# william-dawson/NTPoly

Hardware: AMD Instinct MI355X
Metric: TRS2 iters/s + SpGEMM nnz-out/s, N=262k ~200 nnz/row, 1/2/4/8 GPU (higher is better)
Workload: dtype f64

## Files before the change

### include/ntpoly_amd.h

```cpp
#ifndef NTPOLY_AMD_H
#define NTPOLY_AMD_H
#include "ntpoly_amd_process_grid.h"
#include "ntpoly_amd_psmatrix.h"
#include "ntpoly_amd_smatrix.h"
#include "ntpoly_amd_triplet_list.h"
#include "ntpoly_amd_permutation.h"
#include "ntpoly_amd_memory_pool.h"
#include "ntpoly_amd_solver_parameters.h"
#include "ntpoly_amd_density_matrix_solvers.h"
#include "ntpoly_amd_sign_solvers.h"
#include "ntpoly_amd_inverse_solvers.h"
#include "ntpoly_amd_square_root_solvers.h"
#include "ntpoly_amd_load_balancer.h"
#include "ntpoly_amd_eigen_bounds.h"
#include "ntpoly_amd_logging.h"
#include "ntpoly_amd_polynomial_solvers.h"
#include "ntpoly_amd_function_solvers.h"
#include "ntpoly_amd_linear_solvers.h"
#include "ntpoly_amd_eigen_solvers.h"
#include "ntpoly_amd_geometry.h"
#ifdef __cplusplus
extern "C" {
#endif

void ntpoly_amd_allreduce_max(double* values, const int* n);
int ntpoly_amd_band_order(const int* ih, int* newpos, long long* bandwidth);
void ntpoly_amd_band_scope_counts(long long* out);
void ntpoly_amd_band_searches(long long* out);
void ntpoly_amd_barrier();
void ntpoly_amd_block_algebra_counts(long long* out);
int ntpoly_amd_block_order(const int* ih, int* position);
int ntpoly_amd_block_order_of_pattern(const int* ih, int* position, int* ns);
void ntpoly_amd_block_scope_counts(long long* out);
void ntpoly_amd_column_fused_counts(long long* out);
int ntpoly_amd_comm_rank();
int ntpoly_amd_comm_size();
void ntpoly_amd_comm_split_matrix(const int* ih_this, int* ih_split, int* my_color, bool* split_slice);
void ntpoly_amd_complex_fusion_counts(long long* out);
int ntpoly_amd_device_count();
void ntpoly_amd_drop_block_caches();
void ntpoly_amd_drop_grouped_caches();
void ntpoly_amd_exchange_stats(long long* out);
void ntpoly_amd_fill_prepartitioned(const int* ih_this, const int* ih_triplet_list);
void ntpoly_amd_finalize_comm();
void ntpoly_amd_fusion_counts(long long* out);
void ntpoly_amd_gather_matrix_to_process(const int* ih_this, int* ih_local, const int* within_slice_id);
int ntpoly_amd_get_option(const char* name);
void ntpoly_amd_get_spgemm_accum(long long* out, double* dout);
void ntpoly_amd_get_unique_id(char* out128);
void ntpoly_amd_ghash_class_counts(long long out[4]);
void ntpoly_amd_grid_comm_info(const int* ih_grid, int* out);
void ntpoly_amd_halo_segment(const int* dim, const int* nranks, const int* s, const int* kmin, const int* kmax, int* a, int* b);
void ntpoly_amd_increment_identity(const int* ih_identity, int* ih_matB, const double* alpha);
void ntpoly_amd_init_comm(const char* id128, const int* rank, const int* nranks);
void ntpoly_amd_isr_chain_counts(long long out[3]);
int ntpoly_amd_isr_chain_step(const int* ih_X, const int* ih_X2, const int* order, const double* a, const double* b, const double* c, int* ih_Out1, int* ih_Out2);
void ntpoly_amd_last_block_stats(long long* out, double* fill);
void ntpoly_amd_last_grouped_stats(long long* out, double* ratio);
void ntpoly_amd_last_spgemm_stats(long long* out, float* ms_numeric, float* ms_total);
int ntpoly_amd_last_spgemm_thin();
void ntpoly_amd_log_element_bool(const char* key, const int* nk, const bool* v);
void ntpoly_amd_log_element_int(const char* key, const int* nk, const int* v);
void ntpoly_amd_log_element_real(const char* key, const int* nk, const double* v);
void ntpoly_amd_log_element_string(const char* key, const int* nk, const char* v, const int* nv);
void ntpoly_amd_log_enter();
void ntpoly_amd_log_exit();
void ntpoly_amd_log_header(const char* text, const int* n);
void ntpoly_amd_log_list_element(const char* key, const int* nk);
void ntpoly_amd_malloc_stats(long long* calls, double* ms);
int ntpoly_amd_matrix_is_complex(const int* ih_this);
void ntpoly_amd_matrix_local_columns(const int* ih_this, int* c0, int* c1);
void ntpoly_amd_memory(long long* in_use, long long* cached);
int ntpoly_amd_norm_axpby(const int* ih_matA, const int* ih_matB, const double* alpha, const double* beta, double* norm);
void ntpoly_amd_panel_exchange_layout(const int* dim, const int* nranks, const int* me, const long long* req, const long long* cnt, int* sa, int* sb, long long* soff, int* ra, int* rb, long long* zoff);
void ntpoly_amd_panel_product_counts(long long* out);
void ntpoly_amd_panel_range(const int* dim, const int* nranks, const int* rank, int* c0, int* c1);
void ntpoly_amd_permutation_set(int* ih_this, const int* n, const int* index_lookup);
int ntpoly_amd_pm_fused_step(const int* ih_X, const int* ih_Z, const int* ih_X2, const int* ih_X3, const double* a1, const double* a2, const double* a3, const double* thr, int* ih_Out, int* ih_Zout, double* sc);
void ntpoly_amd_pm_session_counts(long long out[4]);
void ntpoly_amd_pm_session_longest_list(long long* out);
int ntpoly_amd_recurrence_step(const int* ih_P, const int* ih_Tkm2, int* ih_Tk, int* ih_R, const double* a, const double* c);
void ntpoly_amd_recurrence_step_count(long long* out);
void ntpoly_amd_release_cache();
void ntpoly_amd_reset_spgemm_accum();
void ntpoly_amd_session_begin(const int* complex_ok);
void ntpoly_amd_session_end();
void ntpoly_amd_set_option(const char* name, const int* value);
void ntpoly_amd_slab_algebra_counts(long long* out);
void ntpoly_amd_slab_view_counts(long long out[4]);
void ntpoly_amd_split_process_grid(const int* ih_old_grid, int* ih_new_grid, int* my_color, bool* split_slice);
void ntpoly_amd_square_root_order(const int* ih_Input, int* ih_Output, const int* ih_solver_parameters, const int* inverse, const int* order);
void ntpoly_amd_synchronize();
void ntpoly_amd_thin_slab_counts(long long* out);
void ntpoly_amd_tile2_counts(long long* out);
void ntpoly_amd_trace_get(double* value, double* energy, double* sigma, long long* nnz);
int ntpoly_amd_trace_iterations();
void ntpoly_amd_trace_times(double* setup_ms, double* loop_ms);
void ntpoly_amd_triplets_get(const int* ih_list, int* col, int* row, double* val);
void ntpoly_amd_triplets_set_c(int* ih_list, const long long* n, const int* col, const int* row, const double* val_ri);
void ntpoly_amd_triplets_set_r(int* ih_list, const long long* n, const int* col, const int* row, const double* val);
void ntpoly_amd_trs2_step(int* ih_X, int* ih_X2, const int* ih_WH, const double* trace, const double* threshold, double* energy_out, double* sigma_out, double* trace_io);

#ifdef __cplusplus
}
#endif
#endif
```

### ntpoly_amd/csrc/common.hpp

```cpp
#pragma once
#include <hip/hip_runtime.h>

#include <cstdint>
#include <cstdio>
#include <cstdlib>
#include <map>
#include <string>
#include <utility>
#include <memory>
#include <vector>

namespace ntp {

[[noreturn]] void fatal(const char* file, int line, const std::string& msg);
#define NTP_FATAL(msg) ::ntp::fatal(__FILE__, __LINE__, (msg))
#define HIP_CHECK(expr)                                                              \
  do {                                                                               \
    hipError_t e_ = (expr);                                                          \
    if (e_ != hipSuccess)                                                            \
      ::ntp::fatal(__FILE__, __LINE__, std::string(#expr) + ": " + hipGetErrorString(e_)); \
  } while (0)

struct Context {
  int device = 0;
  hipStream_t stream = nullptr;
  hipStream_t comm_stream = nullptr;
  int num_cus = 256;
  bool initialised = false;
};
Context& ctx();
void ensure_init();
inline hipStream_t stream() { return ctx().stream; }
void sync_stream();
long long& host_sync_count();

struct ScalarFetch {
  const void* src[16];
  int words[16];
  void* dst[16];
  int n = 0;
  void add(const void* dev, int words8, void* host_dst) {
    src[n] = dev; words[n] = words8; dst[n] = host_dst; ++n;
  }
  void run();
};

void* dev_alloc(size_t bytes);
void dev_free(void* p);
unsigned long long dev_alloc_serial(const void* p);
void dev_release_cache();
size_t dev_bytes_in_use();
size_t dev_bytes_cached();
void dev_malloc_stats(long long* calls, double* ms);

template <typename T>
struct DevBuf {
  T* p = nullptr;
  size_t n = 0;
  DevBuf() = default;
  explicit DevBuf(size_t count) { alloc(count); }
  DevBuf(const DevBuf&) = delete;
  DevBuf& operator=(const DevBuf&) = delete;
  DevBuf(DevBuf&& o) noexcept : p(o.p), n(o.n) { o.p = nullptr; o.n = 0; }
  DevBuf& operator=(DevBuf&& o) noexcept {
    if (this != &o) {
      release();
      p = o.p; n = o.n; o.p = nullptr; o.n = 0;
    }
    return *this;
  }
  ~DevBuf() { release(); }
  void alloc(size_t count) {
    release();
    n = count;
    p = static_cast<T*>(dev_alloc((count ? count : 1) * sizeof(T)));
  }
  void release() {
    if (p) dev_free(p);
    p = nullptr; n = 0;
  }
  void upload(const T* host, size_t count) {
    if (count) HIP_CHECK(hipMemcpyAsync(p, host, count * sizeof(T), hipMemcpyHostToDevice, stream()));
  }
  void download(T* host, size_t count) const {
    const size_t bytes = count * sizeof(T);
    if (bytes > 0 && bytes <= 1024 && bytes % 8 == 0) {
      ScalarFetch f;
      f.add(p, (int)(bytes / 8), host);
      f.run();
      return;
    }
    if (count) HIP_CHECK(hipMemcpyAsync(host, p, bytes, hipMemcpyDeviceToHost, stream()));
    sync_stream();
  }
  void zero() { if (n) HIP_CHECK(hipMemsetAsync(p, 0, n * sizeof(T), stream())); }
};

constexpr size_t kIndexSlack = 1024;

struct SlabPlan {
  DevBuf<int32_t> blk_lo, blk_w, blk_kmin, blk_kn;
  DevBuf<int64_t> blk_toff;
  int64_t total = 0;
  int max_w = 0, max_kn = 0;
  int align = 0;
};
struct SlabForm {
  DevBuf<int32_t> first, last, count;
  DevBuf<int64_t> off;
  DevBuf<int64_t> tile_off;
  DevBuf<double> val, tiles;
  int64_t slots = 0;
  bool no_tile2 = false;
  std::unique_ptr<SlabPlan> next_plan;
  std::shared_ptr<struct DevMat> origin;
  DevBuf<int32_t> zlast;
  mutable int64_t span_sum = -1;
  int row_pad = 1;
  DevBuf<int32_t> lab, plast;
  bool labelled() const { return lab.p != nullptr; }
};

struct DevMat {
  int32_t rows = 0, cols = 0;
  bool cplx = false;
  int64_t nnz = 0;
  DevBuf<int64_t> outer;
  DevBuf<int32_t> inner;
  DevBuf<double> val;
  DevBuf<int32_t> cnt;
  int64_t slots = 0;
  bool loose() const { return cnt.p != nullptr; }
  mutable int zero_free = 0;
  std::unique_ptr<SlabForm> slab;
  bool expanded() const { return slab != nullptr; }
  std::shared_ptr<struct BlockForm> blk;
  bool blocked() const { return blk != nullptr; }
  mutable int block_hint = 0;
  mutable int slab_hint = 0;

  DevMat() = default;
  DevMat(int32_t r, int32_t c, bool z) { reset_empty(r, c, z); }
  DevMat(DevMat&&) noexcept = default;
  DevMat& operator=(DevMat&&) noexcept = default;
  void reset_empty(int32_t r, int32_t c, bool z);
  void alloc(int32_t r, int32_t c, bool z, int64_t nz);
  DevMat clone() const;
  size_t wval() const { return cplx ? 2 : 1; }
};

DevMat packed_copy(const DevMat& M);

struct HostTriplets {
  std::vector<int32_t> col, row;
  std::vector<double> val;
  bool cplx = false;
  size_t size() const { return col.size(); }
};

}
```

### ntpoly_amd/csrc/kernels.hip

```cpp
#include "kernels.hpp"
#include "device_util.hpp"
#include "spgemm_grouped.hpp"
#include "slab_types.hpp"
#include "spgemm_tile.hpp"
#include "spgemm_block.hpp"

#include <hip/hip_runtime.h>

#include <algorithm>
#include <cstdlib>
#include <climits>
#include <cmath>
#include <cstring>
#include <type_traits>
#include <numeric>
#include <utility>

#include <rocprim/device/device_radix_sort.hpp>

namespace ntp {

namespace {

__global__ __launch_bounds__(1024) void k_scan_excl_i64(const int64_t* __restrict__ in,
// ... 2590 lines not shown

static int64_t exclusive_scan_i64_from_i32(const int32_t* d_in, int64_t* d_out, int64_t n) {
  scan_async<int32_t>(d_in, d_out, n);
  int64_t total = 0;
  ScalarFetch f;
  f.add(d_out + n, 1, &total);
  f.run();
  return total;
}
int64_t exclusive_scan_i64(const int64_t* d_in, int64_t* d_out, int64_t n) {
  scan_async<int64_t>(d_in, d_out, n);
  int64_t total = 0;
  HIP_CHECK(hipMemcpyAsync(&total, d_out + n, sizeof(int64_t), hipMemcpyDeviceToHost, stream()));
  sync_stream();
  return total;
}

namespace {
struct TimedCall {
  hipEvent_t ev[4];
};
std::vector<hipEvent_t>& event_pool() {
  static auto* p = new std::vector<hipEvent_t>();
  return *p;
}
std::vector<TimedCall>& pending_timings() {
  static auto* p = new std::vector<TimedCall>();
  return *p;
}
hipEvent_t get_event() {
  auto& pool = event_pool();
  if (!pool.empty()) {
    hipEvent_t e = pool.back();
    pool.pop_back();
    return e;
  }
  hipEvent_t e;
  HIP_CHECK(hipEventCreate(&e));
  return e;
}
struct EventTimer {
  hipEvent_t a = nullptr, b = nullptr;
  bool on;
  explicit EventTimer(bool enable) : on(enable) {
    if (on) {
      a = get_event();
      b = get_event();
    }
  }
  void start() { if (on) HIP_CHECK(hipEventRecord(a, stream())); }
  void stop() { if (on) HIP_CHECK(hipEventRecord(b, stream())); }
};
}

namespace {
unsigned long long& value_epoch() {
  static unsigned long long e = 0;
  return e;
}
}
unsigned long long matrix_value_epoch() { return value_epoch(); }
void bump_matrix_value_epoch() { value_epoch() += 1; }
namespace {
struct DotOperand {
  const void* val = nullptr;
  unsigned long long serial = 0, epoch = 0;
  int64_t nnz = -1;
  int32_t cols = 0;
  DevBuf<int32_t> dmin, dmax;
  DevBuf<int64_t> doff;
  DevBuf<double> dexp;
  int64_t max_tile = 0;
  int align = 1;
};
template <typename T>
__global__ __launch_bounds__(256) void k_count_zero_values(Csc A, unsigned long long* __restrict__ out, int32_t* __restrict__ zlast) {
  const int j = (blockIdx.x * blockDim.x + threadIdx.x) / WAVE;
  if (j >= A.cols) return;
  const int lane = lane_id();
  const T* __restrict__ v = static_cast<const T*>(A.val);
  int zl = -1;
  for (int64_t p = A.outer[j] + lane, e = col_end(A, j); p < e; p += WAVE)
    if (Sc<T>::is_zero(v[p])) zl = max(zl, A.inner[p]);
  zl = wave_max_i32(zl);
  if (lane == 0) {
    if (zlast) zlast[j] = zl;
    if (zl >= 0) atomicAdd(out, 1ull);
  }
}
__global__ void k_span_block_max(const int32_t* __restrict__ span, int n, int J, unsigned long long* __restrict__ out) {
  const int b = blockIdx.x * blockDim.x + threadIdx.x;
  if (b * J >= n) return;
  unsigned long long t = 0;
  for (int j = b * J; j < min(n, (b + 1) * J); ++j) t += (unsigned long long)span[j];
  atomicMax(out, t);
}
DotOperand*& dot_operand_slot() {
  static DotOperand* c = new DotOperand();
  return c;
}
void drop_dot_operand() { *dot_operand_slot() = DotOperand(); }
const DotOperand& dot_operand(const DevMat& D) {
  DotOperand* c = dot_operand_slot();
  const unsigned long long ser = dev_alloc_serial(D.val.p);
  const int want_al = options().spgemm_fma == 1 ? tile_expand_align() : 1;
  if (c->val == D.val.p && c->serial == ser && ser != 0 && c->epoch == value_epoch() && c->nnz == D.nnz && c->cols == D.cols &&
      c->align == want_al)
    return *c;
  const int n = D.cols;
  c->dmin.alloc((size_t)n); c->dmax.alloc((size_t)n); c->doff.alloc((size_t)n + 1);
  DevBuf<int32_t> dlen((size_t)n), dspan((size_t)n);
  hipLaunchKernelGGL(k_col_extent, dim3(cdiv(n, 256)), dim3(256), 0, stream(), view(D), c->dmin.p, c->dmax.p, dlen.p);
  const int al = options().spgemm_fma == 1 ? tile_expand_align() : 1;
  if (al > 1) hipLaunchKernelGGL(k_span_aligned, dim3(cdiv(n, 256)), dim3(256), 0, stream(), c->dmin.p, c->dmax.p, dspan.p, n, al);
  else hipLaunchKernelGGL(k_span_of, dim3(cdiv(n, 256)), dim3(256), 0, stream(), c->dmin.p, c->dmax.p, dspan.p, n);
  scan_async<int32_t>(dspan.p, c->doff.p, (int64_t)n);
  DevBuf<unsigned long long> tmax(1);
  tmax.zero();
  hipLaunchKernelGGL(k_span_block_max, dim3(cdiv(cdiv(n, SLAB_J), 256)), dim3(256), 0, stream(), dspan.p, n, SLAB_J, tmax.p);
  int64_t total = 0;
  unsigned long long hmax = 0;
  {
    ScalarFetch f;
    f.add(c->doff.p + n, 1, &total);
    f.add(tmax.p, 1, &hmax);
    f.run();
  }
  c->max_tile = (int64_t)hmax;
  c->dexp.alloc((size_t)total + 1);
  if (al > 1)
    hipLaunchKernelGGL(k_aligned_offsets<double>, dim3(cdiv((int64_t)n * WAVE, 256)), dim3(256), 0, stream(), c->dmin.p, c->dmax.p,
                       c->doff.p, c->dexp.p, n, al);
  c->align = al;
  hipLaunchKernelGGL(k_slab_expand_a<double>, dim3(cdiv((int64_t)n * WAVE, 256)), dim3(256), 0, stream(), view(D), c->dmin.p,
                     c->doff.p, c->dexp.p);
  c->val = D.val.p;
  c->serial = ser;
  c->epoch = value_epoch();
  c->nnz = D.nnz;
  c->cols = n;
  return *c;
}
}

long long* fusion_counts() {
  static long long c[3] = {0, 0, 0};
  return c;
}
long long* complex_fusion_counts() {
  static long long c[3] = {0, 0, 0};
  return c;
}
long long* tile2_counts() {
  static long long c[2] = {0, 0};
  return c;
}

void flush_spgemm_timers() {
  auto& pend = pending_timings();
  if (pend.empty()) return;
  SpgemmAccum& acc = spgemm_accum();
  for (size_t i = 0; i < pend.size(); ++i) {
    float t_all = 0.f, t_num = 0.f;
    HIP_CHECK(hipEventSynchronize(pend[i].ev[1]));
    HIP_CHECK(hipEventElapsedTime(&t_all, pend[i].ev[0], pend[i].ev[1]));
    HIP_CHECK(hipEventElapsedTime(&t_num, pend[i].ev[2], pend[i].ev[3]));
    acc.ms_total += t_all;
    acc.ms_numeric += t_num;
    if (i + 1 == pend.size()) {
      last_spgemm_stats().ms_total = t_all;
      last_spgemm_stats().ms_numeric = t_num;
    }
    for (int k = 0; k < 4; ++k) event_pool().push_back(pend[i].ev[k]);
  }
  pend.clear();
}

namespace {
__global__ __launch_bounds__(256) void k_pack_slab(int ncols, const int32_t* __restrict__ first, const int32_t* __restrict__ last,
                                                   const int64_t* __restrict__ off, const double* __restrict__ val,
                                                   const int64_t* __restrict__ outer, int32_t* __restrict__ inner,
                                                   double* __restrict__ out) {
  const int j = (blockIdx.x * blockDim.x + threadIdx.x) / WAVE;
  if (j >= ncols) return;
  const int lane = lane_id();
  const int f = first[j], l = last[j];
  int64_t pos = outer[j];
  const double* __restrict__ src = val + off[j];
  for (int r0 = f; r0 <= l; r0 += WAVE) {
    const int r = r0 + lane;
    const double v = r <= l ? src[r - f] : 0.0;
    const unsigned long long m = __ballot(v != 0.0);
    if (v != 0.0) {
      const int64_t q = pos + __popcll(m & lanemask_lt());
      inner[q] = r;
      out[q] = v;
    }
    pos += __popcll(m);
  }
}
__global__ __launch_bounds__(256) void k_pack_slab_c(int ncols, const int32_t* __restrict__ first, const int32_t* __restrict__ last,
                                                     const int64_t* __restrict__ off, const double2* __restrict__ val,
                                                     const int64_t* __restrict__ outer, int32_t* __restrict__ inner,
                                                     double2* __restrict__ out) {
  const int j = (blockIdx.x * blockDim.x + threadIdx.x) / WAVE;
  if (j >= ncols) return;
  const int lane = lane_id();
  const int f = first[j], l = last[j];
  int64_t pos = outer[j];
  const double2* __restrict__ src = val + off[j];
  for (int r0 = f; r0 <= l; r0 += WAVE) {
    const int r = r0 + lane;
    const double2 v = r <= l ? src[r - f] : make_double2(0.0, 0.0);
    const bool nz = v.x != 0.0 || v.y != 0.0;
    const unsigned long long m = __ballot(nz);
    if (nz) {
      const int64_t q = pos + __popcll(m & lanemask_lt());
      inner[q] = r;
      out[q] = v;
    }
    pos += __popcll(m);
  }
}
template <int MAXCH, int NW>
void launch_pair3(int bin_lo, int bin_hi, int wrt, const DevMat& A, const DevMat& B, const int32_t* lo, const int32_t* span,
                  const uint8_t* binarr, const int64_t* tmpoff, int32_t* out_inner, double* out_val, int32_t* count,
                  double alpha, double thr, int dense_rule) {
  const int ngroups = cdiv(B.cols, 2);
  const int nblocks = cdiv(ngroups, NW);
  const size_t lds = (size_t)NW * 2 * (size_t)wrt * sizeof(double);
  hipLaunchKernelGGL((k_spgemm_pair3<MAXCH, NW>), dim3(xcd_grid(nblocks)), dim3(NW * WAVE), lds, stream(), view(A), view(B),
                     lo, span, binarr, bin_lo, bin_hi, tmpoff, out_inner, out_val, count, alpha, thr, dense_rule, nblocks, wrt);
}

template <typename T, int W, int NW>
void launch_window(int bin, const DevMat& A, const DevMat& B, const int32_t* lo, const int32_t* span,
                   const uint8_t* binarr, const int64_t* tmpoff, int32_t* out_inner, T* out_val,
                   int32_t* count, double alpha, double thr, int dense_rule) {
  const int nblocks = cdiv(B.cols, NW);
  hipLaunchKernelGGL((k_spgemm_window<T, W, NW>), dim3(xcd_grid(nblocks)), dim3(NW * WAVE), 0, stream(),
                     view(A), view(B), lo, span, binarr, bin, tmpoff, out_inner, out_val, count, alpha, thr,
                     dense_rule, nblocks);
}
}

namespace {
struct StripCtx { bool active = false, failed = false; };
constexpr int kMaxStrips = 16;
int* strips_memory(bool cplx) {
  static int m[2][2] = {{-1, 0}, {-1, 0}};
  return m[cplx ? 1 : 0];
}
StripCtx& strip_ctx() {
  static StripCtx c;
  return c;
}
template <typename T>
__global__ __launch_bounds__(256) void k_strip_count(Csc A, int shift, int S, int s, int32_t* __restrict__ cnt) {
  const int j = (blockIdx.x * blockDim.x + threadIdx.x) / WAVE;
  if (j >= A.cols) return;
  const int lane = lane_id();
  int c = 0;
  for (int64_t p = A.outer[j] + lane, e = A.outer[j + 1]; p < e; p += WAVE) c += ((A.inner[p] >> shift) % S) == s ? 1 : 0;
  c = (int)wave_sum_i64(c);
  if (lane == 0) cnt[j] = c;
}
template <typename T>
__global__ __launch_bounds__(256) void k_strip_fill(Csc A, int shift, int S, int s, const int64_t* __restrict__ outer,
                                                    int32_t* __restrict__ inner, T* __restrict__ val) {
  const int j = (blockIdx.x * blockDim.x + threadIdx.x) / WAVE;
  if (j >= A.cols) return;
  const int lane = lane_id();
  const T* __restrict__ Av = static_cast<const T*>(A.val);
  int64_t pos = outer[j];
  for (int64_t p0 = A.outer[j], e = A.outer[j + 1]; p0 < e; p0 += WAVE) {
    const int64_t p = p0 + lane;
    const bool in = p < e && ((A.inner[p] >> shift) % S) == s;
    const unsigned long long m = __ballot(in);
    if (in) {
      const int64_t q = pos + __popcll(m & lanemask_lt());
      inner[q] = A.inner[p];
      val[q] = Av[p];
    }
    pos += __popcll(m);
  }
}
struct StripCols { const int64_t* outer[16]; const int32_t* inner[16]; const void* val[16]; };
__global__ void k_strip_total(StripCols P, int S, int n, int32_t* __restrict__ total) {
  const int j = blockIdx.x * blockDim.x + threadIdx.x;
  if (j >= n) return;
  int t = 0;
  for (int s = 0; s < S; ++s) t += (int)(P.outer[s][j + 1] - P.outer[s][j]);
  total[j] = t;
}
template <typename T>
__global__ __launch_bounds__(256) void k_strip_merge(StripCols P, int S, int shift, int n, const int64_t* __restrict__ outer,
                                                     int32_t* __restrict__ inner, T* __restrict__ val) {
  const int j = (blockIdx.x * blockDim.x + threadIdx.x) / WAVE;
  if (j >= n) return;
  const int lane = lane_id();
  int rmin = INT_MAX, rmax = -1;
  for (int s = 0; s < S; ++s) {
    const int64_t a = P.outer[s][j], e = P.outer[s][j + 1];
    if (e > a) {
      rmin = min(rmin, P.inner[s][a]);
      rmax = max(rmax, P.inner[s][e - 1]);
// ... 947 lines not shown
  C.rows = m;
  C.cols = n;
  C.cplx = A.cplx;
  C.outer.alloc((size_t)n + 1);
  scan_async<int32_t>(count.p, C.outer.p, (int64_t)n);
  int64_t nnz = 0;
  unsigned long long slab_products = 0;
  {
    ScalarFetch f;
    f.add(C.outer.p + n, 1, &nnz);
    if (use_slab) f.add(blk_prod_scan.p + snb, 1, &slab_products);
    f.run();
  }
  if (use_slab) st.products = (int64_t)slab_products;
  C.nnz = nnz;
  C.inner.alloc((size_t)nnz + kIndexSlack);
  C.val.alloc(((size_t)nnz + kIndexSlack) * C.wval());
  const int nblocks = cdiv(n, 4);
  if (use_tile)
    hipLaunchKernelGGL(k_pack_slab, dim3(cdiv((int64_t)n * WAVE, 256)), dim3(256), 0, stream(), n, fz_first.p, fz_last.p,
                       tile_ooff.p, tmp_val.p, C.outer.p, C.inner.p, C.val.p);
  else if (use_ctile)
    hipLaunchKernelGGL(k_pack_slab_c, dim3(cdiv((int64_t)n * WAVE, 256)), dim3(256), 0, stream(), n, fz_first.p, fz_last.p,
                       tile_ooff.p, reinterpret_cast<const double2*>(tmp_val.p), C.outer.p, C.inner.p, reinterpret_cast<double2*>(C.val.p));
  else dispatch_type(A.cplx, [&](auto tag) {
    using T = decltype(tag);
    hipLaunchKernelGGL((k_compact<T>), dim3(xcd_grid(nblocks)), dim3(256), 0, stream(), n, tmpoff.p,
                       overflow ? tmpoff2.p : nullptr, overflow ? bin.p : nullptr, C.outer.p, tmp_inner.p,
                       reinterpret_cast<const T*>(tmp_val.p), tmp2_inner.p, reinterpret_cast<const T*>(tmp2_val.p),
                       C.inner.p, reinterpret_cast<T*>(C.val.p), nblocks);
  });
  t_all.stop();
  st.nnz_c = nnz;
  if (timing) {
    if (pending_timings().size() >= 4096) flush_spgemm_timers();
    pending_timings().push_back(TimedCall{{t_all.a, t_all.b, t_num.a, t_num.b}});
  }
  last_spgemm_stats() = st;
  SpgemmAccum& acc = spgemm_accum();
  acc.calls += 1;
  acc.products += st.products;
  acc.nnz_c += nnz;
  const double per = A.cplx ? 20.0 : 12.0;
  acc.alg_bytes += per * (double)(A.nnz + B.nnz + nnz) + 4.0 * ((double)A.cols + B.cols + n + 3);
}


namespace {
}

namespace {
__global__ void k_pack_reduce4(const double* __restrict__ tot, const int* __restrict__ flag, double* __restrict__ out) {
  out[0] = tot[3];
  out[1] = 0.0;
  out[2] = tot[4];
  out[3] = flag[0] == 0 ? 1.0 : 0.0;
}
__global__ void k_slab_runs_addr(const int32_t* __restrict__ first, const int32_t* __restrict__ last,
                                 const unsigned long long* __restrict__ addr, unsigned long long fallback,
                                 SlabRun* __restrict__ runs, int n, int elem_bytes) {
  const int k = blockIdx.x * blockDim.x + threadIdx.x;
  if (k >= n + 4) return;
  const bool any = k < n && last[k] >= first[k];
  SlabRun r;
  const unsigned long long a = any ? addr[k] : fallback;
  r.addr_lo = (uint32_t)a;
  r.addr_hi = (uint32_t)(a >> 32) & 0xffffu;
  r.nbytes = any ? (uint32_t)(last[k] - first[k] + 1) * (uint32_t)elem_bytes : 0u;
  r.flags = kBufferFlags;
  r.first = any ? first[k] : (1 << 30);
  r.first8 = any ? first[k] * elem_bytes : 0;
  r.span62 = any ? (last[k] - first[k] + 1) + 62 : 0;
  r.pad = 0;
  runs[k] = r;
}

__global__ __launch_bounds__(256) void k_slab_order_steps(const int32_t* __restrict__ lab, const int32_t* __restrict__ blk_kmin,
                                                          const int32_t* __restrict__ blk_kn, const int64_t* __restrict__ tile_off,
                                                          const double* __restrict__ tiles_in, const SlabRun* __restrict__ runs,
                                                          int ncols, double* __restrict__ tiles_out, SlabRun* __restrict__ blkruns,
                                                          int32_t* __restrict__ steps, int nblocks) {
  extern __shared__ unsigned long long sk[];
  const int b = xcd_block(nblocks);
  if (b < 0) return;
  const int kn = blk_kn[b], kmin = blk_kmin[b];
  if (kn == 0) return;
  int m = 1;
  while (m < kn) m <<= 1;
  for (int i = threadIdx.x; i < m; i += blockDim.x)
    sk[i] = i < kn ? (((unsigned long long)(unsigned)lab[kmin + i] << 32) | (unsigned)i) : ~0ull;
  __syncthreads();
  for (int k = 2; k <= m; k <<= 1) {
    for (int j = k >> 1; j > 0; j >>= 1) {
      for (int i = threadIdx.x; i < m; i += blockDim.x) {
        const int l = i ^ j;
        if (l > i) {
          const bool up = (i & k) == 0;
          const unsigned long long x = sk[i], y = sk[l];
          if ((x > y) == up) { sk[i] = y; sk[l] = x; }
        }
      }
      __syncthreads();
    }
  }
  const int64_t toff = tile_off[b];
  const int64_t rbase = toff / SLAB_J + 4 * (int64_t)b;
  for (int t = threadIdx.x; t < kn + 4; t += blockDim.x) {
    if (t < kn) {
      const int i = (int)(unsigned)(sk[t] & 0xffffffffull);
      const int k = kmin + i;
      if (steps) steps[rbase + t] = k;
      SlabRun r = runs[k];
      r.pad = i * (int)(SLAB_J * sizeof(double));
      blkruns[rbase + t] = r;
    } else {
      if (steps) steps[rbase + t] = ncols;
      blkruns[rbase + t] = runs[ncols];
    }
  }
  if (!tiles_out) return;
  const double2* __restrict__ src = reinterpret_cast<const double2*>(tiles_in + toff);
  double2* __restrict__ dst = reinterpret_cast<double2*>(tiles_out + toff);
  for (int i = threadIdx.x; i < kn * (SLAB_J / 2); i += blockDim.x) {
    const int t = i / (SLAB_J / 2), q = i % (SLAB_J / 2);
    dst[(size_t)t * (SLAB_J / 2) + q] = src[(size_t)(unsigned)(sk[t] & 0xffffffffull) * (SLAB_J / 2) + q];
  }
}
}

namespace {
template <int J = SLAB_J>
void launch_slab_plan(SlabPlan& P, int n, const int32_t* first, const int32_t* last, const int32_t* afirst, const int32_t* alast,
                      int align, unsigned long long* stats, DevBuf<int64_t>* tile_offsets = nullptr) {
  const int snb = cdiv(n, J);
  P.blk_lo.alloc(snb); P.blk_w.alloc(snb); P.blk_kmin.alloc(snb); P.blk_kn.alloc(snb);
  P.blk_toff.alloc((size_t)snb + 1);
  P.align = align;
  DevBuf<int64_t> bsz(snb), tsz(snb);
  if (tile_offsets) tile_offsets->alloc((size_t)snb + 1);
  hipLaunchKernelGGL((k_slab_plan<J>), dim3(cdiv((int64_t)snb * WAVE, 256)), dim3(256), 0, stream(), n, first, last, afirst,
                     alast, P.blk_lo.p, P.blk_w.p, P.blk_kmin.p, P.blk_kn.p, bsz.p, tsz.p, snb, align);
  if (options().plan_fused != 0) {
    const int part = cdiv(cdiv(snb, kOffParts), 256) * 256;
    hipLaunchKernelGGL(k_slab_offsets, dim3(cdiv(snb, part)), dim3(256), 0, stream(), P.blk_w.p, P.blk_kn.p, tsz.p, bsz.p, snb, part,
                       P.blk_toff.p, tile_offsets ? tile_offsets->p : (int64_t*)nullptr, stats);
    return;
  }
  hipLaunchKernelGGL(k_slab_reduce, dim3(64), dim3(256), 0, stream(), P.blk_w.p, P.blk_kn.p, snb, (const int32_t*)nullptr, 0, stats);
  scan_async<int64_t>(tsz.p, P.blk_toff.p, (int64_t)snb);
  if (tile_offsets) scan_async<int64_t>(bsz.p, tile_offsets->p, (int64_t)snb);
}
}

bool slab_step(DevMat& X, SlabFusion& fu, double threshold, bool dense_rule, const SlabHalo* halo) {
  fu.done = false;
  if (!X.expanded() || X.cplx || (!halo && X.rows != X.cols) || !fu.D || fu.D->cplx || fu.D->loose() || fu.D->expanded() ||
      fu.D->rows != X.rows || fu.D->cols != X.cols || (fu.mode != 1 && fu.mode != 2))
    return false;
  const bool tile = options().spgemm_fma == 1;
  if ((options().spgemm_variant >= 0 && !(tile && options().spgemm_variant / 100 == 6)) || (options().spgemm_fma && !tile) || options().spgemm_force_bin > 0 || !options().fused_update)
    return false;
  const SlabForm& in = *X.slab;
  int trows = 1;
  if (tile) {
    trows = tile_rows();
    while (trows > 1 && (in.row_pad % (16 * trows) != 0 || (halo && halo->row_pad % (16 * trows) != 0))) trows >>= 1;
  }
  const int n = X.cols, snb = cdiv(n, SLAB_J);
  const DotOperand& dop = dot_operand(*fu.D);
  if (!tile && dop.max_tile > SLAB_DTILE) return false;
  const bool timing = options().time_kernels != 0;
  EventTimer t_all(timing), t_num(timing);
  t_all.start();
  SpgemmStats st;
  st.nnz_a = st.nnz_b = X.nnz;
  DevBuf<int32_t> count((size_t)n), ofirst((size_t)n), olast((size_t)n);
  DevBuf<int64_t> tmpoff((size_t)n + 1);
  DevBuf<int64_t> zwords((size_t)4 * snb + 4 + 48);
  zwords.zero();
  if (!tile) count.zero();
  int64_t* fz_flag = zwords.p;
  int64_t* fz_pnnz = zwords.p + 2;
  double* fz_part = reinterpret_cast<double*>(zwords.p + 3 + 2 * (size_t)snb);
  unsigned long long* stats = reinterpret_cast<unsigned long long*>(zwords.p + 4 * (size_t)snb + 4);
  unsigned long long* next_stats = stats + 24;
  const int ka = halo ? halo->ka : 0, nka = halo ? halo->kb - halo->ka : n;
  const int plan_align = tile ? 16 * tile_rows() : 0;
  SlabPlan own_plan;
  SlabPlan* plan = &own_plan;
  if (!halo && in.next_plan && in.next_plan->align == plan_align && (int64_t)in.next_plan->blk_lo.n == snb) {
    plan = in.next_plan.get();
  } else if (halo && halo->plan && halo->plan->align == plan_align && (int64_t)halo->plan->blk_lo.n == snb) {
    plan = halo->plan;
  } else {
    const int32_t* afirst = halo ? halo->first - ka : in.first.p;
    const int32_t* alast = halo ? halo->last - ka : in.last.p;
    launch_slab_plan(own_plan, n, in.first.p, in.last.p, afirst, alast, plan_align, stats);
    unsigned long long hs[3] = {0, 0, 0};
    ScalarFetch f;
    f.add(own_plan.blk_toff.p + snb, 1, &own_plan.total);
    f.add(stats + 16, 3, hs);
    f.run();
    own_plan.max_w = (int)hs[0];
    own_plan.max_kn = (int)hs[1];
  }
  DevBuf<int32_t>&blk_lo = plan->blk_lo, &blk_w = plan->blk_w, &blk_kmin = plan->blk_kmin, &blk_kn = plan->blk_kn;
  DevBuf<int64_t>& blk_toff = plan->blk_toff;
  const int64_t tmp_total = plan->total;
  const unsigned long long hst[2] = {(unsigned long long)plan->max_w, (unsigned long long)plan->max_kn};
  const int64_t max_w = (int64_t)hst[0];
  auto give_up = [&]() {
    if (timing) {
      event_pool().push_back(t_all.a); event_pool().push_back(t_all.b);
      event_pool().push_back(t_num.a); event_pool().push_back(t_num.b);
    }
    return false;
  };
  if (max_w <= 0 || (!tile && max_w > 8 * SLAB_SL * WAVE)) return give_up();
  if (tile && !spgemm_tile_fits((int)hst[1], (int)max_w)) return give_up();
  if (in.labelled() && (int64_t)hst[1] > 2048) return give_up();
  if (!tile)
    hipLaunchKernelGGL((k_slab_tmpoff<SLAB_J>), dim3(cdiv(n + 1, 256)), dim3(256), 0, stream(), n, blk_w.p, blk_toff.p, tmpoff.p);
  DevBuf<char> runs(((size_t)nka + 4) * sizeof(SlabRun));
  if (halo)
    hipLaunchKernelGGL(k_slab_runs_addr, dim3(cdiv(nka + 4, 256)), dim3(256), 0, stream(), halo->first, halo->last, halo->addr,
                       (unsigned long long)reinterpret_cast<uintptr_t>(in.val.p), reinterpret_cast<SlabRun*>(runs.p), nka, 8);
  else
    hipLaunchKernelGGL(k_slab_runs, dim3(cdiv(n + 4, 256)), dim3(256), 0, stream(), in.first.p, in.last.p, in.off.p,
                       reinterpret_cast<const char*>(in.val.p), 8, reinterpret_cast<SlabRun*>(runs.p), n);
  const size_t oslots = (size_t)tmp_total + (size_t)tmp_total / 5 + kIndexSlack;
  const bool runs_only = tile && !halo && options().tile_runs_only != 0;
  DevBuf<double> oval(oslots), otiles(runs_only ? 0 : oslots);
  SlabFuseArgs fz;
  fz.am = fu.am; fz.bm = fu.bm; fz.thr_m = fu.threshold;
  fz.xexp = in.val.p; fz.xoff = in.off.p; fz.xmin = in.first.p; fz.xmax = in.last.p;
  fz.dexp = dop.dexp.p; fz.doff = dop.doff.p; fz.dmin = dop.dmin.p; fz.dmax = dop.dmax.p;
  fz.ofirst = ofirst.p; fz.olast = olast.p; fz.tiles = runs_only ? nullptr : otiles.p;
  fz.part = fz_part; fz.pnnz = reinterpret_cast<long long*>(fz_pnnz); fz.flag = reinterpret_cast<int*>(fz_flag);
  fz.col_offset = fu.col_offset;
  int64_t* blk_prod = zwords.p + 3 + snb;
  const bool labelled = in.labelled() && !halo && !tile;
  if (in.labelled() && halo) return give_up();
  DevBuf<double> tiles_ord;
  DevBuf<char> blkruns;
  DevBuf<int32_t> steps, oplast;
  const bool rowoff = labelled && options().label_rowoff != 0;
  if (labelled) {
    const size_t nrec = in.tiles.n / SLAB_J + 4 * (size_t)snb + 8;
    blkruns.alloc(nrec * sizeof(SlabRun));
    oplast.alloc((size_t)n);
    if (!rowoff) {
      tiles_ord.alloc(in.tiles.n);
      steps.alloc(nrec);
    }
    int m = 1;
    while (m < (int)hst[1]) m <<= 1;
    hipLaunchKernelGGL(k_slab_order_steps, dim3(xcd_grid(snb)), dim3(256), (size_t)m * 8, stream(), in.lab.p, blk_kmin.p, blk_kn.p,
                       in.tile_off.p, in.tiles.p, reinterpret_cast<const SlabRun*>(runs.p), n, tiles_ord.p,
                       reinterpret_cast<SlabRun*>(blkruns.p), steps.p, snb);
    fz.lab = in.lab.p;
    fz.blkruns = reinterpret_cast<const SlabRun*>(blkruns.p);
    fz.steps = steps.p;
    fz.xplast = in.plast.p;
    fz.oplast = oplast.p;
  }
  const bool scope_lab = tile && halo && !in.labelled() && scope_labels() != nullptr && in.plast.p != nullptr && fu.mode != 0;
  const bool tile_labelled = tile && ((in.labelled() && !halo) || scope_lab);
  if (tile_labelled) {
    oplast.alloc((size_t)n);
    fz.lab = scope_lab ? scope_labels() : in.lab.p;
    fz.xplast = in.plast.p;
    fz.oplast = oplast.p;
  }
  fz.prod = reinterpret_cast<long long*>(blk_prod);
  if (!halo || halo->count) fz.in_count = halo ? halo->count - ka : in.count.p;
  DevBuf<char> fz_args;
  if (!tile) {
    fz_args.alloc(sizeof(SlabFuseArgs));
    fz_args.upload(reinterpret_cast<const char*>(&fz), sizeof(SlabFuseArgs));
  }
  const int dr = dense_rule ? 1 : 0;
  t_num.start();
  auto launch = [&](auto nw_tag, auto mode_tag, auto epi_tag) {
    constexpr int FNW = decltype(nw_tag)::value;
    hipLaunchKernelGGL((k_spgemm_slab<SLAB_J, SLAB_SL, FNW, decltype(mode_tag)::value, decltype(epi_tag)::value>),
                       dim3(xcd_grid(snb)), dim3(FNW * WAVE), 0, stream(), reinterpret_cast<const SlabRun*>(runs.p) - ka,
                       (labelled && !rowoff) ? tiles_ord.p : in.tiles.p, in.tile_off.p, blk_kmin.p, blk_kn.p, blk_lo.p, blk_w.p, blk_toff.p, (int32_t*)nullptr,
                       oval.p, count.p, 1.0, threshold, dr, n, snb, reinterpret_cast<const SlabFuseArgs*>(fz_args.p));
  };
  auto by_mode = [&](auto nw_tag, auto mode_tag) {
    if (fu.mode == 1) launch(nw_tag, mode_tag, std::integral_constant<int, 1>{});
    else launch(nw_tag, mode_tag, std::integral_constant<int, 2>{});
  };
  DevBuf<int64_t> tile_ooff, tile_otoff;
  bool used_tile2 = false;
  if (tile) {
    tile_ooff.alloc((size_t)n + 1);
    tile_otoff.alloc((size_t)snb + 1);
    TileLaunch tl;
    tl.runs = reinterpret_cast<const SlabRun*>(runs.p) - ka;
    tl.bblk = in.tiles.p; tl.blk_boff = in.tile_off.p;
    if (in.tiles.p == nullptr || in.tile_off.p == nullptr) {
      tl.bblk = nullptr; tl.blk_boff = nullptr;
      tl.brun_first = in.first.p; tl.brun_last = in.last.p; tl.brun_off = in.off.p; tl.brun_val = in.val.p; tl.bbytes = in.val.n * sizeof(double); tl.brun_pad = in.row_pad;
    }
    tl.blk_kmin = blk_kmin.p; tl.blk_kn = blk_kn.p; tl.blk_lo = blk_lo.p;
    tl.blk_w = blk_w.p; tl.blk_toff = blk_toff.p; tl.out_val = oval.p; tl.count = count.p;
    tl.ofirst = ofirst.p; tl.olast = olast.p; tl.ooff = tile_ooff.p; tl.otoff = tile_otoff.p;
    tl.alpha = 1.0; tl.threshold = threshold; tl.dense_rule = dr; tl.ncols = n; tl.nblocks = snb;
    tl.max_kn = (int)hst[1]; tl.max_w = (int)max_w; tl.epi = fu.mode; tl.fz = &fz; tl.rows = trows; tl.labelled = tile_labelled;
    tl.nrows = X.rows;
    if (!halo) {
      tl.abase = in.val.p; tl.abytes = in.val.n * sizeof(double);
      tl.dbase = dop.dexp.p; tl.dbytes = dop.dexp.n * sizeof(double);
    }
    if (!halo && options().tile2 != 0 && !in.no_tile2) used_tile2 = launch_spgemm_tile2(tl, reinterpret_cast<int*>(fz_flag) + 2);
    if (!used_tile2) launch_spgemm_tile(tl);
  } else if (rowoff) {
    if (max_w > 6 * SLAB_SL * WAVE) by_mode(std::integral_constant<int, 8>{}, std::integral_constant<int, 9>{});
    else if (max_w > SLAB_NW * SLAB_SL * WAVE) by_mode(std::integral_constant<int, 6>{}, std::integral_constant<int, 9>{});
    else by_mode(std::integral_constant<int, SLAB_NW>{}, std::integral_constant<int, 9>{});
  } else if (max_w > 6 * SLAB_SL * WAVE) by_mode(std::integral_constant<int, 8>{}, std::integral_constant<int, 0>{});
  else if (max_w > SLAB_NW * SLAB_SL * WAVE) by_mode(std::integral_constant<int, 6>{}, std::integral_constant<int, 0>{});
  else by_mode(std::integral_constant<int, SLAB_NW>{}, std::integral_constant<int, 8>{});
  t_num.stop();
  DevBuf<double> lvl((size_t)5 * FT_BLOCKS), tot(5);
  hipLaunchKernelGGL(k_fused_totals, dim3(FT_BLOCKS), dim3(256), 0, stream(), count.p, n,
                     reinterpret_cast<const long long*>(fz_pnnz), reinterpret_cast<const long long*>(blk_prod), fz_part, snb,
                     (const double*)nullptr, lvl.p, 0);
  hipLaunchKernelGGL(k_fused_totals, dim3(1), dim3(256), 0, stream(), (const int32_t*)nullptr, 0, (const long long*)nullptr,
                     (const long long*)nullptr, (const double*)nullptr, 0, lvl.p, tot.p, 1);
  unsigned long long raw[5] = {0, 0, 0, 0, 0};
  int64_t flagv[2] = {0, 0};
  DevBuf<double> red4;
  if (halo && halo->reduce) {
    red4.alloc(4);
    hipLaunchKernelGGL(k_pack_reduce4, dim3(1), dim3(1), 0, stream(), tot.p, reinterpret_cast<const int*>(fz_flag), red4.p);
    halo->reduce->allreduce(red4.p);
  }
  std::unique_ptr<SlabPlan> next;
  unsigned long long next_hs[3] = {0, 0, 0};
  if (tile && !halo && options().plan_ahead != 0) {
    next.reset(new SlabPlan());
    launch_slab_plan(*next, n, ofirst.p, olast.p, ofirst.p, olast.p, plan_align, next_stats);
  }
  DevMat R;
  R.rows = X.rows;
  R.cols = n;
  R.cplx = false;
  R.zero_free = 1;
  R.slab.reset(new SlabForm());
  R.slab->first = std::move(ofirst);
  R.slab->last = std::move(olast);
  R.slab->count = std::move(count);
  R.slab->row_pad = tile ? 16 * trows : 1;
  R.slab->no_tile2 = in.no_tile2;
  R.slab->off = tile ? std::move(tile_ooff) : std::move(tmpoff);
  if (tile) R.slab->tile_off = std::move(tile_otoff);
  R.slab->val = std::move(oval);
  if (runs_only) { R.slab->tile_off.release(); } else R.slab->tiles = std::move(otiles);
  R.slab->slots = tmp_total;
  {
    ScalarFetch f;
    f.add(tot.p, 5, raw);
    f.add(fz_flag, 2, flagv);
    if (red4.p) f.add(red4.p, 4, halo->reduce->reduced);
    if (next) {
      f.add(next->blk_toff.p + snb, 1, &next->total);
      f.add(next_stats + 16, 3, next_hs);
    }
    if (halo && halo->before_fetch) halo->before_fetch(R, reinterpret_cast<const long long*>(tot.p), f);
    f.run();
    if (red4.p) halo->reduce->done = true;
  }
  t_all.stop();
  if (next) {
    next->max_w = (int)next_hs[0];
    next->max_kn = (int)next_hs[1];
  }
  if (std::getenv("NTPOLY_AMD_DEBUG_SPGEMM"))
    std::fprintf(stderr, "[slab_step] mode %d slots %lld w %llu kn %llu in-slots %lld nnz-in %lld plan %s\n", fu.mode, (long long)tmp_total,
                 hst[0], hst[1], (long long)in.slots, (long long)X.nnz, plan == &own_plan ? "made here" : "left by the step before");
  if (timing) {
    if (pending_timings().size() >= 4096) flush_spgemm_timers();
    pending_timings().push_back(TimedCall{{t_all.a, t_all.b, t_num.a, t_num.b}});
  }
  if (used_tile2 && (int32_t)flagv[1] != 0) {
    X.slab->no_tile2 = true;
    tile2_counts()[1] += 1;
    return slab_step(X, fu, threshold, dense_rule, halo);
  }
  if (used_tile2) tile2_counts()[0] += 1;
  if ((int32_t)flagv[0] != 0) {
    fu.refused += 1;
    fusion_counts()[2] += 1;
    return false;
  }
  const int64_t nnz = (int64_t)raw[0], pnz = (int64_t)raw[1];
  double hd[2];
  std::memcpy(hd, &raw[3], 2 * sizeof(double));
  const int64_t nnz_in = X.nnz;
  R.nnz = nnz;
  R.slab->next_plan = std::move(next);
  if (!tile) R.slab->tile_off = std::move(plan->blk_toff);
  if (labelled || tile_labelled) {
    R.slab->lab = std::move(X.slab->lab);
    R.slab->plast = std::move(oplast);
  }
  if (halo) fu.result = std::move(R);
  else X = std::move(R);
  fu.done = true;
  fu.dot = hd[0];
  fu.trace = hd[1];
  fu.product_nnz = pnz;
  fusion_counts()[fu.mode == 1 ? 0 : 1] += 1;
  st.slab = 1;
  st.fused = fu.mode;
  st.nnz_c = pnz;
  st.tmp_entries = tmp_total;
  const bool counted = !halo || halo->count;
  st.products = counted ? (int64_t)raw[2] : -1;
  last_spgemm_stats() = st;
  SpgemmAccum& acc = spgemm_accum();
  acc.calls += 1;
  if (counted) acc.products += (int64_t)raw[2];
  acc.nnz_c += pnz;
  acc.alg_bytes += 12.0 * (double)(2 * nnz_in + pnz) + 4.0 * (3.0 * n + 3);
  return true;
}

bool slab_from_csc(DevMat& Xs, DevBuf<int32_t>& lab) {
  if (Xs.cplx || Xs.loose() || Xs.expanded() || Xs.rows != Xs.cols || Xs.nnz == 0) return false;
  const int n = Xs.cols, snb = cdiv(n, SLAB_J);
  std::unique_ptr<SlabForm> f(new SlabForm());
  f->first.alloc((size_t)n); f->last.alloc((size_t)n); f->count.alloc((size_t)n); f->off.alloc((size_t)n + 1);
  f->tile_off.alloc((size_t)snb + 1); f->plast.alloc((size_t)n);
  DevBuf<int32_t> span((size_t)n), blk_lo(snb), blk_w(snb), blk_kmin(snb), blk_kn(snb);
  DevBuf<int64_t> bsz(snb), tsz(snb), dummy(snb);
  DevBuf<unsigned long long> stats(24);
  stats.zero();
  hipLaunchKernelGGL(k_col_extent, dim3(cdiv(n, 256)), dim3(256), 0, stream(), view(Xs), f->first.p, f->last.p, f->count.p);
  const int al = options().spgemm_fma == 1 ? tile_expand_align() : 1;
  if (al > 1) hipLaunchKernelGGL(k_span_aligned, dim3(cdiv(n, 256)), dim3(256), 0, stream(), f->first.p, f->last.p, span.p, n, al);
  else hipLaunchKernelGGL(k_span_of, dim3(cdiv(n, 256)), dim3(256), 0, stream(), f->first.p, f->last.p, span.p, n);
  scan_async<int32_t>(span.p, f->off.p, (int64_t)n);
  hipLaunchKernelGGL((k_slab_plan<SLAB_J>), dim3(cdiv((int64_t)snb * WAVE, 256)), dim3(256), 0, stream(), n, f->first.p, f->last.p,
                     f->first.p, f->last.p, blk_lo.p, blk_w.p, blk_kmin.p, blk_kn.p, bsz.p, tsz.p, snb);
  hipLaunchKernelGGL(k_slab_reduce, dim3(64), dim3(256), 0, stream(), blk_w.p, blk_kn.p, snb, (const int32_t*)nullptr, 0, stats.p);
  scan_async<int64_t>(bsz.p, f->tile_off.p, (int64_t)snb);
  int64_t tot_val = 0, tot_tiles = 0;
  unsigned long long hst[2] = {0, 0};
  {
    ScalarFetch ft;
    ft.add(f->off.p + n, 1, &tot_val);
    ft.add(f->tile_off.p + snb, 1, &tot_tiles);
    ft.add(stats.p + 16, 2, hst);
    ft.run();
  }
  const int64_t max_w = (int64_t)hst[0], max_kn = (int64_t)hst[1];
  const int pitch = ((int)max_kn + 1) | 1;
  if (max_w <= 0 || max_w > 8 * SLAB_SL * WAVE || (size_t)pitch * SLAB_J * 8 > 128 * 1024) return false;
  if ((double)tot_val > 2.0 * (double)Xs.nnz + (al > 1 ? 2.0 * al * (double)n : 0.0)) return false;
  f->val.alloc((size_t)tot_val + kIndexSlack);
  if (al > 1)
    hipLaunchKernelGGL(k_aligned_offsets<double>, dim3(cdiv((int64_t)n * WAVE, 256)), dim3(256), 0, stream(), f->first.p, f->last.p,
                       f->off.p, f->val.p, n, al);
  f->row_pad = al;
  f->tiles.alloc((size_t)tot_tiles + 16 * SLAB_J + kIndexSlack);
  hipLaunchKernelGGL(k_slab_expand_a<double>, dim3(cdiv((int64_t)n * WAVE, 256)), dim3(256), 0, stream(), view(Xs), f->first.p,
                     f->off.p, f->val.p);
  if ((size_t)pitch * SLAB_J * 8 > 64 * 1024) {
    static bool raised = false;
    if (!raised) {
      HIP_CHECK(hipFuncSetAttribute(reinterpret_cast<const void*>(&k_slab_expand_b<double, SLAB_J>),
                                    hipFuncAttributeMaxDynamicSharedMemorySize, 144 * 1024));
      raised = true;
    }
  }
  hipLaunchKernelGGL((k_slab_expand_b<double, SLAB_J>), dim3(xcd_grid(snb)), dim3(256), (size_t)pitch * SLAB_J * 8, stream(), view(Xs),
                     blk_kmin.p, blk_kn.p, f->tile_off.p, f->tiles.p, snb, pitch, 0, (const int64_t*)nullptr, (double*)nullptr,
                     (const int32_t*)nullptr, dummy.p);
  hipLaunchKernelGGL(k_col_plast, dim3(cdiv((int64_t)n * WAVE, 256)), dim3(256), 0, stream(), view(Xs), lab.p, f->plast.p);
  f->slots = std::max(tot_val, tot_tiles);
  f->lab = std::move(lab);
  DevMat R;
  R.rows = Xs.rows;
  R.cols = n;
  R.cplx = false;
  R.nnz = Xs.nnz;
  R.zero_free = Xs.zero_free;
  R.slab = std::move(f);
  Xs = std::move(R);
  return true;
}

void increment(const DevMat& A, DevMat& B, double alpha, double threshold) {
  axpby(A, B, alpha, 1.0, threshold, nullptr, nullptr, nullptr, 0);
}

namespace {
struct MergeOperand {
  Csc v;
  int32_t rows, cols;
  bool cplx;
  int64_t slots;
  bool loose;
};
void axpby_impl(const MergeOperand& A, DevMat& B, double alpha, double beta, double threshold, const DevMat* D,
                double* dot_out, double* trace_out, int32_t trace_col_offset, int64_t* a_nnz_out,
                const int64_t* d_extra = nullptr, int64_t* extra_out = nullptr, int row_block = 0,
                bool keep_loose = false) {
  if (A.rows != B.rows || A.cols != B.cols) NTP_FATAL("increment: shape mismatch");
  if (A.cplx != B.cplx) NTP_FATAL("increment: mixed scalar types must be up-cast by the caller");
  if (D && (D->rows != A.rows || D->cols != A.cols || D->cplx != A.cplx)) NTP_FATAL("increment: dot operand mismatch");
  if (dot_out) dot_out[0] = dot_out[1] = 0.0;
  if (a_nnz_out) *a_nnz_out = A.loose ? 0 : A.slots;
  const int n = A.cols;
  if (n == 0) return;
  if (!A.loose && A.slots == 0 && B.nnz == 0) return;
  DevBuf<int32_t> lo(n), span(n), count(n);
  DevBuf<uint8_t> bin(n);
  DevBuf<unsigned long long> stats(16);
  const Csc Bv = lview(B);
  hipLaunchKernelGGL(k_inc_plan, dim3(cdiv(n, 256)), dim3(256), 0, stream(), A.v, Bv, lo.p, span.p, bin.p,
                     stats.p, count.p, row_block > 0 ? 2 : options().increment_force_seq);
  hipLaunchKernelGGL(k_bin_hist, dim3(std::min(cdiv(n, 256), 512)), dim3(256), 0, stream(), bin.p, (const int64_t*)nullptr,
                     (const int32_t*)nullptr, n, stats.p);
  unsigned long long hs[16];
  {
    ScalarFetch f;
    f.add(stats.p, 16, hs);
    f.run();
  }
  const int64_t cap = A.slots + B.nnz;
  const size_t wv = A.cplx ? 2 : 1;
  DevBuf<int32_t> tmp_inner((size_t)cap + kIndexSlack);
  DevBuf<double> tmp_val(((size_t)cap + kIndexSlack) * wv);
  DevBuf<int64_t> srcoff((size_t)n + 1);
  if (keep_loose || B.loose()) {
    DevBuf<int32_t> both((size_t)n);
    hipLaunchKernelGGL(k_sum_counts, dim3(cdiv(n, 256)), dim3(256), 0, stream(), A.v, Bv, both.p);
    scan_async<int32_t>(both.p, srcoff.p, (int64_t)n);
  } else {
    hipLaunchKernelGGL(k_sum_outer, dim3(cdiv(n + 1, 256)), dim3(256), 0, stream(), A.v.outer, B.outer.p, srcoff.p, n);
  }
// ... 1406 lines not shown
  if (M.cplx || M.loose() || (M.rows != M.cols && !g_panels_ok) || M.nnz == 0 || (options().spgemm_fma != 0 && options().spgemm_fma != 1)) return false;
  const int n = M.cols;
  std::unique_ptr<SlabForm> f(new SlabForm());
  f->first.alloc((size_t)n); f->last.alloc((size_t)n); f->count.alloc((size_t)n); f->off.alloc((size_t)n + 1);
  DevBuf<int32_t> span((size_t)n);
  DevBuf<unsigned long long> zc(1);
  zc.zero();
  const int al = options().spgemm_fma == 1 ? tile_expand_align() : 1;
  hipLaunchKernelGGL(k_col_extent, dim3(cdiv(n, 256)), dim3(256), 0, stream(), view(M), f->first.p, f->last.p, f->count.p);
  hipLaunchKernelGGL(k_span_aligned, dim3(cdiv(n, 256)), dim3(256), 0, stream(), f->first.p, f->last.p, span.p, n, al);
  scan_async<int32_t>(span.p, f->off.p, (int64_t)n);
  const bool views = options().stored_zero_views != 0;
  if (M.zero_free != 1) {
    if (views) f->zlast.alloc((size_t)n);
    hipLaunchKernelGGL(k_count_zero_values<double>, dim3(cdiv((int64_t)n * WAVE, 256)), dim3(256), 0, stream(), view(M), zc.p, f->zlast.p);
  }
  int64_t tot = 0;
  unsigned long long hz = 0;
  {
    ScalarFetch ft;
    ft.add(f->off.p + n, 1, &tot);
    ft.add(zc.p, 1, &hz);
    ft.run();
  }
  if (hz == 0) f->zlast.release();
  const bool dbg = std::getenv("NTPOLY_AMD_DEBUG_SPGEMM") != nullptr;
  if (hz == 0) M.zero_free = 1;
  if ((double)tot > 2.0 * (double)M.nnz + 2.0 * al * (double)n) {
    if (dbg) std::fprintf(stderr, "[slab_enter] refused: slots %lld for %lld entries\n", (long long)tot, (long long)M.nnz);
    M.slab_hint = -1;
    return false;
  }
  f->val.alloc((size_t)tot + kIndexSlack);
  hipLaunchKernelGGL(k_aligned_offsets<double>, dim3(cdiv((int64_t)n * WAVE, 256)), dim3(256), 0, stream(), f->first.p, f->last.p,
                     f->off.p, f->val.p, n, al);
  hipLaunchKernelGGL(k_slab_expand_a<double>, dim3(cdiv((int64_t)n * WAVE, 256)), dim3(256), 0, stream(), view(M), f->first.p,
                     f->off.p, f->val.p);
  f->row_pad = al;
  f->slots = tot;
  DevMat R;
  R.rows = M.rows; R.cols = n; R.cplx = false; R.nnz = M.nnz; R.zero_free = hz == 0 ? 1 : 0;
  if (hz != 0) {
    f->origin.reset(new DevMat(std::move(M)));
    if (views) slab_view_counts()[0] += 1;
  }
  R.slab = std::move(f);
  M = std::move(R);
  return true;
}

static bool sa_axpby_impl(const DevMat* A, const DevMat& Bin, DevMat& Out, double alpha, double beta, double thr) {
  const DevMat& X = A ? *A : Bin;
  const bool cplx = X.cplx;
  const bool have_b = A != nullptr;
  const SlabForm& fa = *X.slab;
  const SlabForm* fb = have_b ? Bin.slab.get() : nullptr;
  const int n = X.cols;
  const int al = have_b ? std::max(fa.row_pad, fb->row_pad) : fa.row_pad;
  if (have_b && (fa.row_pad != fb->row_pad && (al % fa.row_pad != 0 || al % fb->row_pad != 0))) return false;
  const int64_t bound = fa.slots + (have_b ? fb->slots : 0) + 2LL * al * n;
  std::unique_ptr<SlabForm> fo(new SlabForm());
  fo->first.alloc((size_t)n); fo->last.alloc((size_t)n); fo->count.alloc((size_t)n); fo->off.alloc((size_t)n + 1);
  DevBuf<int32_t> span((size_t)n);
  DevBuf<int64_t> base((size_t)n + 1);
  DevBuf<unsigned long long> stat(2);
  stat.zero();
  hipLaunchKernelGGL(k_sa_span, dim3(cdiv(n, 256)), dim3(256), 0, stream(), fa.first.p, fa.last.p, have_b ? fb->first.p : nullptr,
                     have_b ? fb->last.p : nullptr, n, al, span.p);
  scan_async<int32_t>(span.p, base.p, (int64_t)n);
  fo->val.alloc(((size_t)bound + kIndexSlack) * (cplx ? 2 : 1));
  if (cplx) {
    const double2* va = reinterpret_cast<const double2*>(fa.val.p);
    const double2* vb = have_b ? reinterpret_cast<const double2*>(fb->val.p) : nullptr;
    double2* vo = reinterpret_cast<double2*>(fo->val.p);
    if (have_b)
      hipLaunchKernelGGL((k_sa_axpby<double2, true>), dim3(cdiv((int64_t)n * WAVE, 256)), dim3(256), 0, stream(), n, fa.first.p, fa.last.p, fa.off.p,
                         va, fb->first.p, fb->last.p, fb->off.p, vb, base.p, al, alpha, beta, thr, vo, fo->first.p, fo->last.p, fo->count.p,
                         fo->off.p, stat.p, bound, fa.zlast.p, fb->zlast.p);
    else
      hipLaunchKernelGGL((k_sa_axpby<double2, false>), dim3(cdiv((int64_t)n * WAVE, 256)), dim3(256), 0, stream(), n, fa.first.p, fa.last.p, fa.off.p,
                         va, (const int32_t*)nullptr, (const int32_t*)nullptr, (const int64_t*)nullptr, (const double2*)nullptr, base.p, al, 1.0, 0.0,
                         0.0, vo, fo->first.p, fo->last.p, fo->count.p, fo->off.p, stat.p, bound, (const int32_t*)nullptr, (const int32_t*)nullptr);
  } else if (have_b)
    hipLaunchKernelGGL((k_sa_axpby<double, true>), dim3(cdiv((int64_t)n * WAVE, 256)), dim3(256), 0, stream(), n, fa.first.p, fa.last.p, fa.off.p,
                       fa.val.p, fb->first.p, fb->last.p, fb->off.p, fb->val.p, base.p, al, alpha, beta, thr, fo->val.p, fo->first.p,
                       fo->last.p, fo->count.p, fo->off.p, stat.p, bound, fa.zlast.p, fb->zlast.p);
  else
    hipLaunchKernelGGL((k_sa_axpby<double, false>), dim3(cdiv((int64_t)n * WAVE, 256)), dim3(256), 0, stream(), n, fa.first.p, fa.last.p, fa.off.p,
                       fa.val.p, (const int32_t*)nullptr, (const int32_t*)nullptr, (const int64_t*)nullptr, (const double*)nullptr,
                       base.p, al, 1.0, 0.0, 0.0, fo->val.p, fo->first.p, fo->last.p, fo->count.p, fo->off.p, stat.p, bound, (const int32_t*)nullptr,
                       (const int32_t*)nullptr);
  DevBuf<long long> tot;
  sa_sum_counts(fo->count.p, n, tot);
  int64_t nnz = 0, slots = 0;
  unsigned long long hs = 0;
  {
    ScalarFetch ft;
    ft.add(tot.p, 1, &nnz);
    ft.add(base.p + n, 1, &slots);
    ft.add(stat.p, 1, &hs);
    ft.run();
  }
  if (hs & 4ull) slab_view_counts()[3] += 1;
  if (hs != 0) return false;
  if (have_b && (fa.origin || fb->origin)) slab_view_counts()[2] += 1;
  fo->row_pad = al;
  fo->slots = slots;
  DevMat R;
  R.rows = X.rows; R.cols = n; R.cplx = cplx; R.nnz = nnz; R.zero_free = 1;
  R.slab = std::move(fo);
  Out = std::move(R);
  return true;
}

bool slab_axpby(const DevMat& A, DevMat& B, double alpha, double beta, double threshold) {
  if (!sa_operand(A) || !sa_operand(B) || A.cols != B.cols || &A == &B) return false;
  if (alpha == 0.0 || beta == 0.0) return false;
  if (!sa_mergeable(A) || !sa_mergeable(B)) return false;
  DevMat R;
  if (!sa_axpby_impl(&A, B, R, alpha, beta, threshold)) return false;
  value_epoch() += 1;
  B = std::move(R);
  return true;
}

bool slab_axpby_to(const DevMat& A, const DevMat& B, DevMat& Out, double alpha, double beta, double threshold) {
  if (!sa_operand(A) || !sa_operand(B) || A.cols != B.cols || &A == &B) return false;
  if (alpha == 0.0 || beta == 0.0 || !sa_mergeable(A) || !sa_mergeable(B)) return false;
  DevMat R;
  if (!sa_axpby_impl(&A, B, R, alpha, beta, threshold)) return false;
  Out = std::move(R);
  return true;
}

bool slab_clone(const DevMat& A, DevMat& Out) {
  if (sa_operand(A) && sa_view(A)) { sa_clone_view(A, Out); return true; }
  if (!sa_operand(A) || A.zero_free != 1) return false;
  return sa_axpby_impl(nullptr, A, Out, 1.0, 0.0, 0.0);
}

bool slab_scale(DevMat& A, double c) {
  if (!sa_operand(A) || c == 0.0 || (A.slab->origin && !sa_view(A))) return false;
  SlabForm& f = *A.slab;
  if (f.origin) {
    scale(*f.origin, c);
    slab_view_counts()[2] += 1;
  }
  value_epoch() += 1;
  hipLaunchKernelGGL(k_sa_scale<double>, dim3(cdiv((int64_t)A.cols * WAVE, 256)), dim3(256), 0, stream(), A.cols, f.first.p, f.last.p, f.off.p,
                     f.val.p, c);
  f.tiles.release();
  f.tile_off.release();
  f.next_plan.reset();
  return true;
}

bool slab_dot(const DevMat& A, const DevMat& B, double out[2]) {
  if (!sa_operand(A) || !sa_operand(B) || A.cols != B.cols) return false;
  const int n = A.cols;
  const SlabForm &fa = *A.slab, &fb = *B.slab;
  DevBuf<double> part((size_t)2 * n), res(2);
  hipLaunchKernelGGL(k_sa_dot, dim3(cdiv((int64_t)n * WAVE, 256)), dim3(256), 0, stream(), n, fa.first.p, fa.last.p, fa.off.p, fa.val.p,
                     fb.first.p, fb.last.p, fb.off.p, fb.val.p, part.p);
  reduce_sum2_async(part.p, n, res.p);
  unsigned long long h[2] = {0, 0};
  ScalarFetch ft;
  ft.add(res.p, 2, h);
  ft.run();
  std::memcpy(out, h, sizeof(h));
  return true;
}

bool slab_norm(const DevMat& A, double* out) {
  if (!sa_operand(A)) return false;
  const SlabForm& f = *A.slab;
  DevBuf<double> cs((size_t)A.cols);
  hipLaunchKernelGGL(k_sa_colstat<double>, dim3(cdiv((int64_t)A.cols * WAVE, 256)), dim3(256), 0, stream(), A.cols, f.first.p, f.last.p, f.off.p,
                     f.val.p, 0, 0, cs.p, (double*)nullptr);
  *out = max_of(cs, (size_t)A.cols);
  return true;
}

bool slab_gershgorin(const DevMat& A, int32_t col_offset, double* mn, double* mx) {
  if (!sa_operand(A)) return false;
  const SlabForm& f = *A.slab;
  DevBuf<double> lo((size_t)A.cols), hi((size_t)A.cols), res(2);
  hipLaunchKernelGGL(k_sa_colstat<double>, dim3(cdiv((int64_t)A.cols * WAVE, 256)), dim3(256), 0, stream(), A.cols, f.first.p, f.last.p, f.off.p,
                     f.val.p, col_offset, 1, lo.p, hi.p);
  launch_reduce_minmax(lo.p, hi.p, (int64_t)A.cols, res.p);
  double h[2];
  res.download(h, 2);
  *mn = h[0];
  *mx = h[1];
  return true;
}

namespace {
__global__ __launch_bounds__(256) void k_sa_tiles(int n, const int32_t* __restrict__ first, const int32_t* __restrict__ last,
                                                  const int64_t* __restrict__ off, const double* __restrict__ val,
                                                  const int32_t* __restrict__ blk_kmin, const int32_t* __restrict__ blk_kn,
                                                  const int64_t* __restrict__ boff, double* __restrict__ tiles, int nblocks) {
  const int b = xcd_block(nblocks);
  if (b < 0) return;
  const int kmin = blk_kmin[b], kn = blk_kn[b], kn2 = (kn + 1) & ~1;
  const int c = threadIdx.x & 15, j = b * SLAB_J + c;
  const bool colv = j < n;
  const int f = colv ? first[j] : INT_MAX, l = colv ? last[j] : -1;
  const double* __restrict__ p = (colv && l >= f) ? val + (off[j] - f) : val;
  double* __restrict__ dst = tiles + boff[b];
  for (int idx = threadIdx.x; idx < kn2 * SLAB_J; idx += 256) {
    const int r = kmin + (idx >> 4);
    dst[idx] = (r >= f && r <= l) ? p[r] : 0.0;
  }
}
struct EmptyDot {
  DevBuf<int32_t> dmin, dmax;
  DevBuf<int64_t> doff;
  DevBuf<double> dexp;
  int n = 0;
};
const EmptyDot& empty_dot(int n) {
  static EmptyDot* e = new EmptyDot();
  if (e->n < n) {
    e->dmin.alloc((size_t)n); e->dmax.alloc((size_t)n); e->doff.alloc((size_t)n + 1); e->dexp.alloc(8);
    std::vector<int32_t> hmin((size_t)n, INT_MAX), hmax((size_t)n, -1);
    e->dmin.upload(hmin.data(), (size_t)n);
    e->dmax.upload(hmax.data(), (size_t)n);
    sync_stream();
    e->doff.zero();
    e->dexp.zero();
    e->n = n;
  }
  return *e;
}

bool slab_multiply_loop(const DevMat& A, const DevMat& B, DevMat& C, double alpha, double threshold, bool dense_rule) {
  const SlabForm &fa = *A.slab, &fb = *B.slab;
  const int n = B.cols, snb = cdiv(n, SLAB_J);
  const bool timing = options().time_kernels != 0;
  EventTimer t_all(timing), t_num(timing);
  t_all.start();
  auto give_up = [&]() {
    if (timing) {
      event_pool().push_back(t_all.a); event_pool().push_back(t_all.b);
      event_pool().push_back(t_num.a); event_pool().push_back(t_num.b);
    }
    return false;
  };
  SlabPlan P;
  DevBuf<int64_t> zwords((size_t)4 * snb + 4 + 24);
  zwords.zero();
  int64_t* fz_flag = zwords.p;
  int64_t* fz_pnnz = zwords.p + 2;
  double* fz_part = reinterpret_cast<double*>(zwords.p + 3 + 2 * (size_t)snb);
  unsigned long long* stats = reinterpret_cast<unsigned long long*>(zwords.p + 4 * (size_t)snb + 4);
  const bool have_tiles = fb.tiles.p != nullptr && (int64_t)fb.tile_off.n == (int64_t)snb + 1;
  DevBuf<int64_t> boff;
  launch_slab_plan(P, n, fb.first.p, fb.last.p, fa.first.p, fa.last.p, 0, stats, have_tiles ? nullptr : &boff);
  unsigned long long hs[3] = {0, 0, 0};
  int64_t btotal = 0;
  {
    ScalarFetch f;
    f.add(P.blk_toff.p + snb, 1, &P.total);
    f.add(stats + 16, 3, hs);
    if (!have_tiles) f.add(boff.p + snb, 1, &btotal);
    f.run();
  }
  P.max_w = (int)hs[0];
  P.max_kn = (int)hs[1];
  const int64_t max_w = P.max_w;
  if (max_w <= 0 || max_w > 8 * SLAB_SL * WAVE || (((int64_t)P.max_kn + 1) | 1) * SLAB_J * 8 > 128 * 1024) return give_up();
  if (!have_tiles) {
    SlabForm& mb = const_cast<SlabForm&>(fb);
    mb.tiles.alloc((size_t)btotal + 16 * SLAB_J + kIndexSlack);
    hipLaunchKernelGGL(k_sa_tiles, dim3(xcd_grid(snb)), dim3(256), 0, stream(), n, fb.first.p, fb.last.p, fb.off.p, fb.val.p,
                       P.blk_kmin.p, P.blk_kn.p, boff.p, mb.tiles.p, snb);
    mb.tile_off = std::move(boff);
  }
  DevBuf<int64_t> tmpoff((size_t)n + 1);
  hipLaunchKernelGGL((k_slab_tmpoff<SLAB_J>), dim3(cdiv(n + 1, 256)), dim3(256), 0, stream(), n, P.blk_w.p, P.blk_toff.p, tmpoff.p);
  DevBuf<char> runs(((size_t)A.cols + 4) * sizeof(SlabRun));
  hipLaunchKernelGGL(k_slab_runs, dim3(cdiv(A.cols + 4, 256)), dim3(256), 0, stream(), fa.first.p, fa.last.p, fa.off.p,
                     reinterpret_cast<const char*>(fa.val.p), 8, reinterpret_cast<SlabRun*>(runs.p), A.cols);
  const size_t oslots = (size_t)P.total + kIndexSlack;
  std::unique_ptr<SlabForm> fo(new SlabForm());
  fo->first.alloc((size_t)n); fo->last.alloc((size_t)n); fo->count.alloc((size_t)n);
  fo->count.zero();
  fo->val.alloc(oslots);
  fo->tiles.alloc(oslots);
  const EmptyDot& ed = empty_dot(n);
  SlabFuseArgs fz;
  fz.dexp = ed.dexp.p; fz.doff = ed.doff.p; fz.dmin = ed.dmin.p; fz.dmax = ed.dmax.p;
  fz.ofirst = fo->first.p; fz.olast = fo->last.p; fz.tiles = fo->tiles.p;
  fz.part = fz_part; fz.pnnz = reinterpret_cast<long long*>(fz_pnnz); fz.flag = reinterpret_cast<int*>(fz_flag);
  fz.col_offset = 0;
  DevBuf<char> fz_args(sizeof(SlabFuseArgs));
  fz_args.upload(reinterpret_cast<const char*>(&fz), sizeof(SlabFuseArgs));
  const int dr = dense_rule ? 1 : 0;
  t_num.start();
  auto launch = [&](auto nw_tag, auto mode_tag) {
    constexpr int FNW = decltype(nw_tag)::value;
    hipLaunchKernelGGL((k_spgemm_slab<SLAB_J, SLAB_SL, FNW, decltype(mode_tag)::value, 1>), dim3(xcd_grid(snb)), dim3(FNW * WAVE), 0,
                       stream(), reinterpret_cast<const SlabRun*>(runs.p), fb.tiles.p, fb.tile_off.p, P.blk_kmin.p, P.blk_kn.p,
                       P.blk_lo.p, P.blk_w.p, P.blk_toff.p, (int32_t*)nullptr, fo->val.p, fo->count.p, alpha, threshold, dr, n, snb,
                       reinterpret_cast<const SlabFuseArgs*>(fz_args.p));
  };
// ... 521 lines not shown
```

### ntpoly_amd/csrc/kernels.hpp

```cpp
#pragma once
#include <functional>
#include "common.hpp"

namespace ntp {

struct SpgemmStats {
  int64_t nnz_a = 0, nnz_b = 0, nnz_c = 0;
  int64_t products = 0;
  int64_t tmp_entries = 0;
  int slab = 0;
  int fused = 0;
  int64_t bin_cols[6] = {0, 0, 0, 0, 0, 0};
  int64_t overflow_cols = 0;
  int grouped = 0;
  int strips = 0;
  int64_t gh_failed_cols = 0, gh_groups = 0, gh_tile_rows = 0;
  int gh_level = 0, gh_minhash = 0;
  double gh_union_ratio = 0;
  int block = 0;
  double block_fill = 0;
  int64_t block_tile_products = 0, block_cand = 0;
  int thin = 0;
  float ms_total = 0.f;
  float ms_numeric = 0.f;
};

struct EngineOptions {
  int spgemm_force_bin = -1;
  int increment_force_seq = 0;
  int time_kernels = 0;
  int spgemm_fma = 1;
  int block_path = 1;
  int slab_algebra = 1;
  int plan_ahead = 1;
  int operand_cache = 1;
  int tile_rows = 2;
  int tile_waves = 0;
  int thin_left = 1;
 int complex_sessions = 1;
  int column_fused = 1;
  int complex_tile = 1;
  int block_complex = 1;
  int tile2 = 0;
  int tile_runs_only = 1;
  int load_balance = 1;
  int virtual_grid = 0;
  int fused_update = 1;
  int block_scope = 1;
  int block_scope_complex = 1;
  int block_match = 0;
  int block_unfused = 0;
  int panel_sessions = 1;
  int thin_slab_complex = 1;
  int complex_poly_sessions = 2;
  int stored_zero_views = 1;
  int complex_panels = 1;
  int complex_density = 1;
  int ghash_mfma = 1;
  int ghash_mfma_complex = 1;
  int pm_session = 1;
  int isr_chain = 1;
  int tile_off32 = 1;
  int tile_bbuf = 2;
  int plan_fused = 1;
  int exchange_ahead = 1;
  int band_scope = 1;
  int label_order = 1;
  int label_rowoff = 1;
  int loose_iterates = 1;
  int halo_overlap = 1;
  int spgemm_variant = -1;
};
EngineOptions& options();
SpgemmStats& last_spgemm_stats();
struct SpgemmAccum { int64_t calls = 0, products = 0, nnz_c = 0; double alg_bytes = 0, ms_numeric = 0, ms_total = 0; };
SpgemmAccum& spgemm_accum();
void flush_spgemm_timers();

struct LooseProduct {
  bool valid = false;
  int32_t rows = 0, cols = 0;
  int64_t slots = 0;
  DevBuf<int64_t> start;
  DevBuf<int32_t> count;
  DevBuf<int32_t> inner;
  DevBuf<double> val;
  DevBuf<int64_t> prod_scan;
  int64_t prod_index = -1;
};

struct ColRange { int32_t a, b; };
struct SlabFusion {
  int mode = 0;
  double am = 0, bm = 0, threshold = 0;
  const DevMat* D = nullptr;
  int32_t col_offset = 0;
  int32_t panel_c0 = -1;
  bool done = false;
  DevMat result;
  double dot = 0, trace = 0;
  int64_t product_nnz = 0;
  int64_t refused = 0;
};
void spgemm(const DevMat& A, const DevMat& B, DevMat& C, double alpha, double threshold,
            bool dense_rule, LooseProduct* loose = nullptr, const ColRange* arange = nullptr, SlabFusion* fuse = nullptr);
bool trs2_block_step(DevMat& X, int mode, double threshold, bool dense_rule, const DevMat& D, double out[4]);
struct BlockKeepScope {
  BlockKeepScope();
  ~BlockKeepScope();
  BlockKeepScope(const BlockKeepScope&) = delete;
  BlockKeepScope& operator=(const BlockKeepScope&) = delete;
};
struct SlabReduce {
  void (*allreduce)(double* dev4) = nullptr;
  double reduced[4] = {0, 0, 0, 0};
  bool done = false;
};
struct SlabHalo {
  int32_t ka = 0, kb = 0;
  const int32_t* first = nullptr;
  const int32_t* last = nullptr;
  const unsigned long long* addr = nullptr;
  const int32_t* count = nullptr;
  int row_pad = 1;
  SlabReduce* reduce = nullptr;
  std::function<void(const DevMat& result, const long long* d_nnz, ScalarFetch& fetch)> before_fetch;
  SlabPlan* plan = nullptr;
  int thin = 0;
  int64_t nnz_a = 0;
  std::function<void(ScalarFetch& fetch)> on_fetch;
};
bool slab_plan_fits_tile(int max_kn, int max_w);
struct SlabPlan;
bool slab_multiply_takes_panel(const DevMat& A, const DevMat& B, int left_row_pad, int32_t ka, int32_t kb, const SlabPlan* plan);
void slab_plan_panel_async(const DevMat& X, const int64_t* d_ext_all, int pitch, int32_t dim, int P, SlabPlan& plan,
                           DevBuf<int32_t>& gfirst, DevBuf<int32_t>& glast, unsigned long long* stats24);
bool slab_step(DevMat& X, SlabFusion& fuse, double threshold, bool dense_rule, const SlabHalo* halo = nullptr);
void slab_request_async(const DevMat& X, int64_t* d_out4, const long long* d_nnz = nullptr);
void slab_extents_async(const DevMat& X, int64_t* d_ext, int64_t* d_pre);
void slab_pack_runs_async(const DevMat& X, const int64_t* d_pre, int32_t ja, int32_t jb, double* dst);
void slab_halo_layout_async(const int64_t* d_ext_all, const int64_t* d_pre_all, int pitch, int32_t dim, int P, int me,
                            int32_t ka, int32_t kb, const int32_t* d_ra, const int64_t* d_zoff, const double* d_recv,
                            const DevMat& X, int32_t* d_first, int32_t* d_last, unsigned long long* d_addr,
                            const int64_t* d_cnt_all = nullptr, int32_t* d_count = nullptr,
                            const int32_t* h_ra = nullptr, const int64_t* h_zoff = nullptr);
void slab_export_async(const DevMat& X, int64_t* d_out4, const long long* d_nnz, int64_t* d_ext, int64_t* d_pre, int64_t* d_cnt64);
void slab_counts_async(const DevMat& X, int64_t* d_cnt64);
bool slab_enter(DevMat& M);
bool slab_multiply(const DevMat& A, const DevMat& B, DevMat& C, double alpha, double threshold, bool dense_rule, const SlabHalo* left = nullptr);
inline bool block_arithmetic_ok() { return options().spgemm_fma == 1 || (options().spgemm_fma == 0 && options().block_unfused != 0); }
bool slab_panels_ok();
void slab_allow_panels(bool on);
bool sa_operand_c(const DevMat& M);
bool sa_readable_c(const DevMat& M);
bool slab_enter_c(DevMat& M, bool* not_run_like = nullptr, bool allow_view = true);
long long* slab_view_counts();
long long* ghash_class_counts();
void drop_grouped_caches();
bool slab_multiply_c(const DevMat& A, const DevMat& B, DevMat& C, double alpha, double threshold, bool dense_rule, const SlabHalo* left = nullptr);
bool slab_multiply_c_takes_panel(const DevMat& A, const DevMat& B, int left_row_pad, int32_t ka, int32_t kb, const SlabPlan* plan);
bool slab_add_diagonal_c(DevMat& B, double alpha, int32_t col_offset);
bool slab_norm_axpby_c(const DevMat& A, const DevMat& B, double alpha, double beta, double* out);
bool slab_recurrence_step_c(const DevMat& P, const DevMat& Tkm2, DevMat& Tk, DevMat& R, double a, double c);
bool slab_dot_trace_c(const DevMat& A, const DevMat* B, int32_t col_offset, double dot[2], double* trace);
bool slab_axpby(const DevMat& A, DevMat& B, double alpha, double beta, double threshold);
bool slab_axpby_to(const DevMat& A, const DevMat& B, DevMat& Out, double alpha, double beta, double threshold);
bool slab_clone(const DevMat& A, DevMat& Out);
bool slab_scale(DevMat& A, double c);
bool slab_dot(const DevMat& A, const DevMat& B, double out[2]);
bool slab_norm(const DevMat& A, double* out);
bool slab_axpby_c(const DevMat& A, DevMat& B, double alpha, double beta, double threshold);
bool slab_axpby_to_c(const DevMat& A, const DevMat& B, DevMat& Out, double alpha, double beta, double threshold);
bool slab_clone_c(const DevMat& A, DevMat& Out);
bool slab_scale_c(DevMat& A, double c);
bool slab_norm_c(const DevMat& A, double* out);
bool slab_gershgorin(const DevMat& A, int32_t col_offset, double* mn, double* mx);
bool slab_add_diagonal(DevMat& B, double alpha, int32_t col_offset);
bool slab_trs4_traces(const DevMat& X, const DevMat& X2, int32_t col_offset, double* trace_fx, double* trace_gx);
bool slab_trs4_operand(const DevMat& X, const DevMat& X2, double sigma, int32_t col_offset, DevMat& Out);
bool slab_norm_axpby(const DevMat& A, const DevMat& B, double alpha, double beta, double* out);
bool slab_isr_chain5(const DevMat& X, const DevMat& X2, double a, double b, double c, int32_t col_offset, DevMat& Temp2, DevMat& Temp);
bool slab_isr_chain3(const DevMat& X, const DevMat& X2, int32_t col_offset, DevMat& Out);
struct ZeroList {
  DevBuf<int64_t> off;
  DevBuf<int32_t> row;
  int64_t count = 0;
  void clear() { off.release(); row.release(); count = 0; }
};
bool slab_pm_sigma(const DevMat& X, const ZeroList& Z, const DevMat& X2, double thr, int32_t col_offset, double out2[2]);
bool slab_pm_update(const DevMat& X, const ZeroList& Z, const DevMat& X2, const DevMat& X3, double a1, double a2, double a3, double thr,
                    DevMat& Out, ZeroList& Zout);
void insert_stored_zeros(DevMat& M, const ZeroList& Z);
void zero_list_from_pattern(const DevMat& M, ZeroList& Z);
DevMat zero_list_matrix(const ZeroList& Z, int32_t rows, int32_t cols);
bool slab_trace(const DevMat& A, int32_t col_offset, double* out);
int64_t slab_span_sum(const DevMat& M);
long long slab_product_count(const DevMat& A, const DevMat& B);
bool slab_from_csc(DevMat& Xs, DevBuf<int32_t>& lab);
bool relabel_enter(DevMat& X, const DevMat& D);
const DevMat* relabelled_operand(const DevMat& D);
void relabel_giveup(const DevMat& D);
void drop_thin_transposes();
void drop_operand_caches();
void set_scope_labels(const int32_t* lab);
const int32_t* scope_labels();
void drop_pending_exchange();
bool find_band_order(const DevMat& A, DevBuf<int32_t>& newpos, int64_t* bandwidth);
int64_t column_span_sum(const DevMat& A);
unsigned long long pattern_fingerprint_of(const DevMat& A);
long long* fusion_counts();
long long* complex_fusion_counts();
long long* tile2_counts();
long long& band_searches();

void increment(const DevMat& A, DevMat& B, double alpha, double threshold);
void increment_blocked(const DevMat& A, DevMat& B, double alpha, double threshold, int32_t row_block);
void axpby(const DevMat& A, DevMat& B, double alpha, double beta, double threshold, const DevMat* D, double* dot_out,
           double* trace_out = nullptr, int32_t trace_col_offset = 0);
void axpby(const LooseProduct& A, DevMat& B, double alpha, double beta, double threshold, const DevMat* D, double* dot_out,
           double* trace_out, int32_t trace_col_offset, int64_t* a_nnz_out, bool keep_loose = false);
DevMat packed_copy(const DevMat& M);
void pack(DevMat& M);
bool square_keep_loose(DevMat& X, double threshold, bool dense_rule, const DevMat& D, double out[2], double* trace_out,
                       int32_t col_offset);
void pairwise(const DevMat& A, const DevMat& B, DevMat& C, bool conj_a);
void dot(const DevMat& A, const DevMat& B, double out[2]);
void dot_trace(const DevMat& A, const DevMat& B, double out[2], double* trace_out, int32_t col_offset);
void grand_sum(const DevMat& A, double out[2]);
double trace(const DevMat& A, int32_t col_offset);
void column_abs_sums(const DevMat& A, DevBuf<double>& out);
double max_of(const DevBuf<double>& v, size_t n);
void gershgorin(const DevMat& A, int32_t col_offset, double* mn, double* mx);
void scale(DevMat& A, double c);
void conjugate(DevMat& A);
void scale_columns(DevMat& A, const double* d_factor);
DevMat to_complex(const DevMat& A);
DevMat to_real(const DevMat& A);
DevMat identity(int32_t n, int32_t col_offset, int32_t cols, bool cplx);
int64_t identity_check(const DevMat& A, int32_t col_offset);
DevMat transpose(const DevMat& A);
DevMat remap_general(const DevMat& A, const int32_t* d_row_map, const int32_t* d_col_map, int32_t new_rows,
                     int32_t col_lo, int32_t col_hi, bool drop_exact_zeros);
DevMat transpose_slice(const DevMat& A, int32_t col_lo, int32_t col_hi);
DevMat column_slice(const DevMat& A, int32_t c0, int32_t c1);
DevMat mask_columns(const DevMat& A, int32_t col_offset, int32_t block, int32_t slices, int32_t slice);
DevMat concat_columns(const std::vector<const DevMat*>& parts);

DevMat from_triplets(const HostTriplets& t, int32_t rows, int32_t cols, int32_t col_offset);
void to_triplets(const DevMat& A, int32_t col_offset, HostTriplets& out);

void copy_shift_i64(const int64_t* d_src, int64_t* d_dst, int64_t count, int64_t shift);

void rebase_i64(const int64_t* d_src, int64_t* d_dst, int64_t count, int64_t add);
void fill_i64(int64_t* d_dst, int64_t count, int64_t v);
void row_range(const DevMat& A, int32_t* lo, int32_t* hi);
void halo_request_async(const DevMat& B, int64_t nnz_a, int64_t* d_out4);
void halo_interior_async(const DevMat& B, int32_t c0, int32_t c1, int64_t* d_out5);
void halo_counts_async(const int64_t* d_req, const int64_t* d_outer_all, int pitch, int32_t dim, int P, int me, int64_t* d_cnt,
                       int64_t* d_bound);
void halo_bounds_async(const DevMat& A, int32_t c0, const int32_t* d_sa, const int32_t* d_sb, int P, int64_t* d_bound,
                       int64_t* d_cnt_row);

bool spgemm_thin_left(const DevMat& A, const DevMat& B, DevMat& C, double alpha, double threshold, int dense_rule_bits, int64_t* products,
                      hipEvent_t ev_begin, hipEvent_t ev_end);
struct ThinSlabArgs {
  const int32_t *blk_lo = nullptr, *blk_w = nullptr;
  const int64_t* blk_toff = nullptr;
  const int32_t *bfirst = nullptr, *blast = nullptr;
  const int64_t* boff = nullptr;
  const double* bval = nullptr;
  const int32_t *afirst = nullptr, *alast = nullptr;
  const int64_t* aoff = nullptr;
  const double* aval = nullptr;
  const int64_t* at_outer = nullptr;
  const int32_t* at_inner = nullptr;
  const double* at_val = nullptr;
  double* out_val = nullptr;
  int32_t *count = nullptr, *ofirst = nullptr, *olast = nullptr;
  int64_t* ooff = nullptr;
  double alpha = 1.0, threshold = 0.0;
  int dense_rule = 0, ncols = 0, nrows = 0;
  int* flag = nullptr;
  const unsigned long long* aaddr = nullptr;
  int nblocks = 0;
};
void launch_thin_slab(const ThinSlabArgs& a, bool left, bool cplx = false);
struct ThinRows {
  DevBuf<int64_t> outer;
  DevBuf<int32_t> inner;
  DevBuf<double> val;
};
void thin_rows_from_runs(bool cplx, const int32_t* first, const int32_t* last, const unsigned long long* addr, const int64_t* off,
                         const double* base, int32_t ka, int32_t kb, int32_t nrows, int64_t cap, ThinRows& out);
inline int slab_thin_rule(int64_t nnz_a, int64_t nnz_b, int64_t dim) {
  return (nnz_a <= 8 * dim && nnz_b >= nnz_a) ? 1 : (nnz_b <= 8 * dim) ? 2 : 0;
}
long long* thin_slab_counts();
unsigned long long matrix_value_epoch();
void bump_matrix_value_epoch();
bool add_identity_inplace(DevMat& B, double alpha, int32_t c0);
bool norm_axpy_columns(const DevMat& A, const DevMat& B, double alpha, double* norm);
DevMat filter(const DevMat& A, double threshold);
void to_dense(const DevMat& A, double* d_dense, int64_t ld);
DevMat from_dense(const double* d_dense, int64_t ld, int32_t rows, int32_t c0, int32_t cols, bool cplx, double threshold);
void dense_zero_columns(double* d_dense, int64_t ld, int32_t rows, int32_t c_first, int32_t c_end, bool cplx);
void dense_eigh(double* d_A, int32_t n, bool cplx, double* d_W);
void dense_cholesky(const double* d_A, double* d_L, int32_t n, double threshold, int32_t rank);
int64_t exclusive_scan_i64(const int64_t* d_in, int64_t* d_out, int64_t n);
void scan_i32_async(const int32_t* d_in, int64_t* d_out, int64_t n);
void scan_i64_async(const int64_t* d_in, int64_t* d_out, int64_t n);

}
```

### ntpoly_amd/csrc/slab_extra.hip

```cpp
#include <hip/hip_runtime.h>

#include <climits>
#include <cstdio>
#include <cstdlib>
#include <cstring>
#include <memory>

#include "device_util.hpp"
#include "kernels.hpp"

namespace ntp {
namespace {
__global__ __launch_bounds__(256) void k_sa_products(int n, const int32_t* __restrict__ first, const int32_t* __restrict__ last,
                                                     const int64_t* __restrict__ off, const double* __restrict__ val,
                                                     const int32_t* __restrict__ acount, int acols, unsigned long long* __restrict__ out) {
  __shared__ long long red[4];
  const int j = (blockIdx.x * blockDim.x + threadIdx.x) / WAVE;
  long long p = 0;
  if (j < n) {
    const int f = first[j], l = last[j];
    if (l >= f) {
      const double* __restrict__ v = val + (off[j] - f);
      for (int k = f + lane_id(); k <= l; k += WAVE)
        if (v[k] != 0.0 && k < acols) p += acount[k];
    }
  }
  p = wave_sum_i64(p);
  if (lane_id() == 0) red[threadIdx.x / WAVE] = p;
  __syncthreads();
  if (threadIdx.x == 0) {
    const long long t = red[0] + red[1] + red[2] + red[3];
    if (t) atomicAdd(out, (unsigned long long)t);
  }
}
}

namespace {
__global__ __launch_bounds__(256) void k_sa_add_diagonal(int n, const int32_t* __restrict__ first, const int32_t* __restrict__ last,
                                                         const int64_t* __restrict__ off, double* __restrict__ val,
                                                         int32_t* __restrict__ count, int col_offset, double alpha, int apply,
                                                         unsigned long long* __restrict__ st) {
  const int j = blockIdx.x * blockDim.x + threadIdx.x;
  int flag = 0, delta = 0;
  if (j < n) {
    const int d = j + col_offset, f = first[j], l = last[j];
    if (l < f || d < f || d > l) {
      flag = 1;
    } else {
      double* p = val + (off[j] + (d - f));
      const double old = *p;
      const bool hb = old != 0.0;
      const double s = hb ? __dadd_rn(alpha, old) : alpha;
      const bool keep = fabs(s) > 0.0;
      if (!keep && (d == f || d == l)) flag = 2;
      delta = (keep ? 1 : 0) - (hb ? 1 : 0);
      if (apply) {
        *p = keep ? s : 0.0;
        count[j] += delta;
      }
    }
  }
  if (!apply) {
    const unsigned long long any = __ballot(flag != 0);
    if (any) {
      int fl = flag;
      for (int o = 32; o > 0; o >>= 1) fl |= __shfl_xor(fl, o, WAVE);
      if (lane_id() == 0) atomicOr(st, (unsigned long long)fl);
    }
    const long long dsum = wave_sum_i64(delta);
    if (lane_id() == 0 && dsum) atomicAdd(st + 1, (unsigned long long)dsum);
  }
}
}

bool slab_add_diagonal(DevMat& B, double alpha, int32_t col_offset) {
  if (!B.expanded() || B.cplx || (B.rows != B.cols && !slab_panels_ok()) || B.slab->labelled() || B.slab->origin || B.zero_free != 1 || alpha == 0.0) return false;
  SlabForm& f = *B.slab;
  const int n = B.cols;
  DevBuf<unsigned long long> st(2);
  st.zero();
  hipLaunchKernelGGL(k_sa_add_diagonal, dim3(cdiv(n, 256)), dim3(256), 0, stream(), n, f.first.p, f.last.p, f.off.p, f.val.p, f.count.p,
                     col_offset, alpha, 0, st.p);
  unsigned long long h[2] = {0, 0};
  {
    ScalarFetch ft;
    ft.add(st.p, 2, h);
    ft.run();
  }
  if (h[0] != 0) return false;
  hipLaunchKernelGGL(k_sa_add_diagonal, dim3(cdiv(n, 256)), dim3(256), 0, stream(), n, f.first.p, f.last.p, f.off.p, f.val.p, f.count.p,
                     col_offset, alpha, 1, st.p);
  B.nnz += (long long)h[1];
  f.tiles.release();
  f.tile_off.release();
  return true;
}

namespace {
struct Trs4Elem {
  double fx, gx;
};
__device__ inline Trs4Elem trs4_elem(double x, double x2, double d) {
  Trs4Elem e;
  e.fx = __dadd_rn(__dmul_rn(4.0, x), __dmul_rn(-3.0, x2));
  e.gx = __dadd_rn(x2, __dadd_rn(__dmul_rn(-2.0, x), d));
  return e;
}
template <int MODE>
__global__ __launch_bounds__(256) void k_sa_trs4(int n, const int32_t* __restrict__ fa, const int32_t* __restrict__ la,
                                                 const int64_t* __restrict__ offa, const double* __restrict__ va,
                                                 const int32_t* __restrict__ fb, const int32_t* __restrict__ lb,
                                                 const int64_t* __restrict__ offb, const double* __restrict__ vb, int col_offset,
                                                 double sigma, int al, const int64_t* __restrict__ base, double* __restrict__ part,
                                                 double* __restrict__ out, int32_t* __restrict__ ofirst, int32_t* __restrict__ olast,
                                                 int32_t* __restrict__ ocount, int64_t* __restrict__ ooff, int64_t bound,
                                                 unsigned long long* __restrict__ stat) {
  const int j = (blockIdx.x * blockDim.x + threadIdx.x) / WAVE;
  if (j >= n) return;
  const int lane = lane_id();
  const int fA = fa[j], lA = la[j], fB = fb[j], lB = lb[j], dg = j + col_offset;
  const bool anyA = lA >= fA, anyB = lB >= fB;
  int f = dg, l = dg;
  if (anyA) { f = min(f, fA); l = max(l, lA); }
  if (anyB) { f = min(f, fB); l = max(l, lB); }
  const int a0 = f / al * al, a1 = (l / al + 1) * al;
  const double* __restrict__ pa = anyA ? va + (offa[j] - fA) : va;
  const double* __restrict__ pb = anyB ? vb + (offb[j] - fB) : vb;
  if (MODE == 0) {
    double s0 = 0.0, s1 = 0.0;
    for (int r = a0 + lane; r < a1; r += WAVE) {
      const double x = (anyA && r >= fA && r <= lA) ? pa[r] : 0.0;
      const double x2 = (anyB && r >= fB && r <= lB) ? pb[r] : 0.0;
      const Trs4Elem e = trs4_elem(x, x2, r == dg ? 1.0 : 0.0);
      s0 = __dadd_rn(s0, __dmul_rn(x2, e.fx));
      s1 = __dadd_rn(s1, __dmul_rn(x2, e.gx));
    }
    s0 = wave_sum_f64(s0);
    s1 = wave_sum_f64(s1);
    if (lane == 0) { part[2 * (size_t)j] = s0; part[2 * (size_t)j + 1] = s1; }
  } else {
    const int64_t slot = base[j];
    if (slot + (int64_t)(a1 - a0) > bound) {
      if (lane == 0) { ofirst[j] = INT_MAX; olast[j] = -1; ocount[j] = 0; ooff[j] = slot; atomicOr(stat, 2ull); }
      return;
    }
    double* __restrict__ dst = out + (slot - a0);
    int cnt = 0, kf = INT_MAX, kl = -1;
    for (int r = a0 + lane; r < a1; r += WAVE) {
      const double x = (anyA && r >= fA && r <= lA) ? pa[r] : 0.0;
      const double x2 = (anyB && r >= fB && r <= lB) ? pb[r] : 0.0;
      const Trs4Elem e = trs4_elem(x, x2, r == dg ? 1.0 : 0.0);
      const double p = __dadd_rn(e.fx, __dmul_rn(sigma, e.gx));
      const bool keep = p != 0.0;
      dst[r] = keep ? p : 0.0;
      cnt += keep ? 1 : 0;
      kf = min(kf, keep ? r : INT_MAX);
      kl = max(kl, keep ? r : -1);
    }
    cnt = (int)wave_sum_i64(cnt);
    kf = wave_min_i32(kf);
    kl = wave_max_i32(kl);
    if (lane == 0) {
      ofirst[j] = kf; olast[j] = kl; ocount[j] = cnt;
      ooff[j] = slot + (cnt ? kf - a0 : 0);
    }
  }
}
__global__ void k_sa_trs4_span(const int32_t* __restrict__ fa, const int32_t* __restrict__ la, const int32_t* __restrict__ fb,
                               const int32_t* __restrict__ lb, int n, int col_offset, int al, int32_t* __restrict__ span) {
  const int j = blockIdx.x * blockDim.x + threadIdx.x;
  if (j >= n) return;
  int f = j + col_offset, l = j + col_offset;
  if (la[j] >= fa[j]) { f = min(f, fa[j]); l = max(l, la[j]); }
  if (lb[j] >= fb[j]) { f = min(f, fb[j]); l = max(l, lb[j]); }
  span[j] = (l / al + 1) * al - f / al * al;
}
__global__ __launch_bounds__(256) void k_sa_count_sum(const int32_t* __restrict__ v, int n, unsigned long long* __restrict__ out) {
  __shared__ long long red[4];
  long long s = 0;
  for (int i = blockIdx.x * 256 + threadIdx.x; i < n; i += gridDim.x * 256) s += v[i];
  s = wave_sum_i64(s);
  if (lane_id() == 0) red[threadIdx.x / WAVE] = s;
  __syncthreads();
  if (threadIdx.x == 0) {
    const long long t = red[0] + red[1] + red[2] + red[3];
    if (t) atomicAdd(out, (unsigned long long)t);
  }
}
__global__ __launch_bounds__(256) void k_sa_sum_pairs(const double* __restrict__ in, int n, int chunk, double* __restrict__ out) {
  __shared__ double ra[256], rb[256];
  const int lo = blockIdx.x * chunk, hi = min(n, lo + chunk);
  double a = 0.0, b = 0.0;
  for (int i = lo + threadIdx.x; i < hi; i += 256) {
    a = __dadd_rn(a, in[2 * (size_t)i]);
    b = __dadd_rn(b, in[2 * (size_t)i + 1]);
  }
  ra[threadIdx.x] = a;
  rb[threadIdx.x] = b;
  __syncthreads();
  for (int o = 128; o > 0; o >>= 1) {
    if ((int)threadIdx.x < o) {
      ra[threadIdx.x] = __dadd_rn(ra[threadIdx.x], ra[threadIdx.x + o]);
      rb[threadIdx.x] = __dadd_rn(rb[threadIdx.x], rb[threadIdx.x + o]);
    }
    __syncthreads();
  }
  if (threadIdx.x == 0) { out[2 * blockIdx.x] = ra[0]; out[2 * blockIdx.x + 1] = rb[0]; }
}
void sum_pairs_async(const double* part, int n, double* out2) {
  const int chunk = 2048, g = cdiv(n, chunk);
  if (g <= 1) {
    hipLaunchKernelGGL(k_sa_sum_pairs, dim3(1), dim3(256), 0, stream(), part, n, std::max(n, 1), out2);
    return;
  }
  DevBuf<double> lvl((size_t)2 * g);
  hipLaunchKernelGGL(k_sa_sum_pairs, dim3(g), dim3(256), 0, stream(), part, n, chunk, lvl.p);
  hipLaunchKernelGGL(k_sa_sum_pairs, dim3(1), dim3(256), 0, stream(), lvl.p, g, g, out2);
}
bool trs4_operands(const DevMat& X, const DevMat& X2) {
  auto ok = [](const DevMat& M) {
    return M.expanded() && !M.cplx && (M.rows == M.cols || slab_panels_ok()) && !M.slab->labelled() && !M.slab->origin && M.zero_free == 1;
  };
  return ok(X) && ok(X2) && X.cols == X2.cols && X.slab->row_pad == X2.slab->row_pad;
}
}

bool slab_trs4_traces(const DevMat& X, const DevMat& X2, int32_t col_offset, double* trace_fx, double* trace_gx) {
  if (!trs4_operands(X, X2)) return false;
  const SlabForm &fa = *X.slab, &fb = *X2.slab;
  const int n = X.cols;
  DevBuf<double> part((size_t)2 * n), res(2);
  hipLaunchKernelGGL((k_sa_trs4<0>), dim3(cdiv((int64_t)n * WAVE, 256)), dim3(256), 0, stream(), n, fa.first.p, fa.last.p, fa.off.p, fa.val.p,
                     fb.first.p, fb.last.p, fb.off.p, fb.val.p, col_offset, 0.0, std::max(1, fa.row_pad), (const int64_t*)nullptr, part.p,
                     (double*)nullptr, (int32_t*)nullptr, (int32_t*)nullptr, (int32_t*)nullptr, (int64_t*)nullptr, (int64_t)0,
                     (unsigned long long*)nullptr);
  sum_pairs_async(part.p, n, res.p);
  unsigned long long h[2] = {0, 0};
  ScalarFetch ft;
  ft.add(res.p, 2, h);
  ft.run();
  double d[2];
  std::memcpy(d, h, sizeof(h));
  *trace_fx = d[0];
  *trace_gx = d[1];
  return true;
}

// ... 1005 lines not shown
```

### ntpoly_amd/csrc/spgemm_tile.hip

```cpp
#include "spgemm_tile.hpp"
#include <string>

#include <hip/hip_runtime.h>

#include <cstdio>
#include <cstdlib>
#include <vector>

#include "device_util.hpp"
#include "kernels.hpp"

namespace ntp {
namespace {

typedef double v4d __attribute__((ext_vector_type(4)));
typedef double v2d __attribute__((ext_vector_type(2)));
template <int R> struct RowVec;
template <> struct RowVec<1> { typedef double type; };
template <> struct RowVec<2> { typedef v2d type; };
template <> struct RowVec<4> { typedef v4d type; };
template <int R> __device__ inline double rv_get(const typename RowVec<R>::type& x, int m) { return x[m]; }
template <> __device__ inline double rv_get<1>(const double& x, int) { return x; }
template <int R> __device__ inline void rv_set(typename RowVec<R>::type& x, int m, double v) { x[m] = v; }
template <> __device__ inline void rv_set<1>(double& x, int, double v) { x = v; }
template <int R> __device__ inline typename RowVec<R>::type rv_load(unsigned long long addr) {
  return *reinterpret_cast<const typename RowVec<R>::type __attribute__((address_space(1)))*>(addr);
}
template <int R> __device__ inline typename RowVec<R>::type rv_load(const double* p) { return rv_load<R>(reinterpret_cast<unsigned long long>(p)); }
template <int R> __device__ inline void rv_store(double* p, const typename RowVec<R>::type& v) {
  *reinterpret_cast<typename RowVec<R>::type __attribute__((address_space(1)))*>(reinterpret_cast<unsigned long long>(p)) = v;
}

typedef unsigned v4u __attribute__((ext_vector_type(4)));
typedef unsigned v2u __attribute__((ext_vector_type(2)));
constexpr unsigned TILE_OOB = 0xffffff00u;
template <int R> __device__ inline typename RowVec<R>::type rv_buffer_load(__amdgpu_buffer_rsrc_t rsrc, unsigned off);
template <> __device__ inline double rv_buffer_load<1>(__amdgpu_buffer_rsrc_t rsrc, unsigned off) {
  return __builtin_bit_cast(double, __builtin_amdgcn_raw_buffer_load_b64(rsrc, off, 0, 0));
}
template <> __device__ inline v2d rv_buffer_load<2>(__amdgpu_buffer_rsrc_t rsrc, unsigned off) {
  return __builtin_bit_cast(v2d, __builtin_amdgcn_raw_buffer_load_b128(rsrc, off, 0, 0));
}
template <> __device__ inline v4d rv_buffer_load<4>(__amdgpu_buffer_rsrc_t rsrc, unsigned off) {
  const v2d lo = __builtin_bit_cast(v2d, __builtin_amdgcn_raw_buffer_load_b128(rsrc, off, 0, 0));
  const v2d hi = __builtin_bit_cast(v2d, __builtin_amdgcn_raw_buffer_load_b128(rsrc, off + 16u, 0, 0));
  return v4d{lo[0], lo[1], hi[0], hi[1]};
}

struct alignas(16) TileRec {
  unsigned long long rz;
  int32_t first;
  uint32_t span;
};
#ifndef NTP_TILE_PF
#define NTP_TILE_PF 6
#endif
constexpr int TILE_PF = NTP_TILE_PF;
constexpr int TILE_RPAD = 4;
__host__ __device__ constexpr int tile_bp(bool) { return 17; }
__host__ __device__ constexpr int tile_bpad(bool) { return 2; }
struct alignas(16) TileDefer {
  int32_t r, jj, prow, pad;
  double o, d;
};
constexpr int TILE_DEFER = 48;


struct TileArgs {
  const SlabRun* runs;
  const double* bblk;
  const int64_t* blk_boff;
  const int32_t *blk_kmin, *blk_kn, *blk_lo, *blk_w;
  const int64_t* blk_toff;
  double* out_val;
  int32_t* count;
  int32_t *ofirst, *olast;
  int64_t* ooff;
  int64_t* otoff;
  double alpha, threshold;
  int dense_rule, ncols, nblocks;
  int nrows;
  int k4max, tmax;
  SlabFuseArgs fzv;
  const int32_t *brun_first, *brun_last;
  const int64_t* brun_off;
  const double* brun_val;
  int bpair;
  uint32_t bbytes;
  const double* zero;
  const void* abase;
  uint32_t abytes;
  const void* dbase;
  uint32_t dbytes;
  int ablate;
#ifdef NTP_TILE_STAMPS
  long long* stamps;
  long long* blkdur;
#endif
};

__host__ __device__ inline size_t tile_lds_bytes(int k4max, int tmax, int lab_rows = 0) {
  return (size_t)lab_rows * 4 + (size_t)(k4max + tile_bpad(lab_rows > 0)) * tile_bp(lab_rows > 0) * 8 + (size_t)(k4max + TILE_RPAD) * sizeof(TileRec) + (size_t)tmax * 4 + (size_t)(k4max / 4 + 1) * 8 + 16 + TILE_DEFER * sizeof(TileDefer) + 16 * 5 * 4 +
         2 * 8 * 8 + (size_t)tmax * 16 + 8 + (size_t)(k4max + 8) * 4 + 64;
}

#ifdef NTP_TILE_STAMPS
#define STAMP(i) do { if (lane == 0 && b % 97 == 0 && b / 97 < 64 && (i) < 64) a.stamps[((b / 97) * 8 + wave) * 64 + (i)] = __builtin_amdgcn_s_memtime(); } while (0)
#else
#define STAMP(i) do { } while (0)
#endif

template <int EPI, int TILE_NW, int R, bool LAB, bool OFF32>
#ifdef NTP_TILE_WPE3
__global__ __launch_bounds__(TILE_NW* WAVE) __attribute__((amdgpu_waves_per_eu((((EPI == 0 || !LAB) && R <= 2) && TILE_NW != 4) ? 4 : 3, 8))) void k_spgemm_tile(const TileArgs a) {
#else
__global__ __launch_bounds__(TILE_NW* WAVE) __attribute__((amdgpu_waves_per_eu(R <= 2 ? 4 : 3, 8))) void k_spgemm_tile(const TileArgs a) {
#endif
  extern __shared__ __attribute__((aligned(16))) char smem[];
  constexpr bool LABK = LAB && EPI != 0;
  constexpr int BP = tile_bp(LABK), BPAD = tile_bpad(LABK);
  const int b = xcd_block(a.nblocks);
  if (b < 0) return;
  const int tid = threadIdx.x, wave = uni_i32(tid / WAVE), lane = lane_id();
  const int lo = a.blk_lo[b], w = a.blk_w[b], kmin = a.blk_kmin[b], kn = a.blk_kn[b];
  const int64_t tbase = a.blk_toff[b];
  const bool brun = a.brun_val != nullptr;
  int bf0 = INT_MAX, bl0 = -1, bf1 = INT_MAX, bl1 = -1;
  const double *bp0 = nullptr, *bp1 = nullptr;
  unsigned bo0 = 0u, bo1 = 0u;
  auto thread_extents = [&]() {
    const int c0 = b * SLAB_J + 2 * (tid & 7);
    if (c0 < a.ncols) {
      bf0 = a.brun_first[c0]; bl0 = a.brun_last[c0];
      const int64_t o = a.brun_off[c0];
      bp0 = a.brun_val + (o - bf0);
      bo0 = ((unsigned)o - (unsigned)bf0) * 8u;
    }
    if (c0 + 1 < a.ncols) {
      bf1 = a.brun_first[c0 + 1]; bl1 = a.brun_last[c0 + 1];
      const int64_t o = a.brun_off[c0 + 1];
      bp1 = a.brun_val + (o - bf1);
      bo1 = ((unsigned)o - (unsigned)bf1) * 8u;
    }
  };
  constexpr bool PAIR_OK = (TILE_NW == 4 || TILE_NW == 8) && BPAD == 2;
  constexpr int CPW = PAIR_OK ? SLAB_J / TILE_NW : 1;
  [[maybe_unused]] int cbf[CPW], cbl[CPW];
  [[maybe_unused]] unsigned cbo[CPW];
  const bool bpair = PAIR_OK && brun && a.bbytes != 0u && a.bpair != 0;
  if (bpair) {
#pragma unroll
    for (int m = 0; m < CPW; ++m) {
      const int c = b * SLAB_J + CPW * wave + m;
      cbf[m] = INT_MAX; cbl[m] = -1; cbo[m] = 0u;
      if (c < a.ncols) {
        cbf[m] = a.brun_first[c]; cbl[m] = a.brun_last[c];
        cbo[m] = ((unsigned)a.brun_off[c] - (unsigned)cbf[m]) * 8u;
      }
    }
  } else if (brun) thread_extents();
  [[maybe_unused]] int e_raw = 0, e_xpl = -1;
  [[maybe_unused]] int64_t e_raw8 = 0;
  if constexpr (EPI != 0) {
    const int jc0 = min(b * SLAB_J + (tid & 15), a.ncols - 1);
    const int sel = (tid >> 4) & 3;
    if constexpr (EPI == 2) {
      const int32_t* p4 = sel == 0 ? a.fzv.dmin : sel == 1 ? a.fzv.dmax : sel == 2 ? a.fzv.xmin : a.fzv.xmax;
      const int64_t* p8 = (sel & 1) ? a.fzv.xoff : a.fzv.doff;
      e_raw = p4[jc0];
      e_raw8 = p8[jc0];
      if constexpr (LAB) e_xpl = a.fzv.xplast[jc0];
    } else {
      const int32_t* p4 = (sel & 1) ? a.fzv.dmax : a.fzv.dmin;
      e_raw = p4[jc0];
      e_raw8 = a.fzv.doff[jc0];
    }
  }
  if (b == 0 && tid == 0) {
    a.ooff[a.ncols] = a.blk_toff[a.nblocks];
    if (EPI != 0 && a.otoff) a.otoff[a.nblocks] = a.blk_toff[a.nblocks];
  }
  if (kn == 0) {
    const int j = b * SLAB_J + tid;
    if (tid < SLAB_J && j < a.ncols) {
      a.ofirst[j] = INT_MAX;
      a.olast[j] = -1;
      a.count[j] = 0;
      a.ooff[j] = tbase + (int64_t)tid * w;
      if constexpr (EPI != 0) {
        if (a.fzv.oplast) a.fzv.oplast[j] = -1;
        if (EPI == 2 && a.fzv.xmax[j] >= a.fzv.xmin[j]) atomicOr(a.fzv.flag, 1);
      }
    }
    if (EPI != 0 && tid == 0) a.otoff[b] = tbase;
    return;
  }
  STAMP(0);
#ifdef NTP_TILE_STAMPS
  if (tid == 0 && a.blkdur) a.blkdur[4 * b] = __builtin_amdgcn_s_memtime();
#endif
  double* Bs = reinterpret_cast<double*>(smem) + (BPAD / 2) * BP;
  TileRec* recs = reinterpret_cast<TileRec*>(reinterpret_cast<double*>(smem) + (size_t)(a.k4max + BPAD) * BP);
  int* grmin = reinterpret_cast<int*>(recs + a.k4max + TILE_RPAD);
  int* grmax = grmin + (a.k4max / 4 + 1);
  unsigned* colmask = reinterpret_cast<unsigned*>(grmax + (a.k4max / 4 + 1));
  TileDefer* dlist = reinterpret_cast<TileDefer*>(colmask + ((a.tmax + 2 * (a.k4max / 4 + 1) + 3) & ~3) - 2 * (a.k4max / 4 + 1));
  int* col_cnt = reinterpret_cast<int*>(dlist + TILE_DEFER);
  int* col_first = col_cnt + 16;
  int* col_last = col_first + 16;
  int* col_pmax = col_last + 16;
  int* col_plast = col_pmax + 16;
  double* red = reinterpret_cast<double*>(col_plast + 16);
  double* tred = red + 2 * 8;
  int* misc = reinterpret_cast<int*>(tred + 2 * a.tmax);
  [[maybe_unused]] int* cntl = misc + 6 + 1;
  [[maybe_unused]] int* labs = misc + 6 + (a.k4max + 8);

  const int KG = (kn + 3) >> 2, K4 = KG * 4;
  constexpr int TROWS = 16 * R;
  typedef typename RowVec<R>::type VR;
  const int T = (w + TROWS - 1) / TROWS;
  if (kn > 0 && w > 0 && tbase >= 0) STAMP(56);
  constexpr int NT = TILE_NW * WAVE, BCH = 3072 / NT;
  const double2* __restrict__ bsrc = reinterpret_cast<const double2*>(a.bblk + (a.blk_boff ? a.blk_boff[b] : 0));
  double2 btmp[BCH];
  auto brun_load = [&](int i) {
    const int r = kmin + (i >> 3);
    double2 v;
#ifdef NTP_ABL_NOBLOAD
    v.x = (i < kn * 8 && r >= bf0 && r <= bl0) ? 1.0 : 0.0;
    v.y = (i < kn * 8 && r >= bf1 && r <= bl1) ? 1.0 : 0.0;
    return v;
#endif
    v.x = (i < kn * 8 && r >= bf0 && r <= bl0) ? bp0[r] : 0.0;
    v.y = (i < kn * 8 && r >= bf1 && r <= bl1) ? bp1[r] : 0.0;
    return v;
  };
  [[maybe_unused]] int bcnt[BCH];
  [[maybe_unused]] const int32_t* __restrict__ prod_count = nullptr;
  [[maybe_unused]] bool want_prod = false;
  if constexpr (EPI != 0) {
    want_prod = a.fzv.prod != nullptr;
    prod_count = a.fzv.in_count;
  }
#ifndef NTP_TILE_NO_RECFIRST
  constexpr int RCH = (384 + 4 + NT - 1) / NT;
// ... 146 lines not shown
          for (int u = 0; u < CCH; ++u)
            if (tid + u * NT <= K4) cntl[tid + u * NT] = tid + u * NT < K4 ? ctmp[u] : 0;
          if (tid == 0) cntl[-1] = 0;
        }
      }
#pragma unroll
      for (int m = 0; m < CPW; ++m) {
        double* const bcol = Bs + (pair_r - kmin) * BP + CPW * wave + m;
#pragma unroll
        for (int u = 0; u < 3; ++u) {
          if (pair_r - kmin + 128 * u < K4) {
            bcol[128 * u * BP] = btmp[m * 3 + u].x;
            bcol[(128 * u + 1) * BP] = btmp[m * 3 + u].y;
          }
          if constexpr (EPI != 0)
            nzm |= ((btmp[m * 3 + u].x != 0.0) ? 1u : 0u) << (2 * (m * 3 + u)) | ((btmp[m * 3 + u].y != 0.0) ? 2u : 0u) << (2 * (m * 3 + u));
        }
      }
    }
  }
  else {
#pragma unroll
    for (int u = 0; u < BCH; ++u) {
      const int i = tid + u * NT;
      if (i < K4 * 8) { Bs[(i >> 3) * BP + 2 * (i & 7)] = btmp[u].x; Bs[(i >> 3) * BP + 2 * (i & 7) + 1] = btmp[u].y; }
      if constexpr (EPI != 0) prod_p += (long long)(((btmp[u].x != 0.0) ? 1 : 0) + ((btmp[u].y != 0.0) ? 1 : 0)) * bcnt[u];
    }
  }
  for (int i = tid + BCH * NT; i < K4 * 8; i += NT) {
    const double2 v = brun ? brun_load(i) : (i < kn * 8 ? bsrc[i] : make_double2(0.0, 0.0));
    Bs[(i >> 3) * BP + 2 * (i & 7)] = v.x;
    Bs[(i >> 3) * BP + 2 * (i & 7) + 1] = v.y;
    if constexpr (EPI != 0) {
      if (want_prod && i < kn * 8)
        prod_p += (long long)(((v.x != 0.0) ? 1 : 0) + ((v.y != 0.0) ? 1 : 0)) * (prod_count ? prod_count[kmin + (i >> 3)] : 1);
    }
  }
  STAMP(61);
  if constexpr (LAB) {
#pragma unroll
    for (int u = 0; u < LABCH; ++u)
      if (tid + u * NT < T * TROWS) labs[tid + u * NT] = labtmp[u];
  }
  for (int t = tid; t < T; t += NT) {
    colmask[t] = 0u;
    if constexpr (EPI != 0) { tred[2 * t] = 0.0; tred[2 * t + 1] = 0.0; }
  }
  if (tid < 16) {
    col_cnt[tid] = 0;
    col_first[tid] = INT_MAX;
    col_last[tid] = -1;
    col_pmax[tid] = -1;
    col_plast[tid] = -1;
  }
  if (tid < 6) misc[tid] = 0;
  __syncthreads();
  STAMP(62);
  STAMP(63);
  if constexpr (EPI != 0) {
    if (want_prod) {
      if constexpr (PAIR_OK) {
        if (bpath == 2) {
#pragma unroll
          for (int u = 0; u < 3; ++u) {
            const int rho = pair_r - kmin + 128 * u;
            const int c0 = cntl[min(rho, K4)], c1 = cntl[min(rho + 1, K4)];
#pragma unroll
            for (int m = 0; m < CPW; ++m)
              prod_p += (long long)(((nzm >> (2 * (m * 3 + u))) & 1u) ? c0 : 0) + (long long)(((nzm >> (2 * (m * 3 + u) + 1)) & 1u) ? c1 : 0);
          }
        }
      }
      prod_p = wave_sum_i64(prod_p);
      if (lane == 0 && prod_p) atomicAdd(reinterpret_cast<unsigned long long*>(misc + 2), (unsigned long long)prod_p);
    }
  }
  if constexpr (LAB) {
    const int32_t* __restrict__ lab_g = a.fzv.lab;
    for (int i = tid + LABCH * NT; i < T * TROWS; i += NT) labs[i] = lab_g[min(lo + i, a.nrows - 1)];
    __syncthreads();
  }
  STAMP(1);

  const int jj = lane & 15, q = lane >> 4;
  const int j = b * SLAB_J + jj;
  const bool colv = j < a.ncols;
  const int jc = min(j, a.ncols - 1);
  const double* const zp = a.zero;
  const unsigned long long zaddr = reinterpret_cast<unsigned long long>(zp);
  double* const orun = a.out_val + (tbase + (int64_t)jj * w - lo);
  [[maybe_unused]] double* otile = nullptr;
  [[maybe_unused]] int xf = INT_MAX, xlrow = -1, xpl = -1, df = INT_MAX, dl = -1;
  [[maybe_unused]] const double *xrz = zp, *drz = zp;
  [[maybe_unused]] double am = 0, bm = 0, thr_m = 0;
  [[maybe_unused]] int diag = -1;
  if constexpr (EPI != 0) {
    if (a.fzv.tiles) otile = a.fzv.tiles + (tbase - (int64_t)lo * SLAB_J + jj);
    const int pj = 4 * jj;
    auto pull64 = [&](int from, int64_t v) {
      const int lo32 = __builtin_amdgcn_ds_bpermute(from, (int)(unsigned)(unsigned long long)v);
      const int hi32 = __builtin_amdgcn_ds_bpermute(from, (int)(unsigned)((unsigned long long)v >> 32));
      return (int64_t)(((unsigned long long)(unsigned)hi32 << 32) | (unsigned long long)(unsigned)lo32);
    };
    const int e_d0 = __builtin_amdgcn_ds_bpermute(pj, e_raw), e_d1 = __builtin_amdgcn_ds_bpermute(pj + 64, e_raw);
    const int64_t e_doff = EPI == 2 ? pull64(pj, e_raw8) : e_raw8;
    const int d0 = e_d0, d1 = e_d1;
    if (colv && d1 >= d0) {
      df = d0;
      dl = d1;
      drz = a.fzv.dexp + (e_doff - d0);
    }
    diag = j + a.fzv.col_offset;
    if constexpr (EPI == 2) {
      am = a.fzv.am; bm = a.fzv.bm; thr_m = a.fzv.thr_m;
      const int e_x0 = __builtin_amdgcn_ds_bpermute(pj + 128, e_raw), e_x1 = __builtin_amdgcn_ds_bpermute(pj + 192, e_raw);
      const int64_t e_xoff = pull64(pj + 64, e_raw8);
      const int x0 = e_x0, x1 = e_x1;
      if (colv && x1 >= x0) {
        xf = x0;
        xlrow = x1;
        xrz = a.fzv.xexp + (e_xoff - x0);
        xpl = LAB ? e_xpl : x1;
        if (x0 < lo || x1 >= lo + w) atomicOr(a.fzv.flag, 1);
      }
    }
  }
  [[maybe_unused]] unsigned xo0 = 0, xsp = 0, do0 = 0, dsp = 0;
  [[maybe_unused]] int xf1 = INT_MAX, df1 = INT_MAX;
  [[maybe_unused]] __amdgpu_buffer_rsrc_t xrsrc, drsrc;
  if constexpr (OFF32 && EPI != 0) {
    drsrc = __builtin_amdgcn_make_buffer_rsrc(const_cast<void*>(a.dbase), 0, a.dbytes, 0x00020000);
    if (dl >= df) {
      df1 = df - (R - 1);
      dsp = (unsigned)(dl - df + (R - 1));
      do0 = (unsigned)(reinterpret_cast<unsigned long long>(drz) - reinterpret_cast<unsigned long long>(a.dbase));
    }
    if constexpr (EPI == 2) {
      xrsrc = __builtin_amdgcn_make_buffer_rsrc(const_cast<void*>(a.abase), 0, a.abytes, 0x00020000);
      if (xlrow >= xf) {
        xf1 = xf - (R - 1);
        xsp = (unsigned)(xlrow - xf + (R - 1));
        xo0 = (unsigned)(reinterpret_cast<unsigned long long>(xrz) - reinterpret_cast<unsigned long long>(a.abase));
      }
    }
  }
  const double alpha = a.alpha, thr = a.threshold;
  const bool dense_rule = (a.dense_rule & 1) != 0;
  double dsum = 0.0, tsum = 0.0;
  int pn = 0;
  const int rend = lo + w;
  const int mid = (T - 1) >> 1;

  [[maybe_unused]] int sidx = 4;
#ifdef NTP_TILE_STATIC
  for (int ti = 0;; ++ti) {
    const int ts = ti * TILE_NW + ((ti & 1) ? TILE_NW - 1 - wave : wave);
    if (ti * TILE_NW >= T) break;
    if (ts >= T) continue;
#else
  for (;;) {
    int ts = 0;
    if (lane == 0) ts = atomicAdd(&misc[4], 1);
    ts = __builtin_amdgcn_readfirstlane(ts);
    if (ts >= T) break;
    if constexpr (EPI != 0) { dsum = 0.0; tsum = 0.0; }
#endif
    STAMP(sidx); ++sidx;
    const int t = (ts & 1) ? mid + ((ts + 1) >> 1) : mid - (ts >> 1);
    const int r0 = lo + TROWS * t;
    int g0 = INT_MAX, g1 = -1;
    for (int c = 0; c < KG; c += WAVE) {
      const int gq = min(c + lane, KG);
      const unsigned long long m = __ballot(grmin[gq] <= r0 + TROWS - 1 && grmax[gq] >= r0);
      if (m) {
        if (g0 == INT_MAX) g0 = c + (int)__builtin_ctzll(m);
        g1 = c + 63 - (int)__builtin_clzll(m);
      }
    }
    [[maybe_unused]] VR xv[4], dv[4];
    auto epilogue_loads = [&]() {
#pragma unroll
      for (int v = 0; v < 4; ++v) {
        const int rb = r0 + R * (4 * v + q);
        if constexpr (OFF32) {
          if constexpr (EPI == 2) xv[v] = rv_buffer_load<R>(xrsrc, (unsigned)(rb - xf1) <= xsp ? xo0 + (unsigned)rb * 8u : TILE_OOB);
          if constexpr (EPI != 0) dv[v] = rv_buffer_load<R>(drsrc, (unsigned)(rb - df1) <= dsp ? do0 + (unsigned)rb * 8u : TILE_OOB);
        } else {
          if constexpr (EPI == 2) xv[v] = rv_load<R>(((rb + R - 1 >= xf) & (rb <= xlrow)) ? xrz + rb : zp);
          if constexpr (EPI != 0) {
            dv[v] = rv_load<R>(((rb + R - 1 >= df) & (rb <= dl)) ? drz + rb : zp);
          }
        }
      }
    };
    v4d acc[R];
#pragma unroll
    for (int m = 0; m < R; ++m) acc[m] = v4d{0.0, 0.0, 0.0, 0.0};
    if (g1 >= g0) {
      const int rl = r0 + R * jj;
      [[maybe_unused]] const unsigned long long r8 = (unsigned long long)((long long)rl * 8);
      const uint4* __restrict__ rq = reinterpret_cast<const uint4*>(recs) + q;
      const double* __restrict__ bq = Bs + q * BP + jj;
#ifdef NTP_TILE_ABL_NOLOAD
      const unsigned long long abl_base = reinterpret_cast<unsigned long long>(a.out_val) & ~0x3fffull;
#endif
#ifdef NTP_ABLATIONS
      const unsigned long long abl_base = reinterpret_cast<unsigned long long>(a.out_val) & ~0x3fffull;
#endif
      [[maybe_unused]] const unsigned r8lo = (unsigned)rl * 8u;
      [[maybe_unused]] __amdgpu_buffer_rsrc_t arsrc;
      if constexpr (OFF32) arsrc = __builtin_amdgcn_make_buffer_rsrc(const_cast<void*>(a.abase), 0, a.abytes, 0x00020000);
      auto run_load = [&](const uint4 raw) -> VR {
        const bool ok = (unsigned)(rl - (int)raw.z) <= raw.w;
        if constexpr (OFF32) {
          return rv_buffer_load<R>(arsrc, ok ? raw.x + r8lo : TILE_OOB);
        } else {
          const unsigned long long rz = (unsigned long long)raw.x | ((unsigned long long)raw.y << 32);
#ifdef NTP_ABLATIONS
          if (a.ablate == 1) return rv_load<R>(ok ? abl_base + ((rz + r8 - abl_base) & 0x3fe0ull) : zaddr);
#endif
          return rv_load<R>(ok ? rz + r8 : zaddr);
        }
      };
      auto gi = [&](int x) { return OFF32 ? x : min(x, KG); };
      auto bi = [&](int x) { return OFF32 ? x : min(x, KG - 1); };
      VR ring[TILE_PF];
      double bb[3];
#pragma unroll
      for (int u = 0; u < TILE_PF; ++u) ring[u] = run_load(rq[4 * gi(g0 + u)]);
      bb[0] = bq[4 * BP * g0];
      bb[1] = bq[4 * BP * bi(g0 + 1)];
      bb[2] = 0.0;
      uint4 raw = rq[4 * gi(g0 + TILE_PF)];
      int g = g0;
      STAMP(sidx);
      for (; g + TILE_PF - 1 <= g1; g += TILE_PF) {
#pragma unroll
        for (int u = 0; u < TILE_PF; ++u) {
          const uint4 raw_n = rq[4 * gi(g + u + TILE_PF + 1)];
          __builtin_amdgcn_sched_barrier(0);
#pragma unroll
          for (int m = 0; m < R; ++m) acc[m] = __builtin_amdgcn_mfma_f64_16x16x4f64(rv_get<R>(ring[u], m), bb[u % 3], acc[m], 0, 0, 0);
          __builtin_amdgcn_sched_barrier(0);
          ring[u] = run_load(raw);
          bb[(u + 2) % 3] = bq[4 * BP * bi(g + u + 2)];
          raw = raw_n;
          __builtin_amdgcn_sched_barrier(0);
        }
      }
      epilogue_loads();
#pragma unroll
      for (int u = 0; u < TILE_PF - 1; ++u) {
        if (g + u <= g1) {
          const double bt = bq[4 * BP * (g + u)];
#pragma unroll
          for (int m = 0; m < R; ++m) acc[m] = __builtin_amdgcn_mfma_f64_16x16x4f64(rv_get<R>(ring[u], m), bt, acc[m], 0, 0, 0);
        }
      }
    }
    else epilogue_loads();
    ++sidx; STAMP(sidx); ++sidx;
#ifdef NTP_ABLATIONS
    if (a.ablate == 2) {
      if (acc[0][0] == 1.2345e300) colmask[t] = 1u;
      continue;
    }
#endif
    {
      bool live = false;
#pragma unroll
      for (int v = 0; v < 4; ++v) {
#pragma unroll
        for (int m = 0; m < R; ++m) {
          const double vv = acc[m][v];
          live |= dense_rule ? (fabs(vv) > thr) : (fabs(__dmul_rn(alpha, vv)) > thr);
          if constexpr (EPI == 2) live |= rv_get<R>(xv[v], m) != 0.0;
        }
      }
      if (__ballot(live) == 0ull) {
        if (lane == 0) colmask[t] = 0u;
        STAMP(sidx); ++sidx;
        continue;
      }
    }
#ifndef NTP_TILE_NO_FULL_TILES
    if constexpr (EPI == 2 && !LAB) {
      bool full = true;
      VR both[4];
#pragma unroll
      for (int v = 0; v < 4; ++v) {
#pragma unroll
        for (int m = 0; m < R; ++m) {
          const double vv = acc[m][v];
          const double sv = __dmul_rn(alpha, vv);
          const double bv = rv_get<R>(xv[v], m);
          const double bo = __dadd_rn(__dmul_rn(am, sv), __dmul_rn(bm, bv));
          full &= (dense_rule ? (fabs(vv) > thr) : (fabs(sv) > thr)) & (bv != 0.0) & (fabs(bo) > thr_m);
          rv_set<R>(both[v], m, bo);
        }
      }
      if (__ballot(!full) == 0ull) {
        pn += 64 * 4 * R;
        const bool has_diag = r0 <= b * SLAB_J + SLAB_J - 1 + a.fzv.col_offset && r0 + TROWS - 1 >= b * SLAB_J + a.fzv.col_offset;
#pragma unroll
        for (int v = 0; v < 4; ++v) {
#pragma unroll
          for (int m = 0; m < R; ++m) {
            const double o = rv_get<R>(both[v], m);
            dsum = __dadd_rn(dsum, __dmul_rn(o, rv_get<R>(dv[v], m)));
            if (has_diag) tsum = __dadd_rn(tsum, (r0 + R * (4 * v + q) + m == diag) ? o : 0.0);
          }
        }
        if (q == 0) {
          atomicAdd(&col_cnt[jj], TROWS);
          atomicMin(&col_first[jj], r0);
          atomicMax(&col_last[jj], r0 + TROWS - 1);
          atomicMax(&col_pmax[jj], r0 + TROWS - 1);
        }
#pragma unroll
        for (int v = 0; v < 4; ++v) rv_store<R>(orun + (r0 + R * (4 * v + q)), both[v]);
        if (otile) {
#pragma unroll
          for (int v = 0; v < 4; ++v) {
#pragma unroll
            for (int m = 0; m < R; ++m) otile[(int64_t)(r0 + R * (4 * v + q) + m) * SLAB_J] = rv_get<R>(both[v], m);
          }
        }
        if (lane == 0) colmask[t] = 0xffffu;
#ifndef NTP_TILE_STATIC
        {
          const double td = wave_sum_f64(dsum), tt = wave_sum_f64(tsum);
          if (lane == 0) {
            tred[2 * t] = td;
            tred[2 * t + 1] = tt;
          }
        }
#endif
        STAMP(sidx); ++sidx;
        continue;
      }
    }
#endif
    VR res[4];
    unsigned long long anykeep = 0;
    int c_l = 0, f_l = INT_MAX, l_l = -1, pm_l = -1, pl_l = -1;
#pragma unroll
    for (int v = 0; v < 4; ++v) {
#pragma unroll
      for (int m = 0; m < R; ++m) {
        const int r = r0 + R * (4 * v + q) + m;
        const double vv = acc[m][v];
        const double sv = __dmul_rn(alpha, vv);
        const bool ha = dense_rule ? (fabs(vv) > thr) : (fabs(sv) > thr);
        bool keep;
        double o;
        [[maybe_unused]] double dval = 0.0;
        [[maybe_unused]] int pr = r;
        if constexpr (EPI != 0) {
          dval = rv_get<R>(dv[v], m);
          if constexpr (LAB) pr = labs[r - lo];
        }
        if constexpr (EPI != 2) {
          keep = ha;
          o = sv;
        } else {
          const double bv = rv_get<R>(xv[v], m);
          const bool hb = bv != 0.0;
          const double bs = __dmul_rn(bm, bv);
          const double wa = __dmul_rn(am, sv);
          const double both = __dadd_rn(wa, bs);
          o = ha ? (hb ? both : wa) : bs;
          const bool big = fabs(o) > thr_m;
          if (ha) {
            keep = (!hb && pr > xpl) || big;
          } else {
            keep = hb && big;
            if (hb && !big) {
              const int slot = atomicAdd(&misc[0], 1);
              if (slot < TILE_DEFER) {
                *reinterpret_cast<int4*>(&dlist[slot]) = make_int4(r, jj, pr, 0);
                dlist[slot].o = o;
                dlist[slot].d = dval;
              }
            }
          }
        }
        pn += (int)__popcll(__ballot(ha));
        anykeep |= __ballot(keep);
        if constexpr (EPI != 0) {
          dsum = __dadd_rn(dsum, __dmul_rn(keep ? o : 0.0, keep ? dval : 0.0));
          tsum = __dadd_rn(tsum, (keep && r == diag) ? o : 0.0);
          pm_l = max(pm_l, ha ? pr : -1);
          pl_l = max(pl_l, keep ? pr : -1);
        }
        c_l += keep ? 1 : 0;
        f_l = min(f_l, keep ? r : INT_MAX);
        l_l = max(l_l, keep ? r : -1);
        rv_set<R>(res[v], m, keep ? o : 0.0);
      }
    }
    const unsigned cm = (unsigned)((anykeep | (anykeep >> 16) | (anykeep >> 32) | (anykeep >> 48)) & 0xffffull);
    if (c_l) {
      atomicAdd(&col_cnt[jj], c_l);
      atomicMin(&col_first[jj], f_l);
      atomicMax(&col_last[jj], l_l);
      if constexpr (EPI != 0) {
        if constexpr (LAB) atomicMax(&col_plast[jj], pl_l);
      }
    }
    if constexpr (EPI == 2) {
      if (pm_l >= 0) atomicMax(&col_pmax[jj], pm_l);
    }
    if ((cm >> jj) & 1u) {
#pragma unroll
      for (int v = 0; v < 4; ++v) rv_store<R>(orun + (r0 + R * (4 * v + q)), res[v]);
    }
    if constexpr (EPI != 0) {
      if (cm && otile) {
#pragma unroll
        for (int v = 0; v < 4; ++v) {
#pragma unroll
          for (int m = 0; m < R; ++m) otile[(int64_t)(r0 + R * (4 * v + q) + m) * SLAB_J] = rv_get<R>(res[v], m);
        }
      }
    }
    if (lane == 0) colmask[t] = cm;
#ifndef NTP_TILE_STATIC
    if constexpr (EPI != 0) {
      const double td = wave_sum_f64(dsum), tt = wave_sum_f64(tsum);
      if (lane == 0) {
        tred[2 * t] = td;
        tred[2 * t + 1] = tt;
      }
    }
#endif
    STAMP(sidx); ++sidx;
  }
  STAMP(2);
#ifdef NTP_TILE_STATIC
  if constexpr (EPI != 0) {
    dsum = wave_sum_f64(dsum);
    tsum = wave_sum_f64(tsum);
    if (lane == 0) {
      red[2 * wave] = dsum;
      red[2 * wave + 1] = tsum;
    }
  }
#endif
  if (lane == 0 && pn) atomicAdd(&misc[1], pn);
  __syncthreads();
  STAMP(3);
  if constexpr (EPI == 2) {
    const int nd = misc[0];
    if (nd != 0) {
    if (nd > TILE_DEFER) {
      if (tid == 0) atomicOr(a.fzv.flag, 1);
    } else {
      for (int i = tid; i < nd; i += TILE_NW * WAVE) {
        const int4 e = *reinterpret_cast<const int4*>(&dlist[i]);
        const bool kept = e.z > col_pmax[e.y];
        if (kept) {
          atomicAdd(&col_cnt[e.y], 1);
          atomicMin(&col_first[e.y], e.x);
          atomicMax(&col_last[e.y], e.x);
          if constexpr (LAB) atomicMax(&col_plast[e.y], e.z);
        }
        dlist[i].pad = kept ? 1 : 0;
      }
    }
    __syncthreads();
    if (nd <= TILE_DEFER && tid < nd) {
      const TileDefer e = dlist[tid];
      if (e.pad) {
        int rank = 0;
        for (int m2 = 0; m2 < nd; ++m2) {
          const TileDefer f = dlist[m2];
          rank += (f.pad && (f.r < e.r || (f.r == e.r && f.jj < e.jj))) ? 1 : 0;
        }
        Bs[rank] = __dmul_rn(e.o, e.d);
        Bs[TILE_DEFER + rank] = (e.r == b * SLAB_J + e.jj + a.fzv.col_offset) ? e.o : 0.0;
      }
    }
    __syncthreads();
    }
  }
  if (tid < SLAB_J) {
    const int jt = b * SLAB_J + tid;
    const int cf = col_first[tid], cl = col_last[tid];
    if (jt < a.ncols) {
      a.count[jt] = col_cnt[tid];
      a.ofirst[jt] = cf;
      a.olast[jt] = cl;
      a.ooff[jt] = tbase + (int64_t)tid * w + (cl >= cf ? cf - lo : 0);
      if constexpr (EPI != 0) {
        if constexpr (LAB) a.fzv.oplast[jt] = col_plast[tid];
      }
    }
  }
  int tk0 = INT_MAX, tk1 = -1;
#pragma unroll
  for (int c = 0; c < SLAB_J; ++c) {
    tk0 = min(tk0, col_first[c]);
    tk1 = max(tk1, col_last[c]);
  }
  if constexpr (EPI != 0) {
    if (tid == 0) {
      a.otoff[b] = tbase + (tk1 >= tk0 ? (int64_t)(tk0 - lo) * SLAB_J : 0);
      a.fzv.pnnz[b] = misc[1];
      if (a.fzv.prod) a.fzv.prod[b] = *reinterpret_cast<long long*>(misc + 2);
    }
    if (tid == 64) {
      double x = 0.0, y = 0.0;
#ifdef NTP_TILE_STATIC
      for (int qq = 0; qq < TILE_NW; ++qq) {
        x = __dadd_rn(x, red[2 * qq]);
        y = __dadd_rn(y, red[2 * qq + 1]);
      }
#else
      for (int t2 = 0; t2 < T; ++t2) {
        x = __dadd_rn(x, tred[2 * t2]);
        y = __dadd_rn(y, tred[2 * t2 + 1]);
      }
#endif
      if constexpr (EPI == 2) {
        const int nd = min(misc[0], TILE_DEFER);
        int nk = 0;
        for (int m2 = 0; m2 < nd; ++m2) nk += dlist[m2].pad;
        for (int m2 = 0; m2 < nk; ++m2) {
          x = __dadd_rn(x, Bs[m2]);
          y = __dadd_rn(y, Bs[TILE_DEFER + m2]);
        }
      }
      a.fzv.part[2 * b] = x;
      a.fzv.part[2 * b + 1] = y;
    }
  }
  for (int p = tid; p < T * SLAB_J; p += TILE_NW * WAVE) {
    const int t = p >> 4, c = p & 15;
    const unsigned cmk = colmask[t];
    const int cf = col_first[c], cl = col_last[c];
    const int r0 = lo + TROWS * t;
    if (cl >= cf && r0 + TROWS - 1 >= cf && r0 <= cl && !((cmk >> c) & 1u)) {
      double* dst = a.out_val + (tbase + (int64_t)c * w - lo);
      for (int r = r0; r < min(r0 + TROWS, rend); ++r) dst[r] = 0.0;
    }
    if constexpr (EPI != 0) {
      if (a.fzv.tiles && tk1 >= tk0 && r0 + TROWS - 1 >= tk0 && r0 <= tk1 && cmk == 0u) {
        double* dst = a.fzv.tiles + (tbase - (int64_t)lo * SLAB_J + c);
        for (int r = r0; r < min(r0 + TROWS, rend); ++r) dst[(int64_t)r * SLAB_J] = 0.0;
      }
    }
  }
  if constexpr (EPI == 2) {
    const int nd = min(misc[0], TILE_DEFER);
    if (nd > 0) {
      __syncthreads();
      for (int i = tid; i < nd; i += TILE_NW * WAVE) {
        const TileDefer e = dlist[i];
        if (!e.pad) continue;
        a.out_val[tbase + (int64_t)e.jj * w + (e.r - lo)] = e.o;
        if (a.fzv.tiles) a.fzv.tiles[tbase + (int64_t)(e.r - lo) * SLAB_J + e.jj] = e.o;
      }
    }
  }
  STAMP(55);
#ifdef NTP_TILE_STAMPS
  if (tid == 0 && a.blkdur) {
    a.blkdur[4 * b + 1] = __builtin_amdgcn_s_memtime();
    a.blkdur[4 * b + 2] = EPI == 2 ? misc[0] : 0;
    a.blkdur[4 * b + 3] = kn;
  }
#endif
}

}

#ifndef NTP_WITH_TILE2
bool launch_spgemm_tile2(const TileLaunch&, int*) { return false; }
#endif

int tile_rows() {
  const int r = options().tile_rows;
  return r == 4 ? 4 : r == 1 ? 1 : 2;
}

bool spgemm_tile_fits(int max_kn, int max_w) {
  const int k4 = std::max(8, (max_kn + 3) & ~3), tm = (max_w + 15) >> 4;
  return max_kn > 0 && max_w > 0 && std::max(tile_lds_bytes(k4, tm, 16 * tm + 64), tile_lds_bytes(k4, tm, 0)) <= 150 * 1024;
}

void launch_spgemm_tile(const TileLaunch& L) {
  TileArgs a;
  a.runs = static_cast<const SlabRun*>(L.runs);
  a.bblk = L.bblk; a.blk_boff = L.blk_boff; a.blk_kmin = L.blk_kmin; a.blk_kn = L.blk_kn; a.blk_lo = L.blk_lo; a.blk_w = L.blk_w;
  a.blk_toff = L.blk_toff; a.out_val = L.out_val; a.count = L.count; a.ofirst = L.ofirst; a.olast = L.olast; a.ooff = L.ooff;
  a.otoff = L.otoff; a.alpha = L.alpha; a.threshold = L.threshold; a.dense_rule = L.dense_rule; a.ncols = L.ncols;
  a.nblocks = L.nblocks;
  a.nrows = L.nrows > 0 ? L.nrows : L.ncols;
  a.k4max = std::max(8, (L.max_kn + 3) & ~3);
  const int trows = 16 * (L.rows == 4 ? 4 : L.rows == 2 ? 2 : 1);
  a.tmax = (L.max_w + trows - 1) / trows;
  if (L.fz) a.fzv = *static_cast<const SlabFuseArgs*>(L.fz);
  a.brun_first = L.brun_first; a.brun_last = L.brun_last; a.brun_off = L.brun_off; a.brun_val = L.brun_val;
  a.bbytes = (options().tile_bbuf != 0 && L.brun_val && L.bbytes > 0 && L.bbytes < 0xffffe000ull) ? (uint32_t)L.bbytes : 0u;
  a.bpair = (a.bbytes != 0u && options().tile_bbuf >= 2 && L.brun_pad >= 2 && L.brun_pad % 2 == 0) ? 1 : 0;
  static DevBuf<double>* zeros = nullptr;
  if (!zeros) {
    zeros = new DevBuf<double>(8);
    zeros->zero();
  }
  a.zero = zeros->p;
  bool off32 = options().tile_off32 != 0 && L.abase != nullptr && L.abytes > 0 && L.abytes < 0xfffff000ull;
  if (off32 && L.epi != 0) {
    const SlabFuseArgs& fzh = *static_cast<const SlabFuseArgs*>(L.fz);
    const char *a0 = static_cast<const char*>(L.abase), *x0 = reinterpret_cast<const char*>(fzh.xexp);
    off32 = L.dbase != nullptr && L.dbytes > 0 && L.dbytes < 0xfffff000ull && (L.epi != 2 || (x0 >= a0 && x0 < a0 + L.abytes));
  }
  a.abase = off32 ? L.abase : nullptr;
  a.abytes = off32 ? (uint32_t)L.abytes : 0u;
  a.dbase = off32 ? L.dbase : nullptr;
  a.dbytes = off32 ? (uint32_t)L.dbytes : 0u;
  a.ablate = options().spgemm_variant == 601 ? 1 : options().spgemm_variant == 602 ? 2 : 0;
#ifdef NTP_TILE_STAMPS
  static DevBuf<long long>* stamps = nullptr;
  if (!stamps) stamps = new DevBuf<long long>(64 * 8 * 64);
  stamps->zero();
  a.stamps = stamps->p;
  static DevBuf<long long>* blkdur = nullptr;
  if (!blkdur || blkdur->n < (size_t)4 * L.nblocks) { delete blkdur; blkdur = new DevBuf<long long>((size_t)4 * L.nblocks); }
  blkdur->zero();
  a.blkdur = blkdur->p;
#endif
  const size_t lds = tile_lds_bytes(a.k4max, a.tmax, (L.labelled && L.epi != 0) ? a.tmax * trows : 0);
#ifdef NTP_TILE_WIDE3
  const bool wide = 3 * ((lds + 511) & ~(size_t)511) > 160 * 1024;
#else
  const bool wide = 4 * ((lds + 511) & ~(size_t)511) > 160 * 1024;
#endif
  const int tw = options().tile_waves;
  const int nw = (tw == 4 || tw == 5 || tw == 6 || tw == 8) ? tw : (wide ? 8 : 4);
  auto go = [&](auto epi_tag, auto nw_tag, auto r_tag, auto lab_tag, auto off_tag) {
    constexpr int E = decltype(epi_tag)::value, NW = decltype(nw_tag)::value, RR = decltype(r_tag)::value;
    constexpr bool LB = decltype(lab_tag)::value, OF = decltype(off_tag)::value;
    static size_t raised = 0;
    if (lds > 64 * 1024 && lds > raised) {
      HIP_CHECK(hipFuncSetAttribute(reinterpret_cast<const void*>(&k_spgemm_tile<E, NW, RR, LB, OF>), hipFuncAttributeMaxDynamicSharedMemorySize,
                                    150 * 1024));
      raised = 150 * 1024;
    }
    hipLaunchKernelGGL((k_spgemm_tile<E, NW, RR, LB, OF>), dim3(xcd_grid(L.nblocks)), dim3(NW * WAVE), lds, stream(), a);
  };
  auto by_off = [&](auto epi_tag, auto nw_tag, auto r_tag, auto lab_tag) {
    constexpr int NW = decltype(nw_tag)::value, RR = decltype(r_tag)::value;
    if constexpr ((NW == 4 || NW == 8) && RR <= 2) {
      if (off32) return go(epi_tag, nw_tag, r_tag, lab_tag, std::true_type{});
    }
    go(epi_tag, nw_tag, r_tag, lab_tag, std::false_type{});
  };
  auto by_nw = [&](auto epi_tag, auto r_tag, auto lab_tag) {
    if (nw == 4) by_off(epi_tag, std::integral_constant<int, 4>{}, r_tag, lab_tag);
    else if (nw == 5) by_off(epi_tag, std::integral_constant<int, 5>{}, r_tag, lab_tag);
    else if (nw == 6) by_off(epi_tag, std::integral_constant<int, 6>{}, r_tag, lab_tag);
    else by_off(epi_tag, std::integral_constant<int, 8>{}, r_tag, lab_tag);
  };
  auto by_r = [&](auto epi_tag) {
    constexpr int E = decltype(epi_tag)::value;
    using F = std::false_type; using T = std::true_type;
    using R1 = std::integral_constant<int, 1>; using R2 = std::integral_constant<int, 2>; using R4 = std::integral_constant<int, 4>;
    if constexpr (E != 0) {
      if (L.labelled) {
        if (L.rows >= 2) by_nw(epi_tag, R2{}, T{});
        else by_nw(epi_tag, R1{}, T{});
        return;
      }
    }
    if (L.rows == 4) by_nw(epi_tag, R4{}, F{});
    else if (L.rows == 2) by_nw(epi_tag, R2{}, F{});
    else by_nw(epi_tag, R1{}, F{});
  };
  if (L.epi == 0) by_r(std::integral_constant<int, 0>{});
  else if (L.epi == 1) by_r(std::integral_constant<int, 1>{});
  else by_r(std::integral_constant<int, 2>{});
#ifdef NTP_TILE_STAMPS
  if (const char* f = std::getenv("NTP_TILE_STAMPS_FILE")) {
    std::vector<long long> h(64 * 8 * 64);
    HIP_CHECK(hipStreamSynchronize(stream()));
    HIP_CHECK(hipMemcpy(h.data(), stamps->p, h.size() * 8, hipMemcpyDeviceToHost));
    if (FILE* fp = std::fopen(f, "wb")) { std::fwrite(h.data(), 8, h.size(), fp); std::fclose(fp); }
    std::vector<long long> hb((size_t)4 * L.nblocks);
    HIP_CHECK(hipMemcpy(hb.data(), blkdur->p, hb.size() * 8, hipMemcpyDeviceToHost));
    if (FILE* fp = std::fopen((std::string(f) + ".blocks").c_str(), "wb")) { std::fwrite(hb.data(), 8, hb.size(), fp); std::fclose(fp); }
  }
#endif
}

}
```

### ntpoly_amd/csrc/spgemm_tile.hpp

```cpp
#pragma once
#include "slab_types.hpp"

namespace ntp {

struct TileLaunch {
  const void* runs = nullptr;
  const double* bblk = nullptr;
  const int64_t* blk_boff = nullptr;
  const int32_t *blk_kmin = nullptr, *blk_kn = nullptr, *blk_lo = nullptr, *blk_w = nullptr;
  const int64_t* blk_toff = nullptr;
  double* out_val = nullptr;
  int32_t* count = nullptr;
  int32_t *ofirst = nullptr, *olast = nullptr;
  int64_t* ooff = nullptr;
  int64_t* otoff = nullptr;
  double alpha = 1.0, threshold = 0.0;
  int dense_rule = 0, ncols = 0, nblocks = 0;
  int max_kn = 0, max_w = 0;
  int epi = 0;
  int rows = 1;
  const void* fz = nullptr;
  const int32_t *brun_first = nullptr, *brun_last = nullptr;
  const int64_t* brun_off = nullptr;
  const double* brun_val = nullptr;
  size_t bbytes = 0;
  int brun_pad = 1;
  const void* abase = nullptr;
  size_t abytes = 0;
  const void* dbase = nullptr;
  size_t dbytes = 0;
  int nrows = 0;
  bool labelled = false;
};
bool spgemm_tile_fits(int max_kn, int max_w);
int tile_rows();
inline int tile_expand_align() { return 16 * tile_rows(); }
void launch_spgemm_tile(const TileLaunch& a);
bool launch_spgemm_tile2(const TileLaunch& a, int* fail);
bool spgemm_tile_c_fits(int max_kn, int max_w);
void launch_spgemm_tile_c(const TileLaunch& a);

}
```

### ntpoly_amd/csrc/wrp.cpp

```cpp
#include <algorithm>
#include <cmath>
#include <cstring>

#include "engine.hpp"
#include "spgemm_block.hpp"
#include "io.hpp"

using namespace ntp;

namespace {
constexpr int SIZE_wrp = 12;

template <typename T>
T* get(const int* ih) {
  T* p;
  std::memcpy(&p, ih, sizeof(p));
  if (!p) NTP_FATAL("null handle passed to the C ABI");
  return p;
}
PSMatrix* get_unpacked(const int* ih) {
  PSMatrix* p;
  std::memcpy(&p, ih, sizeof(p));
  if (!p) NTP_FATAL("null handle passed to the C ABI");
  return p;
}
template <>
PSMatrix* get<PSMatrix>(const int* ih) {
  PSMatrix* p = get_unpacked(ih);
  if (p->loc.loose() || p->loc.expanded() || p->loc.blocked()) pack(p->loc);
  return p;
}
struct ApiSession {
  CommScope cs;
  SlabSession s;
  explicit ApiSession(const int* ih_first) : cs(get_unpacked(ih_first)->grid), s(true, true) {}
  PSMatrix* mat(const int* ih) const { return s.opened ? get_unpacked(ih) : get<PSMatrix>(ih); }
};
template <typename T>
void put(int* ih, T* p) {
  std::memset(ih, 0, sizeof(int) * SIZE_wrp);
  std::memcpy(ih, &p, sizeof(p));
}

struct Pool {
  int dummy = 0;
};
struct LocalMat {
  DevMat m;
};

const ProcessGrid* default_grid() {
  if (!global_grid_constructed()) NTP_FATAL("the global process grid has not been constructed");
  return &global_grid();
}
std::string fstring(const char* s, const int* n) { return std::string(s, (size_t)*n); }

void local_diagonal_scale(DevMat& m, const HostTriplets& t) {
  if (m.cols == 0) return;
  const size_t w = m.wval();
  std::vector<double> f((size_t)m.cols * w, 0.0);
  for (int32_t j = 0; j < m.cols; ++j) f[(size_t)j * w] = 1.0;
  for (size_t i = 0; i < t.size(); ++i) {
    const int32_t col = t.col[i] - 1;
    if (col < 0 || col >= m.cols) continue;
    const double re = t.cplx ? t.val[2 * i] : t.val[i], im = t.cplx ? t.val[2 * i + 1] : 0.0;
    double& fr = f[(size_t)col * w];
    if (m.cplx) {
      double& fi = f[(size_t)col * w + 1];
      const double nr = fr * re - fi * im, ni = fr * im + fi * re;
      fr = nr;
      fi = ni;
    } else {
      fr *= re;
    }
  }
  DevBuf<double> d(f.size());
  d.upload(f.data(), f.size());
  scale_columns(m, d.p);
  sync_stream();
}
void local_print(const DevMat& m, const char* path) {
  HostTriplets t;
  to_triplets(m, 0, t);
  FILE* f = path ? std::fopen(path, "w") : stdout;
  if (!f) NTP_FATAL(std::string("cannot open ") + path + " for writing");
  std::fprintf(f, "%%%%MatrixMarket matrix coordinate %s general\n%%\n", m.cplx ? "complex" : "real");
  std::fprintf(f, "%d %d %lld\n", m.rows, m.cols, (long long)m.nnz);
  for (size_t i = 0; i < t.size(); ++i) {
    if (m.cplx) std::fprintf(f, "%d %d %.17g %.17g\n", t.row[i], t.col[i], t.val[2 * i], t.val[2 * i + 1]);
    else std::fprintf(f, "%d %d %.17g\n", t.row[i], t.col[i], t.val[i]);
  }
  if (path) std::fclose(f);
  else std::fflush(f);
}
std::unique_ptr<SlabSession> g_test_session;
}

extern "C" {

void ntpoly_amd_get_unique_id(char* out128) { comm_get_unique_id(out128); }
void ntpoly_amd_init_comm(const char* id128, const int* rank, const int* nranks) { comm_init(id128, *rank, *nranks); }
void ntpoly_amd_finalize_comm() { comm_finalize(); }
int ntpoly_amd_comm_rank() { return base_world().rank; }
int ntpoly_amd_comm_size() { return base_world().nranks; }
void ntpoly_amd_barrier() { comm_barrier(); }
void ntpoly_amd_allreduce_max(double* values, const int* n) { comm_allreduce_max(values, *n); }
void ntpoly_amd_synchronize() {
  ensure_init();
  sync_stream();
  HIP_CHECK(hipDeviceSynchronize());
}
int ntpoly_amd_device_count() {
  int n = 0;
  if (hipGetDeviceCount(&n) != hipSuccess) return 0;
  return n;
}
void ntpoly_amd_panel_range(const int* dim, const int* nranks, const int* rank, int* c0, int* c1) {
  panel_range(*dim, *nranks, *rank, c0, c1);
}
void ntpoly_amd_halo_segment(const int* dim, const int* nranks, const int* s, const int* kmin, const int* kmax, int* a,
                             int* b) {
  halo_segment(*dim, *nranks, *s, *kmin, *kmax, a, b);
}
void ntpoly_amd_panel_exchange_layout(const int* dim, const int* nranks, const int* me, const long long* req, const long long* cnt,
                                      int* sa, int* sb, long long* soff, int* ra, int* rb, long long* zoff) {
  panel_exchange_layout(*dim, *nranks, *me, reinterpret_cast<const int64_t*>(req), reinterpret_cast<const int64_t*>(cnt), sa, sb,
                        reinterpret_cast<int64_t*>(soff), ra, rb, reinterpret_cast<int64_t*>(zoff));
}
void ntpoly_amd_set_option(const char* name, const int* value) {
  const std::string n(name);
  if (n == "spgemm_force_bin") options().spgemm_force_bin = *value;
  else if (n == "increment_force_seq") options().increment_force_seq = *value;
  else if (n == "spgemm_fma") options().spgemm_fma = *value;
  else if (n == "plan_ahead") options().plan_ahead = *value;
  else if (n == "slab_algebra") options().slab_algebra = *value;
  else if (n == "operand_cache") options().operand_cache = *value;
  else if (n == "tile_rows") options().tile_rows = *value;
  else if (n == "tile_waves") options().tile_waves = *value;
  else if (n == "time_kernels") options().time_kernels = *value;
  else if (n == "spgemm_variant") options().spgemm_variant = *value;
  else if (n == "halo_overlap") options().halo_overlap = *value;
  else if (n == "load_balance") options().load_balance = *value;
  else if (n == "virtual_grid") options().virtual_grid = *value;
  else if (n == "loose_iterates") options().loose_iterates = *value;
  else if (n == "fused_update") options().fused_update = *value;
  else if (n == "label_order") options().label_order = *value;
  else if (n == "band_scope") options().band_scope = *value;
  else if (n == "exchange_ahead") options().exchange_ahead = *value;
  else if (n == "plan_fused") options().plan_fused = *value;
  else if (n == "tile_off32") options().tile_off32 = *value;
  else if (n == "tile_bbuf") options().tile_bbuf = *value;
  else if (n == "ghash_mfma") options().ghash_mfma = *value;
  else if (n == "ghash_mfma_complex") options().ghash_mfma_complex = *value;
  else if (n == "block_unfused") options().block_unfused = *value;
  else if (n == "block_match") options().block_match = *value;
  else if (n == "block_scope") options().block_scope = *value;
  else if (n == "block_scope_complex") options().block_scope_complex = *value;
  else if (n == "panel_sessions") options().panel_sessions = *value;
  else if (n == "complex_panels") options().complex_panels = *value;
  else if (n == "complex_density") options().complex_density = *value;
  else if (n == "label_rowoff") options().label_rowoff = *value;
  else if (n == "block_path") options().block_path = *value;
  else if (n == "tile_runs_only") options().tile_runs_only = *value;
  else if (n == "tile2") options().tile2 = *value;
  else if (n == "complex_tile") options().complex_tile = *value;
  else if (n == "block_complex") options().block_complex = *value;
  else if (n == "thin_left") options().thin_left = *value;
  else if (n == "thin_slab_complex") options().thin_slab_complex = *value;
  else if (n == "complex_poly_sessions") options().complex_poly_sessions = *value;
  else if (n == "stored_zero_views") options().stored_zero_views = *value;
  else if (n == "pm_session") options().pm_session = *value;
  else if (n == "isr_chain") options().isr_chain = *value;
  else if (n == "column_fused") options().column_fused = *value;
  else if (n == "complex_sessions") options().complex_sessions = *value;
  else NTP_FATAL("unknown option " + n);
}
int ntpoly_amd_get_option(const char* name) {
  const std::string n(name);
  if (n == "spgemm_fma") return options().spgemm_fma;
  if (n == "slab_algebra") return options().slab_algebra;
  if (n == "plan_ahead") return options().plan_ahead;
  if (n == "tile_rows") return options().tile_rows;
  if (n == "tile2") return options().tile2;
  if (n == "block_path") return options().block_path;
  if (n == "label_order") return options().label_order;
  if (n == "band_scope") return options().band_scope;
  if (n == "exchange_ahead") return options().exchange_ahead;
  if (n == "plan_fused") return options().plan_fused;
  if (n == "tile_off32") return options().tile_off32;
  if (n == "tile_bbuf") return options().tile_bbuf;
  if (n == "ghash_mfma") return options().ghash_mfma;
  if (n == "ghash_mfma_complex") return options().ghash_mfma_complex;
  if (n == "block_unfused") return options().block_unfused;
  if (n == "block_match") return options().block_match;
  if (n == "block_scope") return options().block_scope;
  if (n == "block_scope_complex") return options().block_scope_complex;
  if (n == "panel_sessions") return options().panel_sessions;
  if (n == "complex_panels") return options().complex_panels;
  if (n == "complex_density") return options().complex_density;
  if (n == "fused_update") return options().fused_update;
  if (n == "loose_iterates") return options().loose_iterates;
  if (n == "complex_tile") return options().complex_tile;
  if (n == "block_complex") return options().block_complex;
  if (n == "thin_left") return options().thin_left;
  if (n == "thin_slab_complex") return options().thin_slab_complex;
  if (n == "complex_poly_sessions") return options().complex_poly_sessions;
  if (n == "stored_zero_views") return options().stored_zero_views;
  if (n == "pm_session") return options().pm_session;
  if (n == "isr_chain") return options().isr_chain;
  if (n == "column_fused") return options().column_fused;
  if (n == "complex_sessions") return options().complex_sessions;
  NTP_FATAL("unknown option " + n);
}
void ntpoly_amd_last_spgemm_stats(long long* out, float* ms_numeric, float* ms_total) {
  flush_spgemm_timers();
  const SpgemmStats& s = last_spgemm_stats();
  out[0] = s.nnz_a; out[1] = s.nnz_b; out[2] = s.nnz_c; out[3] = s.products; out[4] = s.tmp_entries;
  for (int i = 0; i < 6; ++i) out[5 + i] = s.bin_cols[i];
  out[11] = s.overflow_cols;
  out[12] = s.slab;
  *ms_numeric = s.ms_numeric;
  *ms_total = s.ms_total;
}
void ntpoly_amd_last_grouped_stats(long long* out, double* ratio) {
  const SpgemmStats& s = last_spgemm_stats();
  out[0] = s.grouped; out[1] = s.gh_failed_cols; out[2] = s.gh_groups; out[3] = s.gh_level; out[4] = s.gh_minhash;
  out[5] = s.gh_tile_rows;
  *ratio = s.gh_union_ratio;
}
void ntpoly_amd_ghash_class_counts(long long out[4]) {
  for (int q = 0; q < 4; ++q) out[q] = ghash_class_counts()[q];
}
void ntpoly_amd_drop_grouped_caches() { drop_grouped_caches(); }
int ntpoly_amd_last_spgemm_thin() { return last_spgemm_stats().thin; }
void ntpoly_amd_thin_slab_counts(long long* out) {
  for (int q = 0; q < 6; ++q) out[q] = thin_slab_counts()[q];
}
void ntpoly_amd_session_begin(const int* complex_ok) {
  if (g_test_session) NTP_FATAL("ntpoly_amd_session_begin: a session is already open");
  g_test_session.reset(new SlabSession(true, false, *complex_ok != 0));
}
void ntpoly_amd_session_end() { g_test_session.reset(); }
int ntpoly_amd_recurrence_step(const int* ih_P, const int* ih_Tkm2, int* ih_Tk, int* ih_R, const double* a, const double* c) {
  return ps_recurrence_step(*get_unpacked(ih_P), *get_unpacked(ih_Tkm2), *get_unpacked(ih_Tk), *get_unpacked(ih_R), *a, *c) ? 1 : 0;
}
void ntpoly_amd_isr_chain_counts(long long out[3]) {
  for (int q = 0; q < 3; ++q) out[q] = isr_chain_counts()[q];
}
int ntpoly_amd_isr_chain_step(const int* ih_X, const int* ih_X2, const int* order, const double* a, const double* b, const double* c,
                              int* ih_Out1, int* ih_Out2) {
  return ps_isr_chain_step(*get_unpacked(ih_X), *get_unpacked(ih_X2), *order, *a, *b, *c, *get_unpacked(ih_Out1), *get_unpacked(ih_Out2)) ? 1 : 0;
}
void ntpoly_amd_pm_session_counts(long long out[4]) {
  for (int q = 0; q < 4; ++q) out[q] = pm_session_counts()[q];
}
void ntpoly_amd_pm_session_longest_list(long long* out) { *out = pm_session_counts()[4]; }
int ntpoly_amd_pm_fused_step(const int* ih_X, const int* ih_Z, const int* ih_X2, const int* ih_X3, const double* a1, const double* a2,
                             const double* a3, const double* thr, int* ih_Out, int* ih_Zout, double* sc) {
  const PSMatrix &X = *get<PSMatrix>(ih_X), &Z = *get<PSMatrix>(ih_Z), &X2 = *get<PSMatrix>(ih_X2), &X3 = *get<PSMatrix>(ih_X3);
  PSMatrix &Out = *get<PSMatrix>(ih_Out), &Zout = *get<PSMatrix>(ih_Zout);
  CommScope cs(X.grid);
  if (world().active() || X.cplx || Z.cplx || X2.cplx || X3.cplx || X.dim != Z.dim || X.dim != X2.dim || X.dim != X3.dim) return 0;
  DevMat x = X.loc.clone(), x2 = X2.loc.clone(), x3 = X3.loc.clone();
  if (!slab_enter(x) || !slab_enter(x2) || !slab_enter(x3)) return 0;
  ZeroList zl, zn;
  zero_list_from_pattern(Z.loc, zl);
  DevMat R;
  double t[2] = {0.0, 0.0};
  if (!slab_pm_sigma(x, zl, x2, *thr, X.c0, t) || !slab_pm_update(x, zl, x2, x3, *a1, *a2, *a3, *thr, R, zn)) return 0;
  sc[0] = t[0];
  sc[1] = t[1];
  pack(R);
  for (PSMatrix* m : {&Out, &Zout}) { m->grid = X.grid; m->dim = X.dim; m->cplx = false; m->c0 = X.c0; m->c1 = X.c1; }
  Out.loc = std::move(R);
  Zout.loc = zero_list_matrix(zn, X.loc.rows, X.loc.cols);
  return 1;
}
void ntpoly_amd_recurrence_step_count(long long* out) { *out = recurrence_step_count(); }
void ntpoly_amd_last_block_stats(long long* out, double* fill) {
  const SpgemmStats& s = last_spgemm_stats();
  out[0] = s.block; out[1] = s.block_tile_products; out[2] = s.block_cand;
  *fill = s.block_fill;
}
int ntpoly_amd_block_order(const int* ih, int* position) {
  PSMatrix& m = *get<PSMatrix>(ih);
  std::vector<int32_t> pos;
  if (!block_order_for(m.loc, pos)) return 0;
  std::memcpy(position, pos.data(), sizeof(int32_t) * pos.size());
  return 1;
}
void ntpoly_amd_drop_block_caches() { drop_block_caches(); }
int ntpoly_amd_block_order_of_pattern(const int* ih, int* position, int* ns) {
  PSMatrix& m = *get<PSMatrix>(ih);
  DevMat full = ps_gather_full(m);
  std::vector<int32_t> pos;
  int32_t s = 0;
  if (!block_order_of_pattern(full, pos, &s)) return 0;
  std::memcpy(position, pos.data(), sizeof(int32_t) * pos.size());
  *ns = s;
  return 1;
}
void ntpoly_amd_exchange_stats(long long* out) {
  out[0] = exchange_stats().exchanges;
  out[1] = exchange_stats().host_syncs;
  out[2] = host_sync_count();
}
int ntpoly_amd_band_order(const int* ih, int* newpos, long long* bandwidth) {
  PSMatrix& m = *get<PSMatrix>(ih);
  DevBuf<int32_t> pos;
  int64_t bw = 0;
  if (!find_band_order(m.loc, pos, &bw)) return 0;
  HIP_CHECK(hipMemcpyAsync(newpos, pos.p, sizeof(int32_t) * (size_t)m.loc.cols, hipMemcpyDeviceToHost, stream()));
  sync_stream();
  *bandwidth = bw;
  return 1;
}
void ntpoly_amd_fusion_counts(long long* out) {
  for (int q = 0; q < 3; ++q) out[q] = fusion_counts()[q];
}
void ntpoly_amd_complex_fusion_counts(long long* out) {
  for (int q = 0; q < 3; ++q) out[q] = complex_fusion_counts()[q];
}
void ntpoly_amd_tile2_counts(long long* out) {
  for (int q = 0; q < 2; ++q) out[q] = tile2_counts()[q];
}
void ntpoly_amd_gather_matrix_to_process(const int* ih_this, int* ih_local, const int* within_slice_id) {
  const PSMatrix& m = *get<PSMatrix>(ih_this);
  DevMat full = ps_gather_full(m);
  const ProcessGrid& g = m.grid ? *m.grid : global_grid();
  const int slice_size = g.num_rows * g.num_cols;
  const int in_slice = g.global_rank - slice_size * g.my_slice;
  if (*within_slice_id >= 0 && *within_slice_id != in_slice) return;
  auto* L = new LocalMat();
  L->m = std::move(full);
  put(ih_local, L);
}
void ntpoly_amd_comm_split_matrix(const int* ih_this, int* ih_split, int* my_color, bool* split_slice) {
  const PSMatrix& m = *get<PSMatrix>(ih_this);
  if (!m.grid) NTP_FATAL("CommSplitMatrix of a matrix that was never constructed");
  auto* out = new PSMatrix();
  ps_comm_split(m, *out, my_color, split_slice);
  put(ih_split, out);
}
void ntpoly_amd_split_process_grid(const int* ih_old_grid, int* ih_new_grid, int* my_color, bool* split_slice) {
  put(ih_new_grid, split_process_grid(*get<ProcessGrid>(ih_old_grid), my_color, split_slice));
}
void ntpoly_amd_grid_comm_info(const int* ih_grid, int* out) {
  const ProcessGrid* g = get<ProcessGrid>(ih_grid);
  out[0] = g->global_rank;
  out[1] = g->total;
  out[2] = g->comm != nullptr ? 1 : 0;
}
void ntpoly_amd_band_scope_counts(long long* out) {
  for (int q = 0; q < 2; ++q) out[q] = band_scope_counts()[q];
}
void ntpoly_amd_block_scope_counts(long long* out) {
  out[0] = band_scope_counts()[2];
  out[1] = block_scope_products();
}
void ntpoly_amd_column_fused_counts(long long* out) {
  out[0] = column_fused_counts()[0];
  out[1] = column_fused_counts()[1];
}
void ntpoly_amd_increment_identity(const int* ih_identity, int* ih_matB, const double* alpha) {
  ps_increment_identity(*get<PSMatrix>(ih_identity), *get<PSMatrix>(ih_matB), *alpha);
}
int ntpoly_amd_norm_axpby(const int* ih_matA, const int* ih_matB, const double* alpha, const double* beta, double* norm) {
  return ps_norm_axpby(*get<PSMatrix>(ih_matA), *get<PSMatrix>(ih_matB), *alpha, *beta, norm) ? 1 : 0;
}
void ntpoly_amd_block_algebra_counts(long long* out) {
  out[0] = block_algebra_counts()[0];
  out[1] = block_algebra_counts()[1];
}
void ntpoly_amd_slab_algebra_counts(long long* out) {
  for (int q = 0; q < 4; ++q) out[q] = slab_algebra_counts()[q];
}
void ntpoly_amd_slab_view_counts(long long out[4]) {
  for (int q = 0; q < 4; ++q) out[q] = slab_view_counts()[q];
}
void ntpoly_amd_panel_product_counts(long long* out) {
  out[0] = panel_product_counts()[0];
  out[1] = panel_product_counts()[1];
  out[2] = panel_product_counts()[2];
}
void ntpoly_amd_band_searches(long long* out) { *out = band_searches(); }
void ntpoly_amd_reset_spgemm_accum() {
  flush_spgemm_timers();
  spgemm_accum() = SpgemmAccum();
}
void ntpoly_amd_get_spgemm_accum(long long* out, double* dout) {
  flush_spgemm_timers();
  const SpgemmAccum& a = spgemm_accum();
  out[0] = a.calls; out[1] = a.products; out[2] = a.nnz_c;
  dout[0] = a.alg_bytes; dout[1] = a.ms_numeric; dout[2] = a.ms_total;
}
int ntpoly_amd_trace_iterations() { return last_trace().iterations; }
void ntpoly_amd_trace_get(double* value, double* energy, double* sigma, long long* nnz) {
  const SolverTrace& t = last_trace();
  for (int i = 0; i < t.iterations; ++i) {
    value[i] = t.value[(size_t)i];
    energy[i] = t.energy[(size_t)i];
    sigma[i] = t.sigma[(size_t)i];
    nnz[i] = t.nnz[(size_t)i];
  }
}
void ntpoly_amd_trace_times(double* setup_ms, double* loop_ms) {
  *setup_ms = last_trace().setup_ms;
  *loop_ms = last_trace().loop_ms;
}
void ntpoly_amd_memory(long long* in_use, long long* cached) {
  *in_use = (long long)dev_bytes_in_use();
  *cached = (long long)dev_bytes_cached();
}
void ntpoly_amd_release_cache() {
  drop_operand_caches();
  dev_release_cache();
}
void ntpoly_amd_malloc_stats(long long* calls, double* ms) { dev_malloc_stats(calls, ms); }
void ntpoly_amd_triplets_set_r(int* ih_list, const long long* n, const int* col, const int* row, const double* val) {
  HostTriplets* t = get<HostTriplets>(ih_list);
  t->cplx = false;
  t->col.assign(col, col + *n);
  t->row.assign(row, row + *n);
  t->val.assign(val, val + *n);
}
void ntpoly_amd_triplets_set_c(int* ih_list, const long long* n, const int* col, const int* row, const double* val_ri) {
  HostTriplets* t = get<HostTriplets>(ih_list);
  t->cplx = true;
  t->col.assign(col, col + *n);
  t->row.assign(row, row + *n);
  t->val.assign(val_ri, val_ri + 2 * *n);
}
void ntpoly_amd_triplets_get(const int* ih_list, int* col, int* row, double* val) {
  const HostTriplets* t = get<HostTriplets>(ih_list);
  std::copy(t->col.begin(), t->col.end(), col);
  std::copy(t->row.begin(), t->row.end(), row);
  std::copy(t->val.begin(), t->val.end(), val);
}

void ConstructGlobalProcessGrid_wrp(const int* world_comm, const int* process_rows, const int* process_columns,
                                    const int* process_slices) {
  comm_bind_mpi(*world_comm);
  construct_grid(global_grid(), *process_rows, *process_columns, *process_slices, base_world());
}
void ConstructGlobalProcessGrid_onlyslice_wrp(const int* world_comm, const int* process_slices) {
  comm_bind_mpi(*world_comm);
  construct_grid_default(global_grid(), *process_slices, base_world());
}
void ConstructGlobalProcessGrid_default_wrp(const int* world_comm) {
  comm_bind_mpi(*world_comm);
  construct_grid_default(global_grid(), 1, base_world());
}
void CopyProcessGrid_wrp(const int* ih_old_grid, int* ih_new_grid) {
  put(ih_new_grid, new ProcessGrid(*get<ProcessGrid>(ih_old_grid)));
}
int GetGlobalMySlice_wrp() { return global_grid().my_slice; }
int GetGlobalMyColumn_wrp() { return global_grid().my_col; }
int GetGlobalMyRow_wrp() { return global_grid().my_row; }
bool GetGlobalIsRoot_wrp() { return global_grid().is_root(); }
int GetGlobalNumSlices_wrp() { return global_grid().num_slices; }
int GetGlobalNumColumns_wrp() { return global_grid().num_cols; }
int GetGlobalNumRows_wrp() { return global_grid().num_rows; }
void WriteGlobalProcessGridInfo_wrp() { write_grid_info(global_grid()); }
void DestructGlobalProcessGrid_wrp() {}
void ConstructProcessGrid_wrp(int* ih_grid, const int* world_comm, const int* process_rows, const int* process_columns,
                              const int* process_slices) {
  comm_bind_mpi(*world_comm);
  ProcessGrid* g = new ProcessGrid();
  construct_grid(*g, *process_rows, *process_columns, *process_slices, base_world());
  put(ih_grid, g);
}
void ConstructProcessGrid_onlyslice_wrp(int* ih_grid, const int* world_comm, const int* process_slices) {
  comm_bind_mpi(*world_comm);
  ProcessGrid* g = new ProcessGrid();
  construct_grid_default(*g, *process_slices, base_world());
  put(ih_grid, g);
}
void ConstructProcessGrid_default_wrp(int* ih_grid, const int* world_comm) {
  comm_bind_mpi(*world_comm);
  ProcessGrid* g = new ProcessGrid();
  construct_grid_default(*g, 1, base_world());
  put(ih_grid, g);
}
int GetMySlice_wrp(const int* ih_grid) { return get<ProcessGrid>(ih_grid)->my_slice; }
int GetMyColumn_wrp(const int* ih_grid) { return get<ProcessGrid>(ih_grid)->my_col; }
int GetMyRow_wrp(const int* ih_grid) { return get<ProcessGrid>(ih_grid)->my_row; }
int GetNumSlices_wrp(const int* ih_grid) { return get<ProcessGrid>(ih_grid)->num_slices; }
int GetNumColumns_wrp(const int* ih_grid) { return get<ProcessGrid>(ih_grid)->num_cols; }
int GetNumRows_wrp(const int* ih_grid) { return get<ProcessGrid>(ih_grid)->num_rows; }
void WriteProcessGridInfo_wrp(const int* ih_grid) { write_grid_info(*get<ProcessGrid>(ih_grid)); }
void DestructProcessGrid_wrp(int* ih_grid) { delete get<ProcessGrid>(ih_grid); }

void ConstructTripletList_r_wrp(int* ih_this, const int* size) {
  HostTriplets* t = new HostTriplets();
  t->cplx = false;
  t->col.assign((size_t)*size, 0);
  t->row.assign((size_t)*size, 0);
  t->val.assign((size_t)*size, 0.0);
  put(ih_this, t);
}
void ResizeTripletList_r_wrp(int* ih_this, const int* size) {
  HostTriplets* t = get<HostTriplets>(ih_this);
  t->col.resize((size_t)*size);
  t->row.resize((size_t)*size);
  t->val.resize((size_t)*size);
}
void AppendToTripletList_r_wrp(int* ih_this, const int* index_column, const int* index_row, const double* point_value) {
  HostTriplets* t = get<HostTriplets>(ih_this);
  t->col.push_back(*index_column);
  t->row.push_back(*index_row);
  t->val.push_back(*point_value);
}
void SetTripletAt_r_wrp(int* ih_this, const int* index, const int* index_column, const int* index_row,
                        const double* point_value) {
  HostTriplets* t = get<HostTriplets>(ih_this);
  const size_t i = (size_t)*index - 1;
  t->col[i] = *index_column;
  t->row[i] = *index_row;
  t->val[i] = *point_value;
}
void GetTripletAt_r_wrp(const int* ih_this, const int* index, int* index_column, int* index_row, double* point_value) {
  const HostTriplets* t = get<HostTriplets>(ih_this);
  const size_t i = (size_t)*index - 1;
  *index_column = t->col[i];
  *index_row = t->row[i];
  *point_value = t->val[i];
}
void DestructTripletList_r_wrp(int* ih_this) { delete get<HostTriplets>(ih_this); }
static void sort_triplets(const HostTriplets& in, HostTriplets& out) {
  const size_t n = in.size(), w = in.cplx ? 2 : 1;
  std::vector<size_t> order(n);
  for (size_t i = 0; i < n; ++i) order[i] = i;
  std::stable_sort(order.begin(), order.end(), [&](size_t a, size_t b) {
    if (in.col[a] != in.col[b]) return in.col[a] < in.col[b];
    return in.row[a] < in.row[b];
  });
  out.cplx = in.cplx;
  out.col.resize(n);
  out.row.resize(n);
  out.val.resize(n * w);
  for (size_t i = 0; i < n; ++i) {
// ... 684 lines not shown
```

### ntpoly_amd/host.py

```python
import contextlib
import ctypes as C

import numpy as np

from . import capi
from .capi import b, d, handle, i, lib, ll, s


def ConstructGlobalProcessGrid(process_rows=None, process_columns=None, process_slices=None, world_comm=0):
    if process_rows is None and process_slices is None:
        lib.ConstructGlobalProcessGrid_default_wrp(i(world_comm))
    elif process_rows is None:
        lib.ConstructGlobalProcessGrid_onlyslice_wrp(i(world_comm), i(process_slices))
    else:
        lib.ConstructGlobalProcessGrid_wrp(i(world_comm), i(process_rows), i(process_columns), i(process_slices))


def WriteGridInfo():
    lib.WriteGlobalProcessGridInfo_wrp()


def DestructGlobalProcessGrid():
    lib.DestructGlobalProcessGrid_wrp()

# ... 688 lines not shown
    @staticmethod
    def ReduceDimension(AMat, dim, RMat, solver_parameters):
        lib.ReduceDimension_wrp(AMat.ih, i(dim), RMat.ih, solver_parameters.ih)


class GeometryOptimization:
    @staticmethod
    def PurificationExtrapolate(PreviousDensity, Overlap, trace, NewDensity, solver_parameters):
        lib.PurificationExtrapolate_wrp(PreviousDensity.ih, Overlap.ih, d(trace), NewDensity.ih, solver_parameters.ih)

    @staticmethod
    def LowdinExtrapolate(PreviousDensity, OldOverlap, NewOverlap, NewDensity, solver_parameters):
        lib.LowdinExtrapolate_wrp(PreviousDensity.ih, OldOverlap.ih, NewOverlap.ih, NewDensity.ih, solver_parameters.ih)


class MatrixConversion:
    @staticmethod
    def SnapMatrixToSparsityPattern(mat, pattern):
        lib.SnapMatrixToSparsityPattern_wrp(mat.ih, pattern.ih)


class EigenSolvers:
    @staticmethod
    def EigenDecomposition(matrix, eigenvalues, nvals, eigenvectors, solver_parameters):
        lib.EigenDecomposition_wrp(matrix.ih, eigenvalues.ih, i(nvals), eigenvectors.ih, solver_parameters.ih)

    @staticmethod
    def EigenValues(matrix, eigenvalues, nvals, solver_parameters):
        lib.EigenDecomposition_novec_wrp(matrix.ih, eigenvalues.ih, i(nvals), solver_parameters.ih)

    @staticmethod
    def SingularValueDecomposition(matrix, leftvectors, rightvectors, singularvalues, solver_parameters):
        lib.SingularValueDecompostion_wrp(matrix.ih, leftvectors.ih, rightvectors.ih, singularvalues.ih,
                                          solver_parameters.ih)

    @staticmethod
    def EstimateGap(H, K, chemical_potential, solver_parameters):
        gap = C.c_double()
        lib.EstimateGap_wrp(H.ih, K.ih, d(chemical_potential), C.byref(gap), solver_parameters.ih)
        return gap.value


class FermiOperator:
    @staticmethod
    def ComputeDenseFOE(H, ISQ, trace, Density, inv_temp, solver_parameters):
        e, mu = C.c_double(), C.c_double()
        lib.ComputeDenseFOE_wrp(H.ih, ISQ.ih, d(trace), Density.ih, d(inv_temp), C.byref(e), C.byref(mu), solver_parameters.ih)
        return e.value, mu.value

    @staticmethod
    def WOM_GC(H, ISQ, Density, chemical_potential, inv_temp, solver_parameters):
        e = C.c_double()
        lib.WOM_GC_wrp(H.ih, ISQ.ih, Density.ih, d(chemical_potential), d(inv_temp), C.byref(e), solver_parameters.ih)
        return e.value

    @staticmethod
    def WOM_C(H, ISQ, Density, trace, inv_temp, solver_parameters):
        e = C.c_double()
        lib.WOM_C_wrp(H.ih, ISQ.ih, Density.ih, d(trace), d(inv_temp), C.byref(e), solver_parameters.ih)
        return e.value


class DenseSolvers:
    @staticmethod
    def DenseDensity(H, ISQ, trace, Density, solver_parameters):
        return DensityMatrixSolvers._run(lib.DenseDensity_wrp, H, ISQ, trace, Density, solver_parameters)

    @staticmethod
    def _f(name, In, Out, solver_parameters):
        getattr(lib, name)(In.ih, Out.ih, solver_parameters.ih)

    SquareRoot = staticmethod(lambda a, o, p: DenseSolvers._f("DenseSquareRoot_wrp", a, o, p))
    InverseSquareRoot = staticmethod(lambda a, o, p: DenseSolvers._f("DenseInverseSquareRoot_wrp", a, o, p))
    Exponential = staticmethod(lambda a, o, p: DenseSolvers._f("ComputeDenseExponential_wrp", a, o, p))
    Logarithm = staticmethod(lambda a, o, p: DenseSolvers._f("ComputeDenseLogarithm_wrp", a, o, p))
    Sine = staticmethod(lambda a, o, p: DenseSolvers._f("DenseSine_wrp", a, o, p))
    Cosine = staticmethod(lambda a, o, p: DenseSolvers._f("DenseCosine_wrp", a, o, p))
    Invert = staticmethod(lambda a, o, p: DenseSolvers._f("DenseInvert_wrp", a, o, p))
    SignFunction = staticmethod(lambda a, o, p: DenseSolvers._f("DenseSignFunction_wrp", a, o, p))


class LoadBalancer:
    @staticmethod
    def PermuteMatrix(mat_in, mat_out, permutation, memorypool=None):
        pool = memorypool if memorypool is not None else PMatrixMemoryPool(mat_in)
        lib.PermuteMatrix_wrp(mat_in.ih, mat_out.ih, permutation.ih, pool.ih)

    @staticmethod
    def UndoPermuteMatrix(mat_in, mat_out, permutation, memorypool=None):
        pool = memorypool if memorypool is not None else PMatrixMemoryPool(mat_in)
        lib.UndoPermuteMatrix_wrp(mat_in.ih, mat_out.ih, permutation.ih, pool.ih)


class EigenBounds:
    @staticmethod
    def PowerBounds(matrix, solver_parameters):
        v = C.c_double()
        lib.PowerBounds_wrp(matrix.ih, C.byref(v), solver_parameters.ih)
        return v.value

    @staticmethod
    def GershgorinBounds(matrix):
        mn, mx = C.c_double(), C.c_double()
        lib.GershgorinBounds_wrp(matrix.ih, C.byref(mn), C.byref(mx))
        return mn.value, mx.value


def ActivateLogger(start_document=False, file_name=None):
    if file_name:
        raw, n = s(file_name)
        lib.ActivateLoggerFile_wrp(b(start_document), raw, n)
    else:
        lib.ActivateLogger_wrp(b(start_document))


def DeactivateLogger():
    lib.DeactivateLogger_wrp()


def last_spgemm_stats():
    out = (C.c_longlong * 13)()
    a, t = C.c_float(), C.c_float()
    lib.ntpoly_amd_last_spgemm_stats(out, C.byref(a), C.byref(t))
    return dict(nnz_a=out[0], nnz_b=out[1], nnz_c=out[2], products=out[3], tmp_entries=out[4],
                bins=[out[5 + k] for k in range(6)], overflow=out[11], slab=out[12], ms_numeric=a.value, ms_total=t.value)


def band_order(M):
    pos = np.zeros(M.GetActualDimension(), dtype=np.int32)
    bw = C.c_longlong()
    lib.ntpoly_amd_band_order.restype = C.c_int
    ok = lib.ntpoly_amd_band_order(M.ih, pos.ctypes.data_as(C.c_void_p), C.byref(bw))
    return (pos, int(bw.value)) if ok else None


def fusion_counts():
    out = (C.c_longlong * 3)()
    lib.ntpoly_amd_fusion_counts(out)
    return dict(square=out[0], update=out[1], repeated=out[2])


def complex_fusion_counts():
    out = (C.c_longlong * 3)()
    lib.ntpoly_amd_complex_fusion_counts(out)
    return dict(square=out[0], update=out[1], repeated=out[2])


def tile2_counts():
    out = (C.c_longlong * 2)()
    lib.ntpoly_amd_tile2_counts(out)
    return dict(done=out[0], repeated=out[1])


def band_scope_counts():
    out = (C.c_longlong * 2)()
    lib.ntpoly_amd_band_scope_counts(out)
    return dict(solves=out[0], searched=out[1])


def block_scope_counts():
    out = (C.c_longlong * 2)()
    lib.ntpoly_amd_block_scope_counts(out)
    return dict(solves=out[0], products=out[1])


def band_searches():
    out = C.c_longlong()
    lib.ntpoly_amd_band_searches(C.byref(out))
    return int(out.value)


def slab_algebra_counts():
    out = (C.c_longlong * 4)()
    lib.ntpoly_amd_slab_algebra_counts(out)
    return dict(products=out[0], merges=out[1], others=out[2], refusals=out[3])


def slab_view_counts():
    out = (C.c_longlong * 4)()
    lib.ntpoly_amd_slab_view_counts(out)
    return dict(built=out[0], products=out[1], taken=out[2], declined=out[3])


def ghash_class_counts():
    out = (C.c_longlong * 4)()
    lib.ntpoly_amd_ghash_class_counts(out)
    return dict(real_mfma=out[0], real_vector=out[1], complex_mfma=out[2], complex_vector=out[3])


def drop_grouped_caches():
    lib.ntpoly_amd_drop_grouped_caches()


def panel_product_counts():
    out = (C.c_longlong * 3)()
    lib.ntpoly_amd_panel_product_counts(out)
    return dict(slab=out[0], declined=out[1], host_syncs=out[2])


def thin_slab_counts():
    out = (C.c_longlong * 6)()
    lib.ntpoly_amd_thin_slab_counts(out)
    return dict(real_left=out[0], real_right=out[1], complex_left=out[2], complex_right=out[3], panel_real=out[4], panel_complex=out[5])


@contextlib.contextmanager
def solver_session(complex_ok=True):
    lib.ntpoly_amd_session_begin(C.byref(C.c_int(1 if complex_ok else 0)))
    try:
        yield
    finally:
        lib.ntpoly_amd_session_end()


def recurrence_step(P, Tkm2, Tk, R, a, c):
    lib.ntpoly_amd_recurrence_step.restype = C.c_int
    return bool(lib.ntpoly_amd_recurrence_step(P.ih, Tkm2.ih, Tk.ih, R.ih, d(a), d(c)))


def recurrence_step_count():
    out = C.c_longlong()
    lib.ntpoly_amd_recurrence_step_count(C.byref(out))
    return int(out.value)


def pm_session_counts():
    out = (C.c_longlong * 4)()
    lib.ntpoly_amd_pm_session_counts(out)
    return dict(sigma=int(out[0]), updates=int(out[1]), zeros=int(out[2]), left=int(out[3]))


def pm_session_longest_list():
    out = C.c_longlong()
    lib.ntpoly_amd_pm_session_longest_list(C.byref(out))
    return int(out.value)


def pm_fused_step(X, Z, X2, X3, a1, a2, a3, thr, Out, Zout):
    sc = (C.c_double * 2)()
    lib.ntpoly_amd_pm_fused_step.restype = C.c_int
    ok = lib.ntpoly_amd_pm_fused_step(X.ih, Z.ih, X2.ih, X3.ih, d(a1), d(a2), d(a3), d(thr), Out.ih, Zout.ih, sc)
    return (sc[0], sc[1]) if ok else None


def isr_chain_counts():
    out = (C.c_longlong * 3)()
    lib.ntpoly_amd_isr_chain_counts(out)
    return dict(order5=int(out[0]), order3=int(out[1]), refused=int(out[2]))


def isr_chain_step(X, X2, order, a, b, c, Out1, Out2):
    lib.ntpoly_amd_isr_chain_step.restype = C.c_int
    ok = lib.ntpoly_amd_isr_chain_step(X.ih, X2.ih, C.byref(C.c_int(int(order))), d(a), d(b), d(c), Out1.ih, Out2.ih)
    return True if ok else None


def last_grouped_stats():
    out = (C.c_longlong * 6)()
    r = C.c_double()
    lib.ntpoly_amd_last_grouped_stats(out, C.byref(r))
    return dict(used=int(out[0]), failed_cols=int(out[1]), groups=int(out[2]), level=int(out[3]), minhash=int(out[4]),
                tile_rows=int(out[5]), union_ratio=r.value)


def last_block_stats():
    out = (C.c_longlong * 3)()
    r = C.c_double()
    lib.ntpoly_amd_last_block_stats(out, C.byref(r))
    return dict(used=int(out[0]), tile_products=int(out[1]), candidates=int(out[2]), fill=r.value)


def last_spgemm_thin():
    lib.ntpoly_amd_last_spgemm_thin.restype = C.c_int
    return int(lib.ntpoly_amd_last_spgemm_thin())


def block_order(M):
    pos = np.zeros(M.GetActualDimension(), dtype=np.int32)
    lib.ntpoly_amd_block_order.restype = C.c_int
    ok = lib.ntpoly_amd_block_order(M.ih, pos.ctypes.data_as(C.c_void_p))
    return pos if ok else None


def block_order_of_pattern(M):
    pos = np.zeros(M.GetActualDimension(), dtype=np.int32)
    ns = C.c_int()
    lib.ntpoly_amd_block_order_of_pattern.restype = C.c_int
    ok = lib.ntpoly_amd_block_order_of_pattern(M.ih, pos.ctypes.data_as(C.c_void_p), C.byref(ns))
    return (pos, int(ns.value)) if ok else None


def increment_identity(Identity, B, alpha):
    lib.ntpoly_amd_increment_identity(Identity.ih, B.ih, d(alpha))


def norm_axpby(A, B, alpha, beta):
    r = C.c_double()
    lib.ntpoly_amd_norm_axpby.restype = C.c_int
    ok = lib.ntpoly_amd_norm_axpby(A.ih, B.ih, d(alpha), d(beta), C.byref(r))
    return r.value if ok else None


def column_fused_counts():
    out = (C.c_longlong * 2)()
    lib.ntpoly_amd_column_fused_counts(out)
    return dict(identity_in_place=int(out[0]), norms_of_differences=int(out[1]))
# ... 58 lines not shown
```

Before: 690.3.

## Skip SpGEMM output tiles whose norm bound falls below the drop threshold

Adds per-32-element segment max-abs values for slab matrices, written by the tile SpGEMM epilogue (and by a separate segmax kernel when missing). Before computing a tile, a wave sums the products of A segment maxima and B row maxima as an upper bound on output magnitude. If that bound is under the threshold, the tile is zeroed and its computation skipped. This cuts multiply work on tiles that would be filtered anyway, at the cost of extra amax writes, bound evaluation, atomics and an added memory fence.

```diff
diff --git a/include/ntpoly_amd.h b/include/ntpoly_amd.h
--- a/include/ntpoly_amd.h
+++ b/include/ntpoly_amd.h
@@ -93,6 +93,7 @@
 void ntpoly_amd_synchronize();
 void ntpoly_amd_thin_slab_counts(long long* out);
 void ntpoly_amd_tile2_counts(long long* out);
+void ntpoly_amd_tile_skip_counts(long long* out);
 void ntpoly_amd_trace_get(double* value, double* energy, double* sigma, long long* nnz);
 int ntpoly_amd_trace_iterations();
 void ntpoly_amd_trace_times(double* setup_ms, double* loop_ms);
diff --git a/ntpoly_amd/csrc/common.hpp b/ntpoly_amd/csrc/common.hpp
--- a/ntpoly_amd/csrc/common.hpp
+++ b/ntpoly_amd/csrc/common.hpp
@@ -110,6 +110,7 @@
   DevBuf<int64_t> off;
   DevBuf<int64_t> tile_off;
   DevBuf<double> val, tiles;
+  DevBuf<double> amax;
   int64_t slots = 0;
   bool no_tile2 = false;
   std::unique_ptr<SlabPlan> next_plan;
diff --git a/ntpoly_amd/csrc/kernels.hip b/ntpoly_amd/csrc/kernels.hip
--- a/ntpoly_amd/csrc/kernels.hip
+++ b/ntpoly_amd/csrc/kernels.hip
@@ -2766,6 +2766,10 @@
   return c;
 }
 long long* tile2_counts() {
+  static long long c[2] = {0, 0};
+  return c;
+}
+long long* tile_skip_counts() {
   static long long c[2] = {0, 0};
   return c;
 }
@@ -4019,6 +4023,26 @@
 }
 }
 
+namespace {
+__global__ __launch_bounds__(256) void k_slab_segmax(const double* __restrict__ val, int64_t n, double* __restrict__ amax, int64_t nseg) {
+  const int64_t i = (int64_t)blockIdx.x * blockDim.x + threadIdx.x;
+  double mx = 0.0;
+  if (2 * i + 1 < n) {
+    const double2 v = reinterpret_cast<const double2*>(val)[i];
+    mx = fmax(fabs(v.x), fabs(v.y));
+  } else if (2 * i < n) mx = fabs(val[2 * i]);
+  for (int o = 8; o > 0; o >>= 1) mx = fmax(mx, __shfl_xor(mx, o, WAVE));
+  if ((threadIdx.x & 15) == 0 && (i >> 4) < nseg) amax[i >> 4] = mx;
+}
+}
+
+static void slab_segmax(SlabForm& f) {
+  const int64_t nseg = (int64_t)f.val.n / 32 + 1;
+  f.amax.alloc((size_t)nseg);
+  const int64_t threads = (nseg * 16 + 255) / 256 * 256;
+  hipLaunchKernelGGL(k_slab_segmax, dim3((unsigned)(threads / 256)), dim3(256), 0, stream(), f.val.p, (int64_t)f.val.n, f.amax.p, nseg);
+}
+
 bool slab_step(DevMat& X, SlabFusion& fu, double threshold, bool dense_rule, const SlabHalo* halo) {
   fu.done = false;
   if (!X.expanded() || X.cplx || (!halo && X.rows != X.cols) || !fu.D || fu.D->cplx || fu.D->loose() || fu.D->expanded() ||
@@ -4098,6 +4122,9 @@
   const size_t oslots = (size_t)tmp_total + (size_t)tmp_total / 5 + kIndexSlack;
   const bool runs_only = tile && !halo && options().tile_runs_only != 0;
   DevBuf<double> oval(oslots), otiles(runs_only ? 0 : oslots);
+  const bool want_skip = tile && !halo && options().tile_skip != 0 && trows == 2 && in.row_pad == 32 && plan_align == 32 && !in.labelled();
+  DevBuf<double> oamax;
+  bool skip_ran = false;
   SlabFuseArgs fz;
   fz.am = fu.am; fz.bm = fu.bm; fz.thr_m = fu.threshold;
   fz.xexp = in.val.p; fz.xoff = in.off.p; fz.xmin = in.first.p; fz.xmax = in.last.p;
@@ -4182,7 +4209,17 @@
       tl.dbase = dop.dexp.p; tl.dbytes = dop.dexp.n * sizeof(double);
     }
     if (!halo && options().tile2 != 0 && !in.no_tile2) used_tile2 = launch_spgemm_tile2(tl, reinterpret_cast<int*>(fz_flag) + 2);
-    if (!used_tile2) launch_spgemm_tile(tl);
+    if (!used_tile2) {
+      if (want_skip) {
+        tl.amax_bytes = ((size_t)in.val.n / 32 + 1) * sizeof(double);
+        if (spgemm_tile_skips(tl)) {
+          if (!in.amax.p) slab_segmax(*X.slab);
+          oamax.alloc(oslots / 32 + 1);
+          tl.amax = in.amax.p; tl.amax_bytes = in.amax.n * sizeof(double); tl.oamax = oamax.p;
+        }
+      }
+      skip_ran = launch_spgemm_tile(tl);
+    }
   } else if (rowoff) {
     if (max_w > 6 * SLAB_SL * WAVE) by_mode(std::integral_constant<int, 8>{}, std::integral_constant<int, 9>{});
     else if (max_w > SLAB_NW * SLAB_SL * WAVE) by_mode(std::integral_constant<int, 6>{}, std::integral_constant<int, 9>{});
@@ -4225,6 +4262,7 @@
   R.slab->off = tile ? std::move(tile_ooff) : std::move(tmpoff);
   if (tile) R.slab->tile_off = std::move(tile_otoff);
   R.slab->val = std::move(oval);
+  if (skip_ran) R.slab->amax = std::move(oamax);
   if (runs_only) { R.slab->tile_off.release(); } else R.slab->tiles = std::move(otiles);
   R.slab->slots = tmp_total;
   {
@@ -4246,8 +4284,9 @@
     next->max_kn = (int)next_hs[1];
   }
   if (std::getenv("NTPOLY_AMD_DEBUG_SPGEMM"))
-    std::fprintf(stderr, "[slab_step] mode %d slots %lld w %llu kn %llu in-slots %lld nnz-in %lld plan %s\n", fu.mode, (long long)tmp_total,
-                 hst[0], hst[1], (long long)in.slots, (long long)X.nnz, plan == &own_plan ? "made here" : "left by the step before");
+    std::fprintf(stderr, "[slab_step] mode %d slots %lld w %llu kn %llu in-slots %lld nnz-in %lld plan %s; tile skip %s, tiles tested %lld skipped %lld\n", fu.mode, (long long)tmp_total,
+                 hst[0], hst[1], (long long)in.slots, (long long)X.nnz, plan == &own_plan ? "made here" : "left by the step before",
+                 skip_ran ? "on" : want_skip ? "wanted, not in this instantiation" : "off", (long long)((uint64_t)flagv[0] >> 32), (long long)((uint64_t)flagv[1] >> 32));
   if (timing) {
     if (pending_timings().size() >= 4096) flush_spgemm_timers();
     pending_timings().push_back(TimedCall{{t_all.a, t_all.b, t_num.a, t_num.b}});
@@ -4258,6 +4297,10 @@
     return slab_step(X, fu, threshold, dense_rule, halo);
   }
   if (used_tile2) tile2_counts()[0] += 1;
+  if (skip_ran) {
+    tile_skip_counts()[0] += (long long)(uint32_t)((uint64_t)flagv[0] >> 32);
+    tile_skip_counts()[1] += (long long)(uint32_t)((uint64_t)flagv[1] >> 32);
+  }
   if ((int32_t)flagv[0] != 0) {
     fu.refused += 1;
     fusion_counts()[2] += 1;
@@ -5970,6 +6013,7 @@
   f.tiles.release();
   f.tile_off.release();
   f.next_plan.reset();
+  f.amax.release();
   return true;
 }
 
diff --git a/ntpoly_amd/csrc/kernels.hpp b/ntpoly_amd/csrc/kernels.hpp
--- a/ntpoly_amd/csrc/kernels.hpp
+++ b/ntpoly_amd/csrc/kernels.hpp
@@ -42,6 +42,7 @@
   int complex_tile = 1;
   int block_complex = 1;
   int tile2 = 0;
+  int tile_skip = 1;
   int tile_runs_only = 1;
   int load_balance = 1;
   int virtual_grid = 0;
@@ -211,6 +212,7 @@
 long long* fusion_counts();
 long long* complex_fusion_counts();
 long long* tile2_counts();
+long long* tile_skip_counts();
 long long& band_searches();
 
 void increment(const DevMat& A, DevMat& B, double alpha, double threshold);
diff --git a/ntpoly_amd/csrc/slab_extra.hip b/ntpoly_amd/csrc/slab_extra.hip
--- a/ntpoly_amd/csrc/slab_extra.hip
+++ b/ntpoly_amd/csrc/slab_extra.hip
@@ -93,6 +93,7 @@
   B.nnz += (long long)h[1];
   f.tiles.release();
   f.tile_off.release();
+  f.amax.release();
   return true;
 }
 
diff --git a/ntpoly_amd/csrc/spgemm_tile.hip b/ntpoly_amd/csrc/spgemm_tile.hip
--- a/ntpoly_amd/csrc/spgemm_tile.hip
+++ b/ntpoly_amd/csrc/spgemm_tile.hip
@@ -92,6 +92,9 @@
   uint32_t abytes;
   const void* dbase;
   uint32_t dbytes;
+  const double* amax;
+  uint32_t amax_bytes;
+  double* oamax;
   int ablate;
 #ifdef NTP_TILE_STAMPS
   long long* stamps;
@@ -544,6 +547,19 @@
   const int mid = (T - 1) >> 1;
 
   [[maybe_unused]] int sidx = 4;
+  constexpr bool SKIPK = EPI != 0 && R == 2 && OFF32 && !LAB && (TILE_NW == 4 || TILE_NW == 8);
+  [[maybe_unused]] const bool skip_on = SKIPK && a.amax != nullptr && a.oamax != nullptr;
+  [[maybe_unused]] auto seg_max = [&](const typename RowVec<R>::type (&x)[4]) {
+    double mx = 0.0;
+#pragma unroll
+    for (int v = 0; v < 4; ++v) {
+#pragma unroll
+      for (int m = 0; m < R; ++m) mx = fmax(mx, fabs(rv_get<R>(x[v], m)));
+    }
+    mx = fmax(mx, __shfl_xor(mx, 16, WAVE));
+    return fmax(mx, __shfl_xor(mx, 32, WAVE));
+  };
+  [[maybe_unused]] auto seg_of = [&](int r) { return ((int64_t)(orun - a.out_val) + r) >> 5; };
 #ifdef NTP_TILE_STATIC
   for (int ti = 0;; ++ti) {
     const int ts = ti * TILE_NW + ((ti & 1) ? TILE_NW - 1 - wave : wave);
@@ -569,6 +585,36 @@
         g1 = c + 63 - (int)__builtin_clzll(m);
       }
     }
+    if constexpr (SKIPK) {
+      if (skip_on && g1 >= g0) {
+        bool cand;
+        if constexpr (EPI == 2) cand = __ballot(xf <= r0 + TROWS - 1 && xlrow >= r0) == 0ull;
+        else cand = 2 * (g1 - g0 + 1) <= KG;
+        if (cand) {
+          const __amdgpu_buffer_rsrc_t mrsrc = __builtin_amdgcn_make_buffer_rsrc(const_cast<double*>(a.amax), 0, a.amax_bytes, 0x00020000);
+          double bsum = 0.0;
+          for (int kk = 4 * g0 + lane; kk <= 4 * g1 + 3; kk += WAVE) {
+            const uint4 rc = reinterpret_cast<const uint4*>(recs)[kk];
+            const bool meets = (int)rc.z <= r0 + TROWS - R && (int)rc.z + (int)rc.w >= r0;
+            const double am_k = __builtin_bit_cast(double, __builtin_amdgcn_raw_buffer_load_b64(mrsrc, meets ? (((rc.x + (unsigned)r0 * 8u) >> 8) << 3) : TILE_OOB, 0, 0));
+            const double* __restrict__ brow = Bs + kk * BP;
+            double bm_k = 0.0;
+#pragma unroll
+            for (int c = 0; c < SLAB_J; ++c) bm_k = fmax(bm_k, fabs(brow[c]));
+            bsum = __dadd_rn(bsum, __dmul_rn(am_k, bm_k));
+          }
+          bsum = wave_sum_f64(bsum);
+          if (!dense_rule) bsum = __dmul_rn(bsum, fabs(alpha));
+          const bool skipped = __ballot(!(__dmul_rn(bsum, 1.0 + 0x1p-30) <= thr)) == 0ull;
+          if (lane == 0) atomicAdd(&misc[5], skipped ? 0x10001 : 1);
+          if (skipped) {
+            if (lane == 0) colmask[t] = 0u;
+            STAMP(sidx); ++sidx;
+            continue;
+          }
+        }
+      }
+    }
     [[maybe_unused]] VR xv[4], dv[4];
     auto epilogue_loads = [&]() {
 #pragma unroll
@@ -711,6 +757,12 @@
         }
 #pragma unroll
         for (int v = 0; v < 4; ++v) rv_store<R>(orun + (r0 + R * (4 * v + q)), both[v]);
+        if constexpr (SKIPK) {
+          if (skip_on) {
+            const double mx = seg_max(both);
+            if (q == 0) a.oamax[seg_of(r0)] = mx;
+          }
+        }
         if (otile) {
 #pragma unroll
           for (int v = 0; v < 4; ++v) {
@@ -807,6 +859,12 @@
 #pragma unroll
       for (int v = 0; v < 4; ++v) rv_store<R>(orun + (r0 + R * (4 * v + q)), res[v]);
     }
+    if constexpr (SKIPK) {
+      if (skip_on) {
+        const double mx = seg_max(res);
+        if (q == 0 && ((cm >> jj) & 1u)) a.oamax[seg_of(r0)] = mx;
+      }
+    }
     if constexpr (EPI != 0) {
       if (cm && otile) {
 #pragma unroll
@@ -900,6 +958,11 @@
       a.otoff[b] = tbase + (tk1 >= tk0 ? (int64_t)(tk0 - lo) * SLAB_J : 0);
       a.fzv.pnnz[b] = misc[1];
       if (a.fzv.prod) a.fzv.prod[b] = *reinterpret_cast<long long*>(misc + 2);
+      if constexpr (SKIPK) {
+        const int sk = misc[5];
+        if (sk & 0xffff) atomicAdd(a.fzv.flag + 1, sk & 0xffff);
+        if (sk >> 16) atomicAdd(a.fzv.flag + 3, sk >> 16);
+      }
     }
     if (tid == 64) {
       double x = 0.0, y = 0.0;
@@ -928,13 +991,18 @@
     }
   }
   for (int p = tid; p < T * SLAB_J; p += TILE_NW * WAVE) {
-    const int t = p >> 4, c = p & 15;
+    const int t = p >> 4;
+    int c = p & 15;
+    asm volatile("" : "+v"(c));
     const unsigned cmk = colmask[t];
     const int cf = col_first[c], cl = col_last[c];
     const int r0 = lo + TROWS * t;
     if (cl >= cf && r0 + TROWS - 1 >= cf && r0 <= cl && !((cmk >> c) & 1u)) {
       double* dst = a.out_val + (tbase + (int64_t)c * w - lo);
       for (int r = r0; r < min(r0 + TROWS, rend); ++r) dst[r] = 0.0;
+      if constexpr (SKIPK) {
+        if (skip_on) a.oamax[(tbase + (int64_t)c * w + (r0 - lo)) >> 5] = 0.0;
+      }
     }
     if constexpr (EPI != 0) {
       if (a.fzv.tiles && tk1 >= tk0 && r0 + TROWS - 1 >= tk0 && r0 <= tk1 && cmk == 0u) {
@@ -946,11 +1014,17 @@
   if constexpr (EPI == 2) {
     const int nd = min(misc[0], TILE_DEFER);
     if (nd > 0) {
+      asm volatile("s_waitcnt vmcnt(0)" ::: "memory");
       __syncthreads();
       for (int i = tid; i < nd; i += TILE_NW * WAVE) {
         const TileDefer e = dlist[i];
         if (!e.pad) continue;
         a.out_val[tbase + (int64_t)e.jj * w + (e.r - lo)] = e.o;
+        if constexpr (SKIPK) {
+          if (skip_on)
+            atomicMax(reinterpret_cast<unsigned long long*>(a.oamax + ((tbase + (int64_t)e.jj * w + (e.r - lo)) >> 5)),
+                      (unsigned long long)__double_as_longlong(fabs(e.o)));
+        }
         if (a.fzv.tiles) a.fzv.tiles[tbase + (int64_t)(e.r - lo) * SLAB_J + e.jj] = e.o;
       }
     }
@@ -981,8 +1055,43 @@
   return max_kn > 0 && max_w > 0 && std::max(tile_lds_bytes(k4, tm, 16 * tm + 64), tile_lds_bytes(k4, tm, 0)) <= 150 * 1024;
 }
 
-void launch_spgemm_tile(const TileLaunch& L) {
+namespace {
+struct TileGeometry {
+  bool off32;
+  int nw;
+  size_t lds;
+};
+TileGeometry tile_geometry(const TileLaunch& L) {
+  TileGeometry g;
+  g.off32 = options().tile_off32 != 0 && L.abase != nullptr && L.abytes > 0 && L.abytes < 0xfffff000ull;
+  if (g.off32 && L.epi != 0) {
+    const SlabFuseArgs& fzh = *static_cast<const SlabFuseArgs*>(L.fz);
+    const char *a0 = static_cast<const char*>(L.abase), *x0 = reinterpret_cast<const char*>(fzh.xexp);
+    g.off32 = L.dbase != nullptr && L.dbytes > 0 && L.dbytes < 0xfffff000ull && (L.epi != 2 || (x0 >= a0 && x0 < a0 + L.abytes));
+  }
+  const int k4max = std::max(8, (L.max_kn + 3) & ~3);
+  const int trows = 16 * (L.rows == 4 ? 4 : L.rows == 2 ? 2 : 1);
+  const int tmax = (L.max_w + trows - 1) / trows;
+  g.lds = tile_lds_bytes(k4max, tmax, (L.labelled && L.epi != 0) ? tmax * trows : 0);
+#ifdef NTP_TILE_WIDE3
+  const bool wide = 3 * ((g.lds + 511) & ~(size_t)511) > 160 * 1024;
+#else
+  const bool wide = 4 * ((g.lds + 511) & ~(size_t)511) > 160 * 1024;
+#endif
+  const int tw = options().tile_waves;
+  g.nw = (tw == 4 || tw == 5 || tw == 6 || tw == 8) ? tw : (wide ? 8 : 4);
+  return g;
+}
+}
+
+bool spgemm_tile_skips(const TileLaunch& L) {
+  const TileGeometry g = tile_geometry(L);
+  return L.amax_bytes > 0 && L.amax_bytes < 0xffffff00ull && L.epi != 0 && L.rows == 2 && !L.labelled && g.off32 && (g.nw == 4 || g.nw == 8);
+}
+
+bool launch_spgemm_tile(const TileLaunch& L) {
   TileArgs a;
+  const TileGeometry geo = tile_geometry(L);
   a.runs = static_cast<const SlabRun*>(L.runs);
   a.bblk = L.bblk; a.blk_boff = L.blk_boff; a.blk_kmin = L.blk_kmin; a.blk_kn = L.blk_kn; a.blk_lo = L.blk_lo; a.blk_w = L.blk_w;
   a.blk_toff = L.blk_toff; a.out_val = L.out_val; a.count = L.count; a.ofirst = L.ofirst; a.olast = L.olast; a.ooff = L.ooff;
@@ -1002,12 +1111,7 @@
     zeros->zero();
   }
   a.zero = zeros->p;
-  bool off32 = options().tile_off32 != 0 && L.abase != nullptr && L.abytes > 0 && L.abytes < 0xfffff000ull;
-  if (off32 && L.epi != 0) {
-    const SlabFuseArgs& fzh = *static_cast<const SlabFuseArgs*>(L.fz);
-    const char *a0 = static_cast<const char*>(L.abase), *x0 = reinterpret_cast<const char*>(fzh.xexp);
-    off32 = L.dbase != nullptr && L.dbytes > 0 && L.dbytes < 0xfffff000ull && (L.epi != 2 || (x0 >= a0 && x0 < a0 + L.abytes));
-  }
+  const bool off32 = geo.off32;
   a.abase = off32 ? L.abase : nullptr;
   a.abytes = off32 ? (uint32_t)L.abytes : 0u;
   a.dbase = off32 ? L.dbase : nullptr;
@@ -1023,14 +1127,12 @@
   blkdur->zero();
   a.blkdur = blkdur->p;
 #endif
-  const size_t lds = tile_lds_bytes(a.k4max, a.tmax, (L.labelled && L.epi != 0) ? a.tmax * trows : 0);
-#ifdef NTP_TILE_WIDE3
-  const bool wide = 3 * ((lds + 511) & ~(size_t)511) > 160 * 1024;
-#else
-  const bool wide = 4 * ((lds + 511) & ~(size_t)511) > 160 * 1024;
-#endif
-  const int tw = options().tile_waves;
-  const int nw = (tw == 4 || tw == 5 || tw == 6 || tw == 8) ? tw : (wide ? 8 : 4);
+  const size_t lds = geo.lds;
+  const int nw = geo.nw;
+  const bool skip = L.amax != nullptr && L.oamax != nullptr && spgemm_tile_skips(L);
+  a.amax = skip ? L.amax : nullptr;
+  a.amax_bytes = skip ? (uint32_t)L.amax_bytes : 0u;
+  a.oamax = skip ? L.oamax : nullptr;
   auto go = [&](auto epi_tag, auto nw_tag, auto r_tag, auto lab_tag, auto off_tag) {
     constexpr int E = decltype(epi_tag)::value, NW = decltype(nw_tag)::value, RR = decltype(r_tag)::value;
     constexpr bool LB = decltype(lab_tag)::value, OF = decltype(off_tag)::value;
@@ -1084,6 +1186,7 @@
     if (FILE* fp = std::fopen((std::string(f) + ".blocks").c_str(), "wb")) { std::fwrite(hb.data(), 8, hb.size(), fp); std::fclose(fp); }
   }
 #endif
-}
-
-}
+  return skip;
+}
+
+}
diff --git a/ntpoly_amd/csrc/spgemm_tile.hpp b/ntpoly_amd/csrc/spgemm_tile.hpp
--- a/ntpoly_amd/csrc/spgemm_tile.hpp
+++ b/ntpoly_amd/csrc/spgemm_tile.hpp
@@ -29,13 +29,17 @@
   size_t abytes = 0;
   const void* dbase = nullptr;
   size_t dbytes = 0;
+  const double* amax = nullptr;
+  size_t amax_bytes = 0;
+  double* oamax = nullptr;
   int nrows = 0;
   bool labelled = false;
 };
 bool spgemm_tile_fits(int max_kn, int max_w);
 int tile_rows();
 inline int tile_expand_align() { return 16 * tile_rows(); }
-void launch_spgemm_tile(const TileLaunch& a);
+bool spgemm_tile_skips(const TileLaunch& a);
+bool launch_spgemm_tile(const TileLaunch& a);
 bool launch_spgemm_tile2(const TileLaunch& a, int* fail);
 bool spgemm_tile_c_fits(int max_kn, int max_w);
 void launch_spgemm_tile_c(const TileLaunch& a);
diff --git a/ntpoly_amd/csrc/wrp.cpp b/ntpoly_amd/csrc/wrp.cpp
--- a/ntpoly_amd/csrc/wrp.cpp
+++ b/ntpoly_amd/csrc/wrp.cpp
@@ -163,6 +163,7 @@
   else if (n == "block_path") options().block_path = *value;
   else if (n == "tile_runs_only") options().tile_runs_only = *value;
   else if (n == "tile2") options().tile2 = *value;
+  else if (n == "tile_skip") options().tile_skip = *value;
   else if (n == "complex_tile") options().complex_tile = *value;
   else if (n == "block_complex") options().block_complex = *value;
   else if (n == "thin_left") options().thin_left = *value;
@@ -182,6 +183,7 @@
   if (n == "plan_ahead") return options().plan_ahead;
   if (n == "tile_rows") return options().tile_rows;
   if (n == "tile2") return options().tile2;
+  if (n == "tile_skip") return options().tile_skip;
   if (n == "block_path") return options().block_path;
   if (n == "label_order") return options().label_order;
   if (n == "band_scope") return options().band_scope;
@@ -324,6 +326,9 @@
 void ntpoly_amd_tile2_counts(long long* out) {
   for (int q = 0; q < 2; ++q) out[q] = tile2_counts()[q];
 }
+void ntpoly_amd_tile_skip_counts(long long* out) {
+  for (int q = 0; q < 2; ++q) out[q] = tile_skip_counts()[q];
+}
 void ntpoly_amd_gather_matrix_to_process(const int* ih_this, int* ih_local, const int* within_slice_id) {
   const PSMatrix& m = *get<PSMatrix>(ih_this);
   DevMat full = ps_gather_full(m);
@@ -363,7 +368,8 @@
   out[1] = column_fused_counts()[1];
 }
 void ntpoly_amd_increment_identity(const int* ih_identity, int* ih_matB, const double* alpha) {
-  ps_increment_identity(*get<PSMatrix>(ih_identity), *get<PSMatrix>(ih_matB), *alpha);
+  PSMatrix* B = (g_test_session && g_test_session->opened) ? get_unpacked(ih_matB) : get<PSMatrix>(ih_matB);
+  ps_increment_identity(*get<PSMatrix>(ih_identity), *B, *alpha);
 }
 int ntpoly_amd_norm_axpby(const int* ih_matA, const int* ih_matB, const double* alpha, const double* beta, double* norm) {
   return ps_norm_axpby(*get<PSMatrix>(ih_matA), *get<PSMatrix>(ih_matB), *alpha, *beta, norm) ? 1 : 0;
@@ -387,6 +393,7 @@
 void ntpoly_amd_reset_spgemm_accum() {
   flush_spgemm_timers();
   spgemm_accum() = SpgemmAccum();
+  tile_skip_counts()[0] = tile_skip_counts()[1] = 0;
 }
 void ntpoly_amd_get_spgemm_accum(long long* out, double* dout) {
   flush_spgemm_timers();
diff --git a/ntpoly_amd/host.py b/ntpoly_amd/host.py
--- a/ntpoly_amd/host.py
+++ b/ntpoly_amd/host.py
@@ -864,6 +864,12 @@
     return dict(done=out[0], repeated=out[1])
 
 
+def tile_skip_counts():
+    out = (C.c_longlong * 2)()
+    lib.ntpoly_amd_tile_skip_counts(out)
+    return (int(out[0]), int(out[1]))
+
+
 def band_scope_counts():
     out = (C.c_longlong * 2)()
     lib.ntpoly_amd_band_scope_counts(out)
```

Result: faster. 721.9 (median of 6 runs) (+4.6%).
